# lizhiqi49/threestudio-3dgs

Measured on AMD Instinct MI355X. Metric: rendered views/sec fwd+bwd @1M Gaussians, 1024², SH=3; 1/2/4/8 GPU, higher is better.
Workload: dtype fp32

## Files before the change

threestudio-3dgs_amd/csrc/gsr_api.hip:

```cpp
#include <stdio.h>
#include <string.h>

#include <cmath>
#include <mutex>
#include <vector>

#include "../../include/gsr.h"
#include "gsr_kernels.h"

using namespace gsr;

static thread_local char g_err[512] = "";

static int fail(int code, const char* fmt, const char* what) {
  snprintf(g_err, sizeof(g_err), fmt, what);
  return code;
}

#define GSR_HIP_CHECK(expr)                                                        \
  do {                                                                             \
    hipError_t e_ = (expr);                                                        \
    if (e_ != hipSuccess) return fail(GSR_EHIP, "HIP error: %s", hipGetErrorString(e_)); \
  } while (0)

// ... 75 lines not shown
  int dm = (int)std::lround(std::sqrt((double)(M > 0 ? M : 1))) - 1;
  int d = degree < dm ? degree : dm;
  if (d < 0) d = 0;
  if (d > 3) d = 3;
  return d;
}

static int tile_sort_result(int W, int H) { return digit_plan(tile_key_bits(W, H)).passes & 1; }
static int depth_sort_result() { return digit_plan(32).passes & 1; }

static GaussBackwardArgs shared_args(const gsr_set_scene& sc, const gsr_set_grads& gr) {
  GaussBackwardArgs a;
  a.P = sc.P;
  a.g0 = 0;
  a.g1 = sc.P;
  a.M = sc.shs ? sc.M : 0;
  a.deg = effective_degree(sc.degree, a.M);
  a.means3D = sc.means3D;
  a.scales = sc.scales;
  a.rotations = sc.rotations;
  a.shs = sc.shs;
  a.cov3D_precomp = sc.cov3D_precomp;
  a.scale_modifier = sc.scale_modifier;
  a.dL_dcolors = gr.dL_dcolors;
  a.dL_dopacity = gr.dL_dopacity;
  a.dL_dmeans3D = gr.dL_dmeans3D;
  a.dL_dcov3D = gr.dL_dcov3D;
  a.dL_dsh = sc.shs ? gr.dL_dsh : nullptr;
  a.dL_dscales = sc.cov3D_precomp ? nullptr : gr.dL_dscales;
  a.dL_drotations = sc.cov3D_precomp ? nullptr : gr.dL_drotations;
  return a;
}

static int inst_segments(int V, const int* K, SegInfo& seg, long long* total) {
  seg.V = V;
  long long run = 0;
  for (int v = 0; v < V; ++v) {
    if (K[v] < 0) return fail(GSR_EINVAL, "%s", "negative instance count");
    seg.n[v] = (uint32_t)K[v];
    seg.start[v] = (uint32_t)run;
    run += K[v];
    if (run >= (1ll << 32)) return fail(GSR_EINVAL, "%s", "instances of a view set exceed 2^32: use smaller sets");
  }
  seg_fill_blocks(seg, GSR_SORT_TILE);
  if (total) *total = run;
  return GSR_OK;
}

static int set_cams(const gsr_set_scene& sc, SetCams& cams) {
  if (sc.viewmatrices == nullptr || sc.projmatrices == nullptr || sc.campos == nullptr || sc.tanfovx == nullptr ||
      sc.tanfovy == nullptr)
    return fail(GSR_EINVAL, "%s", "null camera array");
  for (int v = 0; v < sc.V; ++v) {
    if (sc.viewmatrices[v] == nullptr || sc.projmatrices[v] == nullptr || sc.campos[v] == nullptr)
      return fail(GSR_EINVAL, "%s", "null camera pointer");
    cams.c[v].view = sc.viewmatrices[v];
    cams.c[v].proj = sc.projmatrices[v];
    cams.c[v].campos = sc.campos[v];
    cams.c[v].tanx = sc.tanfovx[v];
    cams.c[v].tany = sc.tanfovy[v];
  }
  return GSR_OK;
}

static int check_set(int V, int P) {
  if (V < 1 || V > GSR_SET_MAX) return fail(GSR_EINVAL, "%s", "a view set holds 1..64 views");
  if (P < 0) return fail(GSR_EINVAL, "%s", "P must be >= 0");
  if ((long long)V * (long long)(P > 0 ? P : 1) >= (1ll << 32))
    return fail(GSR_EINVAL, "%s", "views x Gaussians of a set exceed 2^32: use smaller sets");
  return GSR_OK;
}

static void render_set_shared(RenderSet& rs, const GeomState& g, const ImageState& img, const BinningState& b,
                              const TilePack& tp, int tres, int V, int P, int width, int height) {
  rs.P = P;
  rs.W = width;
  rs.H = height;
  rs.gx = div_up(width, GSR_TILE_X);
  rs.gy = div_up(height, GSR_TILE_Y);
  rs.gmask = tp.gmask;
  rs.col2_rec = g.drange + 130;
  rs.order = img.order;
  rs.split_mode = img.split_mode;
  rs.split_items = img.split_items;
  rs.split_cap = img.split_cap;
  rs.split_extra = split_extra(V, (size_t)rs.gx * rs.gy);
  rs.qkeys = tp.qmask ? b.key[tres] : nullptr;
}

extern "C" {

#ifndef GSR_BUILD_ID
#define GSR_BUILD_ID "unknown"
#endif
const char* gsr_version(void) { return "gsr 0.4.0 gfx950 build " GSR_BUILD_ID; }
int gsr_abi_version(void) { return GSR_ABI_VERSION; }
const char* gsr_last_error(void) { return g_err; }


size_t gsr_set_geom_bytes(int V, int P) {
  size_t b = 0;
  GeomState::carve(nullptr, V, P, &b);
  return b;
}
static bool set_total(int V, const int* K, SegInfo& seg, long long* total) {
  return V >= 1 && V <= GSR_SET_MAX && K != nullptr && inst_segments(V, K, seg, total) == GSR_OK;
}
size_t gsr_set_binning_bytes(int V, int P, const int* K, int width, int height) {
  SegInfo seg;
  long long total = 0;
  if (!set_total(V, K, seg, &total)) return 0;
  size_t b = 0;
  BinningState::carve(nullptr, V, total, seg.blk[V], !set_tile_pack(P, width, height).packed, &b);
  return b;
}
size_t gsr_set_image_bytes(int V, int P, const int* K, int width, int height, int two_colors) {
  SegInfo seg;
  long long total = 0;
  if (K != nullptr && !set_total(V, K, seg, &total)) return 0;
  size_t b = 0;
  ImageState::carve(nullptr, V, width, height, &b,
                    K == nullptr || split_forward(V, P, width, height, total, two_colors != 0));
  return b;
}
static size_t carry_bytes(int P) { return align_up(sizeof(float) * 6 * (size_t)(P > 0 ? P : 1), 256); }

size_t gsr_set_backward_bytes(int V, int P, const int* K, int two_colors) {
  SegInfo seg;
  long long total = 0;
  if (!set_total(V, K, seg, &total)) return 0;
  return BackwardState::bytes_for(total, V, P, two_colors != 0) + carry_bytes(P);
}

static int check_timed(const gsr_set_scene& sc, const gsr_set_timed& tm) {
  if (sc.shs != nullptr) return fail(GSR_EINVAL, "%s", "timed view sets take precomputed colours: shs is not built");
  if (sc.cov3D_precomp != nullptr) return fail(GSR_EINVAL, "%s", "timed view sets: cov3D_precomp is not built");
  if (tm.means3D_v == nullptr && sc.P > 0) return fail(GSR_EINVAL, "%s", "timed view sets need means3D_v");
  return GSR_OK;
}
static gsr_set_scene timed_scene(const gsr_set_scene& sc, const gsr_set_timed& tm) {
  gsr_set_scene e = sc;
  e.means3D = tm.means3D_v;
  if (tm.scales_v != nullptr) e.scales = tm.scales_v;
  if (tm.rotations_v != nullptr) e.rotations = tm.rotations_v;
  return e;
}

static int set_preprocess(const gsr_set_scene* scene, const gsr_set_state* state, const float* colors2,
                          const gsr_set_timed* timed, void* stream) {
  const gsr_set_scene& sc = *scene;
  const int V = sc.V, P = sc.P;
  if (check_set(V, P) != GSR_OK) return GSR_EINVAL;
  if (sc.width <= 0 || sc.height <= 0) return fail(GSR_EINVAL, "%s", "image size must be positive");
  if ((sc.shs == nullptr) == (sc.colors_precomp == nullptr))
    return fail(GSR_EINVAL, "%s", "Please provide exactly one of either SHs or precomputed colors!");
  if (((sc.scales == nullptr || sc.rotations == nullptr) && sc.cov3D_precomp == nullptr) ||
      ((sc.scales != nullptr || sc.rotations != nullptr) && sc.cov3D_precomp != nullptr))
    return fail(GSR_EINVAL, "%s",
                "Please provide exactly one of either scale/rotation pair or precomputed 3D covariance!");
  if (state->geom == nullptr ||
      (P > 0 && (sc.means3D == nullptr || sc.opacities == nullptr || state->radii == nullptr)))
    return fail(GSR_EINVAL, "%s", "null pointer argument");
  if (sc.shs != nullptr && sc.M <= 0) return fail(GSR_EINVAL, "%s", "M must be >= 1 with SHs");
  SetCams cams;
  if (set_cams(sc, cams) != GSR_OK) return GSR_EINVAL;
  for (int v = 0; v < V; ++v) {
    cams.c[v].fx = (float)sc.width / (2.0f * cams.c[v].tanx);
    cams.c[v].fy = (float)sc.height / (2.0f * cams.c[v].tany);
  }
  hipStream_t s = (hipStream_t)stream;
  GeomState g = GeomState::carve(state->geom, V, P, nullptr);

  PreprocessArgs a;
  a.V = V;
  a.P = P;
  a.deg = effective_degree(sc.degree, sc.M);
  a.M = sc.M;
  a.means3D = sc.means3D;
  a.scales = sc.scales;
  a.rotations = sc.rotations;
  a.opacities = sc.opacities;
  a.shs = sc.shs;
  a.colors_precomp = sc.colors_precomp;
  a.cov3D_precomp = sc.cov3D_precomp;
  a.scale_modifier = sc.scale_modifier;
  a.W = sc.width;
  a.H = sc.height;
  a.radii = state->radii;
  a.col2 = colors2;
  {
    PhaseScope ps(GSR_PHASE_PREPROCESS, s);
    if (timed != nullptr) {
      const size_t n = (size_t)P;
      const PreprocessTimed pt = {3 * n, timed->scales_v ? 3 * n : 0, timed->rotations_v ? 4 * n : 0, 3 * n};
      launch_preprocess(a, cams, g, s, &pt);
    } else {
      launch_preprocess(a, cams, g, s);
    }
  }
  {
    PhaseScope ps(GSR_PHASE_DEPTH_SORT, s);
    SegInfo seg;
    seg.V = V;
    for (int v = 0; v < V; ++v) {
      seg.n[v] = (uint32_t)P;
      seg.start[v] = (uint32_t)((size_t)v * P);
    }
    seg.rebase = g.drange + 128;
    const int res = seg_sort(g.dkey, g.dval, false, seg, 0, 32, g.sort_counts, g.sort_totals, s);
    if (res != depth_sort_result()) return fail(GSR_EHIP, "%s", "internal: depth sort result buffer");
    launch_binning_counts(V, P, g, s);
  }
  return last_launch();
}

int gsr_set_preprocess(const gsr_set_scene* scene, const gsr_set_state* state, const float* colors2, void* stream) {
  if (scene == nullptr || state == nullptr) return fail(GSR_EINVAL, "%s", "null pointer argument");
  return set_preprocess(scene, state, colors2, nullptr, stream);
}

int gsr_set_timed_preprocess(const gsr_set_scene* scene, const gsr_set_state* state, const gsr_set_timed* timed,
                             void* stream) {
  if (scene == nullptr || state == nullptr || timed == nullptr) return fail(GSR_EINVAL, "%s", "null pointer argument");
  if (check_timed(*scene, *timed) != GSR_OK) return GSR_EINVAL;
  const gsr_set_scene e = timed_scene(*scene, *timed);
  return set_preprocess(&e, state, timed->colors2_v, timed, stream);
}

int gsr_composite_forward(int V, int height, int width, const float* color, const float* alpha, const float* bg,
                          int bg_layout, float* out, void* stream) {
  if (V < 0 || height < 0 || width < 0 || bg_layout < 0 || bg_layout > 2) return fail(GSR_EINVAL, "%s", "bad sizes");
  if (V == 0 || height == 0 || width == 0) return last_launch();
  if (color == nullptr || alpha == nullptr || bg == nullptr || out == nullptr)
    return fail(GSR_EINVAL, "%s", "null pointer argument");
  launch_composite_fwd(V, (size_t)height * width, color, alpha, bg, bg_layout, out, (hipStream_t)stream);
  return last_launch();
}

int gsr_composite_backward(int V, int height, int width, const float* dL_dout, const float* color,
                           const float* alpha, const float* bg, int bg_layout, float* dL_dcolor, float* dL_dalpha,
                           float* dL_dbg, void* stream) {
  if (V < 0 || height < 0 || width < 0 || bg_layout < 0 || bg_layout > 2) return fail(GSR_EINVAL, "%s", "bad sizes");
  if (V == 0 || height == 0 || width == 0) return last_launch();
  if (dL_dout == nullptr || color == nullptr || alpha == nullptr || bg == nullptr || dL_dcolor == nullptr ||
      dL_dalpha == nullptr)
    return fail(GSR_EINVAL, "%s", "null pointer argument");
  if (dL_dbg != nullptr && bg_layout == GSR_BG_CONSTANT)
    return fail(GSR_EINVAL, "%s", "dL_dbg is computed for image backgrounds only");
  launch_composite_bwd(V, (size_t)height * width, dL_dout, color, alpha, bg, bg_layout, dL_dcolor, dL_dalpha,
                       dL_dbg, (hipStream_t)stream);
  return last_launch();
}

int gsr_normal_map_forward(int V, int height, int width, const float* normal, const float* alpha, float* out,
                           void* stream) {
  if (V < 0 || height < 0 || width < 0) return fail(GSR_EINVAL, "%s", "bad sizes");
  if (V == 0 || height == 0 || width == 0) return last_launch();
  if (normal == nullptr || alpha == nullptr || out == nullptr) return fail(GSR_EINVAL, "%s", "null pointer argument");
  launch_normal_map_fwd(V, (size_t)height * width, normal, alpha, out, (hipStream_t)stream);
  return last_launch();
}

int gsr_normal_map_backward(int V, int height, int width, const float* dL_dout, const float* normal,
                            const float* alpha, float* dL_dnormal, float* dL_dalpha, void* stream) {
  if (V < 0 || height < 0 || width < 0) return fail(GSR_EINVAL, "%s", "bad sizes");
  if (V == 0 || height == 0 || width == 0) return last_launch();
  if (dL_dout == nullptr || normal == nullptr || alpha == nullptr || dL_dnormal == nullptr || dL_dalpha == nullptr)
    return fail(GSR_EINVAL, "%s", "null pointer argument");
  launch_normal_map_bwd(V, (size_t)height * width, dL_dout, normal, alpha, dL_dnormal, dL_dalpha, (hipStream_t)stream);
  return last_launch();
}

static int shade_args(int V, int H, int W, int flags, const int* modes, const float* color, const float* depth,
                      const float* alpha, const float* rays_o, const float* rays_d, const float* bg, int bg_layout,
                      const float* light, const float* pred_normal, const float* ambient, const float* diffuse,
                      ShadeArgs& A) {
  if (V < 0 || H < 0 || W < 0 || (flags & ~GSR_SHADE_MATERIAL) != 0)
    return fail(GSR_EINVAL, "%s", "bad sizes / flags");
  if (depth == nullptr || alpha == nullptr || rays_o == nullptr || rays_d == nullptr)
    return fail(GSR_EINVAL, "%s", "null pointer argument (depth / alpha / rays)");
  A = ShadeArgs{};
  A.V = V, A.H = H, A.W = W, A.flags = flags, A.bg_layout = bg_layout;
  A.color = color, A.depth = depth, A.alpha = alpha, A.rays_o = rays_o, A.rays_d = rays_d;
  A.bg = bg, A.light = light, A.pred_normal = pred_normal;
  if (flags & GSR_SHADE_MATERIAL) {
    if (color == nullptr || bg == nullptr || light == nullptr || ambient == nullptr || diffuse == nullptr ||
        modes == nullptr)
      return fail(GSR_EINVAL, "%s", "material: color, bg, light, ambient, diffuse and modes are required");
    if (bg_layout != GSR_BG_CONSTANT && bg_layout != GSR_BG_HWC)
      return fail(GSR_EINVAL, "%s", "material: bg_layout must be GSR_BG_CONSTANT or GSR_BG_HWC");
    for (int v = 0; v < V; ++v)
      if (modes[v] < GSR_SHADING_DIFFUSE || modes[v] > GSR_SHADING_TEXTURELESS)
        return fail(GSR_EINVAL, "%s", "bad shading mode");
  }
  return GSR_OK;
}

static void shade_launch(ShadeArgs A, const ShadeGrads* G, const int* modes, const float* ambient,
                         const float* diffuse, hipStream_t s) {
  const int V = A.V;
  for (int v0 = 0; v0 < V; v0 += GSR_SET_MAX) {
    const int n = V - v0 < GSR_SET_MAX ? V - v0 : GSR_SET_MAX;
    A.v0 = v0, A.V = n;
    for (int i = 0; i < n; ++i) {
      A.mode[i] = (A.flags & GSR_SHADE_MATERIAL) ? modes[v0 + i] : 0;
      for (int k = 0; k < 3; ++k) {
// ... 548 lines not shown
  if (((uintptr_t)c.pairs & 15u) != 0) return fail(GSR_EINVAL, "%s", "pairs must be 16-byte aligned");
  if (((uintptr_t)workspace & 7u) != 0) return fail(GSR_EINVAL, "%s", "workspace must be 8-byte aligned");
  if (workspace_bytes < meshreg_workspace_bytes(c.T, c.V, c.P, pass))
    return fail(GSR_EINVAL, "%s", "workspace too small");
  return GSR_OK;
}

size_t gsr_sugar_meshreg_workspace_bytes(int T, int V, int P, int pass) {
  if (pass < GSR_MESHREG_FORWARD || pass > GSR_MESHREG_LAP_BACKWARD) return 0;
  return meshreg_workspace_bytes(T < 0 ? 0 : T, V < 0 ? 0 : V, P < 0 ? 0 : P, pass);
}

int gsr_sugar_normal_consistency_forward(const gsr_sugar_meshreg* in, float* nc, void* workspace,
                                         size_t workspace_bytes, void* stream) {
  if (in == nullptr) return null_argument();
  if (meshreg_check(*in) != GSR_OK) return GSR_EINVAL;
  if (in->T == 0 || in->P == 0) return nothing_to_do();
  if (meshreg_args(*in, true, nc, "nc", workspace, workspace_bytes, false) != GSR_OK) return GSR_EINVAL;
  launch_normal_consistency_forward(*in, nc, workspace, (hipStream_t)stream);
  return last_launch();
}

int gsr_sugar_normal_consistency_backward(const gsr_sugar_meshreg* in, const float* dL_dnc, float* dL_dvert_xyz,
                                          void* workspace, size_t workspace_bytes, void* stream) {
  if (in == nullptr) return null_argument();
  if (meshreg_check(*in) != GSR_OK) return GSR_EINVAL;
  if (in->T == 0 || in->P == 0) return nothing_to_do();
  if (dL_dnc == nullptr) return null_named("dL_dnc");
  if (meshreg_args(*in, true, dL_dvert_xyz, "dL_dvert_xyz", workspace, workspace_bytes, true) != GSR_OK)
    return GSR_EINVAL;
  launch_normal_consistency_backward(*in, dL_dnc, dL_dvert_xyz, workspace, (hipStream_t)stream);
  return last_launch();
}

int gsr_sugar_laplacian_forward(const gsr_sugar_meshreg* in, float* lap, void* workspace, size_t workspace_bytes,
                                void* stream) {
  if (in == nullptr) return null_argument();
  if (meshreg_check(*in) != GSR_OK) return GSR_EINVAL;
  if (in->T == 0 || in->V == 0) return nothing_to_do();
  if (meshreg_args(*in, false, lap, "lap", workspace, workspace_bytes, false) != GSR_OK) return GSR_EINVAL;
  launch_laplacian_forward(*in, lap, workspace, (hipStream_t)stream);
  return last_launch();
}

int gsr_sugar_laplacian_backward(const gsr_sugar_meshreg* in, const float* dL_dlap, float* dL_dvert_xyz,
                                 void* workspace, size_t workspace_bytes, void* stream) {
  if (in == nullptr) return null_argument();
  if (meshreg_check(*in) != GSR_OK) return GSR_EINVAL;
  if (in->T == 0 || in->V == 0) return nothing_to_do();
  if (dL_dlap == nullptr) return null_named("dL_dlap");
  if (meshreg_args(*in, false, dL_dvert_xyz, "dL_dvert_xyz", workspace, workspace_bytes, true) != GSR_OK)
    return GSR_EINVAL;
  launch_laplacian_backward(*in, dL_dlap, dL_dvert_xyz, workspace, (hipStream_t)stream);
  return last_launch();
}

int gsr_densify_stats(const gsr_densify_batch* in, void* stream) {
  if (in == nullptr) return null_argument();
  if (in->V < 0 || in->V > GSR_SET_MAX) return fail(GSR_EINVAL, "%s", "a densification call takes 0..64 views");
  if (in->P < 0) return fail(GSR_EINVAL, "%s", "P must be >= 0");
  if (in->P == 0 || in->V == 0) return nothing_to_do();
  if (in->max_radii == nullptr) return null_named("max_radii");
  if (in->grad_norm_sum == nullptr) return null_named("grad_norm_sum");
  if (in->count == nullptr) return null_named("count");
  int with_rows = 0;
  for (int v = 0; v < in->V; ++v) {
    if (in->radii[v] == nullptr) return null_named("radii row");
    with_rows += in->visible[v] != nullptr;
  }
  if (with_rows != 0 && with_rows != in->V)
    return fail(GSR_EINVAL, "%s", "visibility rows must be given for every view or for none");
  launch_densify_stats(*in, (hipStream_t)stream);
  return last_launch();
}

struct SortWork {
  uint32_t *keys2, *vals2, *counts, *totals;
  static SortWork carve(void* base, int V, long long total, uint32_t blocks, size_t* bytes) {
    Carver c(base);
    SortWork w;
    w.keys2 = c.take<uint32_t>((size_t)(total > 0 ? total : 1));
    w.vals2 = c.take<uint32_t>((size_t)(total > 0 ? total : 1));
    w.counts = c.take<uint32_t>((size_t)GSR_RADIX * (blocks > 0 ? blocks : 1));
    w.totals = c.take<uint32_t>((size_t)GSR_RADIX * (size_t)V);
    if (bytes) *bytes = align_up(c.off, 256);
    return w;
  }
};

size_t gsr_sort_work_bytes(int V, const int* n) {
  SegInfo seg;
  long long total = 0;
  if (!set_total(V, n, seg, &total)) return 0;
  size_t b = 0;
  SortWork::carve(nullptr, V, total, seg.blk[V], &b);
  return b;
}

int gsr_sort_pairs(int V, const int* n, uint32_t* keys, uint32_t* vals, int key_bits, int max_bits, void* work,
                   size_t work_bytes, void* stream) {
  if (V < 1 || V > GSR_SET_MAX) return fail(GSR_EINVAL, "%s", "1..64 segments");
  if (n == nullptr || keys == nullptr || work == nullptr) return fail(GSR_EINVAL, "%s", "null pointer argument");
  if (key_bits < 1 || key_bits > 32 || max_bits < 1 || max_bits > GSR_RADIX_BITS)
    return fail(GSR_EINVAL, "%s", "key_bits must be 1..32 and max_bits 1..8");
  SegInfo seg;
  long long total = 0;
  if (inst_segments(V, n, seg, &total) != GSR_OK) return GSR_EINVAL;
  size_t need = 0;
  SortWork w = SortWork::carve(work, V, total, seg.blk[V], &need);
  if (work_bytes < need) return fail(GSR_EINVAL, "%s", "sort work buffer too small");
  if (total == 0) return last_launch();
  hipStream_t s = (hipStream_t)stream;
  uint32_t* kk[2] = {keys, w.keys2};
  uint32_t* vv[2] = {vals, vals != nullptr ? w.vals2 : nullptr};
  const int r = seg_sort(kk, vals != nullptr ? vv : nullptr, false, seg, 0, key_bits, w.counts, w.totals, s,
                         max_bits);
  if (r == 1) {
    GSR_HIP_CHECK(hipMemcpyAsync(keys, w.keys2, sizeof(uint32_t) * (size_t)total, hipMemcpyDeviceToDevice, s));
    if (vals != nullptr)
      GSR_HIP_CHECK(hipMemcpyAsync(vals, w.vals2, sizeof(uint32_t) * (size_t)total, hipMemcpyDeviceToDevice, s));
  }
  return last_launch();
}

int gsr_sort_rank_mode(void) { return sort_rank_mode(); }

int gsr_set_num_rendered(int V, const void* geom, int P, int* num_rendered, int* num_visible, int* num_listed,
                         void* stream) {
  if (check_set(V, P) != GSR_OK) return GSR_EINVAL;
  if (geom == nullptr || num_rendered == nullptr) return fail(GSR_EINVAL, "%s", "null pointer argument");
  GeomState g = GeomState::carve((void*)geom, V, P, nullptr);
  hipStream_t s = (hipStream_t)stream;
  static thread_local uint32_t* pinned = nullptr;
  if (pinned == nullptr) GSR_HIP_CHECK(hipHostMalloc((void**)&pinned, 3 * GSR_SET_MAX * sizeof(uint32_t), hipHostMallocDefault));
  GSR_HIP_CHECK(hipMemcpyAsync(pinned, g.counters, 3 * (size_t)V * sizeof(uint32_t), hipMemcpyDeviceToHost, s));
  GSR_HIP_CHECK(hipStreamSynchronize(s));
  for (int v = 0; v < V; ++v) {
    num_rendered[v] = (int)pinned[v];
    if (num_visible) num_visible[v] = (int)pinned[V + v];
    if (num_listed) num_listed[v] = (int)pinned[2 * V + v];
    if (pinned[v] > 0x7fffffffu) return fail(GSR_EINVAL, "%s", "instance count of a view exceeds 2^31");
  }
  g_err[0] = 0;
  return GSR_OK;
}

int gsr_set_gauss_state(int V, const void* geom, int P, void* out_rec, void* out_tiles, void* stream) {
  if (check_set(V, P) != GSR_OK) return GSR_EINVAL;
  if (geom == nullptr) return fail(GSR_EINVAL, "%s", "null pointer argument");
  if (P == 0) return GSR_OK;
  GeomState g = GeomState::carve((void*)geom, V, P, nullptr);
  hipStream_t s = (hipStream_t)stream;
  const size_t n = (size_t)V * (size_t)P;
  if (out_rec) GSR_HIP_CHECK(hipMemcpyAsync(out_rec, g.rec, n * sizeof(GaussRec), hipMemcpyDeviceToDevice, s));
  if (out_tiles) GSR_HIP_CHECK(hipMemcpyAsync(out_tiles, g.tiles, n * sizeof(uint2), hipMemcpyDeviceToDevice, s));
  return last_launch();
}

int gsr_set_render(const gsr_set_scene* scene, const gsr_set_state* state, const gsr_set_outputs* outputs,
                   void* stream) {
  if (scene == nullptr || state == nullptr || outputs == nullptr)
    return fail(GSR_EINVAL, "%s", "null pointer argument");
  const gsr_set_outputs& o = *outputs;
  const int V = scene->V, P = scene->P, width = scene->width, height = scene->height;
  const int* K = state->num_rendered;
  const float* const* bgs = scene->bgs;
  void *geom = state->geom, *binning = state->binning, *image = state->image;
  const float* colors2 = o.colors2;
  if (check_set(V, P) != GSR_OK) return GSR_EINVAL;
  if ((colors2 == nullptr) != (o.out_color2 == nullptr)) return fail(GSR_EINVAL, "%s", "null second colour argument");
  if (o.bg_images != nullptr && o.out_render == nullptr) return fail(GSR_EINVAL, "%s", "composite needs out_render");
  if (width <= 0 || height <= 0) return fail(GSR_EINVAL, "%s", "bad sizes");
  if (K == nullptr || bgs == nullptr || geom == nullptr || binning == nullptr || image == nullptr ||
      o.out_color == nullptr || o.out_depth == nullptr || o.out_alpha == nullptr)
    return fail(GSR_EINVAL, "%s", "null pointer argument");
  for (int v = 0; v < V; ++v)
    if (bgs[v] == nullptr) return fail(GSR_EINVAL, "%s", "null background");
  SegInfo inst;
  long long total = 0;
  if (inst_segments(V, K, inst, &total) != GSR_OK) return GSR_EINVAL;
  hipStream_t s = (hipStream_t)stream;
  GeomState g = GeomState::carve(geom, V, P, nullptr);
  const TilePack tp = set_tile_pack(P, width, height);
  BinningState b = BinningState::carve(binning, V, total, inst.blk[V], !tp.packed, nullptr);
  const bool split = split_forward(V, P, width, height, total, colors2 != nullptr);
  ImageState img = ImageState::carve(image, V, width, height, nullptr, split);
  const int gx = div_up(width, GSR_TILE_X), gy = div_up(height, GSR_TILE_Y);
  const int tres = tile_sort_result(width, height);
  inst.ndev = g.counters + 2 * V;
  GSR_HIP_CHECK(hipMemsetAsync(img.split_mode, split ? 1 : 0, sizeof(uint32_t), s));
  const bool tile_masks = fwd_tile_chosen(total, (long long)V * P, V);
  GSR_HIP_CHECK(hipMemsetAsync(img.split_mode + 1, total > 0 ? (tile_masks ? 1 : 2) : 0, sizeof(uint32_t), s));
  {
    PhaseScope ps(GSR_PHASE_BINNING, s);
    GSR_HIP_CHECK(hipMemsetAsync(img.ranges, 0, sizeof(uint2) * (size_t)V * gx * gy, s));
    if (total > 0) {
      launch_emit(V, P, width, g, inst, tp, b.key[0], b.val[0], s);
      const int res = seg_sort(b.key, b.val, false, inst, tp.gbits, tp.tile_bits, b.sort_counts, b.sort_totals, s);
      if (res != tres) return fail(GSR_EHIP, "%s", "internal: tile sort buffer");
      launch_tile_ranges(inst, gx * gy, tp, b.key[res], img.ranges, s);
    }
    launch_tile_order(V, gx, gy, img.ranges, img.order, s);
  }
  {
    PhaseScope ps(GSR_PHASE_RENDER_FWD, s);
    RenderSet rs;
    render_set_shared(rs, g, img, b, tp, tres, V, P, width, height);
    rs.cbg = o.bg_images;
    rs.comp = o.out_render;
    rs.ccolor = nullptr;
    rs.dcbg = nullptr;
    rs.col2 = colors2;
    rs.out_col2 = o.out_color2;
    rs.dpix2 = nullptr;
    rs.ochunk = order_chunk(V, gx, gy, true);
    rs.ckpt = split ? img.ckpt : nullptr;
    rs.qbytes = total > 0 ? reinterpret_cast<uint8_t*>(b.key[tres ^ 1]) : nullptr;
    rs.V = V;
    rs.v0 = 0;
    for (int v = 0; v < V; ++v) {
      rs.inst_start[v] = inst.start[v];
      rs.row_start[v] = 0;
      rs.bg[v] = bgs[v];
    }
    launch_render_forward(rs, g, tp.packed ? b.key[tres] : b.val[tres], img, o.out_color, o.out_depth, o.out_alpha,
                          total, s);
  }
  return last_launch();
}

static int grad_chunk_size(int P, int n) {
  const int q = (P + n - 1) / n;
  return (q + GSR_GRAD_CHUNK_ALIGN - 1) / GSR_GRAD_CHUNK_ALIGN * GSR_GRAD_CHUNK_ALIGN;
}

static int set_backward(const gsr_set_scene* scene, const gsr_set_state* state, const gsr_set_grads* grads,
                        const gsr_set_timed* timed, const gsr_set_timed_grads* tgrads, void* stream) {
  const gsr_set_scene& sc = *scene;
  const gsr_set_grads& gr = *grads;
  const int V = sc.V, P = sc.P, width = sc.width, height = sc.height;
  const int* K = state->num_rendered;
  const float* const* bgs = sc.bgs;
  const float *colors_override = gr.colors_override, *color = gr.color, *comp_bg = gr.bg_images;
  float *dL_dcov3D = gr.dL_dcov3D, *dL_dbg = gr.dL_dbg;
  const float *dL_dcolor = gr.dL_dcolor, *dL_ddepth = gr.dL_ddepth, *dL_dalpha = gr.dL_dalpha;
  if (check_set(V, P) != GSR_OK) return GSR_EINVAL;
  const bool two = gr.colors2 != nullptr || gr.dL_dcolor2 != nullptr || gr.dL_dcolors2 != nullptr;
  if (two && (gr.colors2 == nullptr || gr.dL_dcolor2 == nullptr || gr.dL_dcolors2 == nullptr ||
              colors_override != nullptr))
    return fail(GSR_EINVAL, "%s", "two-colour backward needs colors2, dL_dcolor2 and dL_dcolors2");
  if (colors_override != nullptr && (sc.shs != nullptr || gr.dL_dsh != nullptr || dL_ddepth != nullptr ||
                                     dL_dalpha != nullptr))
    return fail(GSR_EINVAL, "%s", "colors_override excludes SHs and the depth / alpha gradients");
  if (comp_bg != nullptr && color == nullptr) return fail(GSR_EINVAL, "%s", "composite needs the forward's color");
  if (comp_bg == nullptr && dL_dbg != nullptr) return fail(GSR_EINVAL, "%s", "dL_dbg needs bg_images");
  if (gr.n_chunks < 0 || gr.n_chunks > GSR_GRAD_CHUNKS_MAX || (gr.n_chunks > 0 && gr.chunk_events == nullptr))
    return fail(GSR_EINVAL, "%s", "bad gradient chunk request");
  if (width <= 0 || height <= 0) return fail(GSR_EINVAL, "%s", "bad sizes");
  if (P == 0) return last_launch();
  if (K == nullptr || bgs == nullptr || state->geom == nullptr || state->binning == nullptr ||
      state->image == nullptr || gr.work == nullptr || dL_dcolor == nullptr || gr.dL_dmeans2D == nullptr ||
      gr.dL_dcolors == nullptr || gr.dL_dopacity == nullptr || (timed == nullptr && gr.dL_dmeans3D == nullptr) ||
      state->radii == nullptr || sc.means3D == nullptr)
    return fail(GSR_EINVAL, "%s", "null pointer argument");
  for (int v = 0; v < V; ++v)
    if (bgs[v] == nullptr) return fail(GSR_EINVAL, "%s", "null background");
  if (sc.shs != nullptr && gr.dL_dsh == nullptr) return fail(GSR_EINVAL, "%s", "dL_dsh required with SHs");
  const bool need_dscales = timed == nullptr || timed->scales_v == nullptr;
  const bool need_drots = timed == nullptr || timed->rotations_v == nullptr;
  if (sc.cov3D_precomp == nullptr && (sc.scales == nullptr || sc.rotations == nullptr ||
                                      (need_dscales && gr.dL_dscales == nullptr) ||
                                      (need_drots && gr.dL_drotations == nullptr)))
    return fail(GSR_EINVAL, "%s", "scales/rotations and their gradients required");
  SetCams cams;
  if (set_cams(sc, cams) != GSR_OK) return GSR_EINVAL;
  SegInfo inst;
  long long total = 0;
  if (inst_segments(V, K, inst, &total) != GSR_OK) return GSR_EINVAL;
  hipStream_t s = (hipStream_t)stream;
  GeomState g = GeomState::carve(state->geom, V, P, nullptr);
  const TilePack tp = set_tile_pack(P, width, height);
  BinningState b = BinningState::carve(state->binning, V, total, inst.blk[V], !tp.packed, nullptr);
  ImageState img = ImageState::carve(state->image, V, width, height, nullptr, true);
  const int gx = div_up(width, GSR_TILE_X), gy = div_up(height, GSR_TILE_Y);
  const size_t HW = (size_t)width * height;
  const int tres = tile_sort_result(width, height);
  const uint32_t* sorted = tp.packed ? b.key[tres] : b.val[tres];
  GaussBackwardArgs a = shared_args(sc, gr);
  if (timed == nullptr && gr.accumulate != 0 && sc.cov3D_precomp == nullptr && dL_dcov3D == nullptr)
    return fail(GSR_EINVAL, "%s", "accumulate needs dL_dcov3D: it carries the running dL/dcov3D between calls");
  void* work = gr.work;
  if (gr.work_bytes < carry_bytes(P)) return fail(GSR_EINVAL, "%s", "backward work buffer too small");
  const size_t avail = (gr.work_bytes - carry_bytes(P)) & ~(size_t)255;
  float* carry = dL_dcov3D ? dL_dcov3D : (float*)((char*)work + avail);
  bool first = gr.accumulate == 0;
  for (int g0 = 0; g0 < V;) {
    int g1 = g0;
    long long rows = 0;
    while (g1 < V && (g1 == g0 || BackwardState::bytes_for(rows + K[g1], g1 + 1 - g0, P, two) <= avail))
      rows += K[g1++];
    if (BackwardState::bytes_for(rows, g1 - g0, P, two) > avail)
      return fail(GSR_EINVAL, "%s", "backward work buffer smaller than one view's gradient rows");
    BackwardState bw = BackwardState::carve(work, rows, P, two);
    RenderSet rs;
    render_set_shared(rs, g, img, b, tp, tres, V, P, width, height);
    rs.cbg = comp_bg ? comp_bg + (size_t)g0 * HW * 3 : nullptr;
    rs.comp = nullptr;
// ... 237 lines not shown
```

threestudio-3dgs_amd/csrc/gsr_backward.hip:

```cpp
#include <cstdlib>
#include <cstring>

#include "gsr_chain.h"
#include "gsr_kernels.h"
#include "gsr_math.h"
#include "gsr_wave.h"

namespace gsr {

__device__ __forceinline__ void sh_backward(int deg, int M, const float* sh, float (&dsh)[48], float3 dRGB,
                                            const float3 mean, const float* campos, float3& dmean) {
  const float3 dir_orig = make_float3(mean.x - campos[0], mean.y - campos[1], mean.z - campos[2]);
  const float len = sqrtf(dir_orig.x * dir_orig.x + dir_orig.y * dir_orig.y + dir_orig.z * dir_orig.z);
  const float x = dir_orig.x / len, y = dir_orig.y / len, z = dir_orig.z / len;
  float basis[16];
  float bdx[16], bdy[16], bdz[16];
#pragma unroll
  for (int k = 0; k < 16; ++k) basis[k] = bdx[k] = bdy[k] = bdz[k] = 0.f;
  basis[0] = SH_C0;
  if (deg > 0) {
    basis[1] = -SH_C1 * y; basis[2] = SH_C1 * z; basis[3] = -SH_C1 * x;
    bdy[1] = -SH_C1; bdz[2] = SH_C1; bdx[3] = -SH_C1;
    if (deg > 1) {
      const float xx = x * x, yy = y * y, zz = z * z, xy = x * y, yz = y * z, xz = x * z;
      basis[4] = SH_C2[0] * xy; basis[5] = SH_C2[1] * yz;
      basis[6] = SH_C2[2] * (2.f * zz - xx - yy); basis[7] = SH_C2[3] * xz;
      basis[8] = SH_C2[4] * (xx - yy);
      bdx[4] = SH_C2[0] * y; bdy[4] = SH_C2[0] * x;
      bdy[5] = SH_C2[1] * z; bdz[5] = SH_C2[1] * y;
      bdx[6] = SH_C2[2] * 2.f * -x; bdy[6] = SH_C2[2] * 2.f * -y; bdz[6] = SH_C2[2] * 2.f * 2.f * z;
      bdx[7] = SH_C2[3] * z; bdz[7] = SH_C2[3] * x;
      bdx[8] = SH_C2[4] * 2.f * x; bdy[8] = SH_C2[4] * 2.f * -y;
      if (deg > 2) {
        basis[9] = SH_C3[0] * y * (3.f * xx - yy);
        basis[10] = SH_C3[1] * xy * z;
        basis[11] = SH_C3[2] * y * (4.f * zz - xx - yy);
        basis[12] = SH_C3[3] * z * (2.f * zz - 3.f * xx - 3.f * yy);
        basis[13] = SH_C3[4] * x * (4.f * zz - xx - yy);
        basis[14] = SH_C3[5] * z * (xx - yy);
        basis[15] = SH_C3[6] * x * (xx - 3.f * yy);
        bdx[9] = SH_C3[0] * 3.f * 2.f * xy;          bdy[9] = SH_C3[0] * 3.f * (xx - yy);
        bdx[10] = SH_C3[1] * yz;                     bdy[10] = SH_C3[1] * xz;          bdz[10] = SH_C3[1] * xy;
        bdx[11] = SH_C3[2] * -2.f * xy;              bdy[11] = SH_C3[2] * (-3.f * yy + 4.f * zz - xx);
        bdz[11] = SH_C3[2] * 4.f * 2.f * yz;
        bdx[12] = SH_C3[3] * -3.f * 2.f * xz;        bdy[12] = SH_C3[3] * -3.f * 2.f * yz;
        bdz[12] = SH_C3[3] * 3.f * (2.f * zz - xx - yy);
        bdx[13] = SH_C3[4] * (-3.f * xx + 4.f * zz - yy); bdy[13] = SH_C3[4] * -2.f * xy;
        bdz[13] = SH_C3[4] * 4.f * 2.f * xz;
        bdx[14] = SH_C3[5] * 2.f * xz;               bdy[14] = SH_C3[5] * -2.f * yz;   bdz[14] = SH_C3[5] * (xx - yy);
        bdx[15] = SH_C3[6] * 3.f * (xx - yy);        bdy[15] = SH_C3[6] * -3.f * 2.f * xy;
      }
    }
  }
  const int ncoef = (deg + 1) * (deg + 1);
  float3 dRGBdx = make_float3(0.f, 0.f, 0.f), dRGBdy = dRGBdx, dRGBdz = dRGBdx;
#pragma unroll
  for (int k = 0; k < 16; ++k) {
    if (k < ncoef && k < M) {
      dsh[3 * k] += basis[k] * dRGB.x;
      dsh[3 * k + 1] += basis[k] * dRGB.y;
      dsh[3 * k + 2] += basis[k] * dRGB.z;
      if (k > 0) {
        const float3 s = make_float3(sh[3 * k], sh[3 * k + 1], sh[3 * k + 2]);
        dRGBdx.x += bdx[k] * s.x; dRGBdx.y += bdx[k] * s.y; dRGBdx.z += bdx[k] * s.z;
        dRGBdy.x += bdy[k] * s.x; dRGBdy.y += bdy[k] * s.y; dRGBdy.z += bdy[k] * s.z;
        dRGBdz.x += bdz[k] * s.x; dRGBdz.y += bdz[k] * s.y; dRGBdz.z += bdz[k] * s.z;
      }
    }
  }
  const float3 ddir = make_float3(dRGBdx.x * dRGB.x + dRGBdx.y * dRGB.y + dRGBdx.z * dRGB.z,
                                  dRGBdy.x * dRGB.x + dRGBdy.y * dRGB.y + dRGBdy.z * dRGB.z,
                                  dRGBdz.x * dRGB.x + dRGBdz.y * dRGB.y + dRGBdz.z * dRGB.z);
  const float3 v = dir_orig;
  const float sum2 = v.x * v.x + v.y * v.y + v.z * v.z;
  const float invsum32 = 1.0f / sqrtf(sum2 * sum2 * sum2);
  dmean.x += ((sum2 - v.x * v.x) * ddir.x - v.y * v.x * ddir.y - v.z * v.x * ddir.z) * invsum32;
  dmean.y += (-v.x * v.y * ddir.x + (sum2 - v.y * v.y) * ddir.y - v.z * v.y * ddir.z) * invsum32;
  dmean.z += (-v.x * v.z * ddir.x - v.y * v.z * ddir.y + (sum2 - v.z * v.z) * ddir.z) * invsum32;
}

static inline __host__ __device__ int sh_lds_stride(int M) { return ((3 * M + 3) & ~3) + 4; }

#ifndef GSR_VG_ITEMS
#define GSR_VG_ITEMS 16
#endif
template <bool TWO, bool CUT_LDS>
__attribute__((amdgpu_waves_per_eu(4, 8)))
__global__ __launch_bounds__(256) void k_view_grad(GaussBackwardArgs a, ViewGradArgs va) {
  extern __shared__ uint2 s_cut[];
  const int t = threadIdx.x;
  const int vl = blockIdx.x % va.V;
  const int vg = va.v0 + vl;
  const uint2* cut = CUT_LDS ? reinterpret_cast<const uint2*>(s_cut) : va.img.cut + (size_t)vg * va.tiles;
  if (CUT_LDS) {
    const uint4* src = reinterpret_cast<const uint4*>(va.img.cut + (size_t)vg * va.tiles);
    uint4* dst = reinterpret_cast<uint4*>(s_cut);
    for (int k = t; k < va.tiles / 2; k += 256) dst[k] = src[k];
    if ((va.tiles & 1) && t == 0) s_cut[va.tiles - 1] = va.img.cut[(size_t)vg * va.tiles + va.tiles - 1];
    __syncthreads();
  }
  const ViewCam& cam = va.cam[vl];
  typedef __attribute__((address_space(4))) const float* cfptr;
  float viewm[16], projm[16];
#pragma unroll
  for (int i = 0; i < 16; ++i) viewm[i] = ((cfptr)cam.view)[i], projm[i] = ((cfptr)cam.proj)[i];
  ViewGeom vgm;
  vgm.view = viewm;
  vgm.proj = projm;
  vgm.tanx = cam.tanx;
  vgm.tany = cam.tany;
  vgm.fy = va.H / (2.0f * cam.tany);
  vgm.fx = va.W / (2.0f * cam.tanx);
  const float4* grow = va.grow + (size_t)(TWO ? 4 : 3) * va.row_start[vl];
  constexpr int RS = TWO ? GSR_REC_STRIDE2 : GSR_REC_STRIDE;
  float4* recv = reinterpret_cast<float4*>(va.vrec + (size_t)vl * RS * a.P);
  const unsigned long long vbit = 1ull << vl;
  __shared__ uint16_t s_list[4][64 * GSR_VG_ITEMS];
  const int wave = t >> 6, lane = t & 63;
  uint16_t* list = s_list[wave];
  const int items = va.items;
  const int slice = a.g0 + (blockIdx.x / va.V) * (256 * items);
  int cnt = 0;
#pragma unroll
  for (int it = 0; it < GSR_VG_ITEMS; ++it) {
    const int local = it * 256 + t;
    const int idx = slice + local;
    const bool valid = it < items && idx < a.g1;
    const bool rch = valid && (va.reach[idx] & vbit) != 0ull;
    if (valid && !rch) {
      float* m2 = va.dmeans2D + 3 * ((size_t)vg * a.P + idx);
      m2[0] = 0.f;
      m2[1] = 0.f;
      m2[2] = 0.f;
    }
    const unsigned long long bal = __ballot(rch);
    if (rch) list[cnt + mask_rank(bal)] = (uint16_t)local;
    cnt += __popcll(bal);
  }
  asm volatile("s_waitcnt lgkmcnt(0)" ::: "memory");
  GaussRec nrec;
  uint32_t ngo = 0u;
  int nidx = 0;
  if (lane < cnt) {
    nidx = slice + list[lane];
    const size_t o0 = (size_t)vg * a.P + nidx;
    nrec = va.g.rec[o0], ngo = va.g.goff[o0];
  }
#pragma unroll 1
  for (int i = lane; i - lane < cnt; i += 64) {
    if (i >= cnt) break;
    const int idx = nidx;
    const size_t o = (size_t)vg * a.P + idx;
    const GaussRec gr = nrec;
    const uint32_t go = ngo;
    if (i + 64 < cnt) {
      nidx = slice + list[i + 64];
      const size_t on = (size_t)vg * a.P + nidx;
      nrec = va.g.rec[on], ngo = va.g.goff[on];
    }
    float* m2 = va.dmeans2D + 3 * o;
    float4* rec = recv + (size_t)idx * (RS / 4);
    const uint32_t clamp_bits = gr.d.w;
    const RowSums r = gather_rows<TWO>((uint32_t)idx, gr, go, va.gx, cut, grow);
    bool reached = (r.dmx != 0.f) | (r.dmy != 0.f) | (r.dca != 0.f) | (r.dcb != 0.f) | (r.dcc != 0.f) |
                   (r.dop != 0.f) | (r.dcr != 0.f) | (r.dcg != 0.f) | (r.dcbl != 0.f) | (r.ddep != 0.f);
    if (TWO) reached = reached | (r.dr2 != 0.f) | (r.dg2 != 0.f) | (r.db2 != 0.f);
    if (!reached) {
      m2[0] = 0.f;
      m2[1] = 0.f;
      m2[2] = 0.f;
#pragma unroll
      for (int q = 0; q < RS / 4; ++q)
        rec[q] = q == 3 ? make_float4(0.f, __uint_as_float(clamp_bits), 0.f, 0.f) : make_float4(0.f, 0.f, 0.f, 0.f);
      continue;
    }
    m2[0] = TWO ? r.dmx1 : r.dmx;
    m2[1] = TWO ? r.dmy1 : r.dmy;
    m2[2] = 0.f;
    const float3 mean = make_float3(a.means3D[3 * idx], a.means3D[3 * idx + 1], a.means3D[3 * idx + 2]);
    float cov3D[6];
    if (a.cov3D_precomp) {
#pragma unroll
      for (int k = 0; k < 6; ++k) cov3D[k] = a.cov3D_precomp[6 * idx + k];
    } else {
      const float3 scale = make_float3(a.scales[3 * idx], a.scales[3 * idx + 1], a.scales[3 * idx + 2]);
      const float4 rot = make_float4(a.rotations[4 * idx], a.rotations[4 * idx + 1], a.rotations[4 * idx + 2],
                                     a.rotations[4 * idx + 3]);
      cov3d_from_scale_rot(scale, a.scale_modifier, rot, cov3D);
    }
    float dcv[6];
    float3 dm;
    cov2d_backward(mean, cov3D, vgm, r.dca, r.dcb, r.dcc, dcv, dm);
    proj_backward(mean, projm, r.dmx, r.dmy, dm);
    dm.x += viewm[2] * r.ddep;
    dm.y += viewm[6] * r.ddep;
    dm.z += viewm[10] * r.ddep;
    const float f[GSR_REC_STRIDE2] = {dm.x,   dm.y,  dm.z,  dcv[0], dcv[1], dcv[2], dcv[3],
                                      dcv[4], dcv[5], r.dcr, r.dcg,  r.dcbl, r.dop,  __uint_as_float(clamp_bits),
                                      r.dr2,  r.dg2, r.db2, 0.f,   0.f,    0.f};
#pragma unroll
    for (int q = 0; q < RS / 4; ++q) rec[q] = make_float4(f[4 * q], f[4 * q + 1], f[4 * q + 2], f[4 * q + 3]);
  }
}

__attribute__((amdgpu_waves_per_eu(3, 8)))
__global__ __launch_bounds__(256) void k_gauss_accum(GaussBackwardArgs a, AccumArgs b) {
  extern __shared__ __attribute__((aligned(16))) float s_sh[];
  const int t = threadIdx.x;
  const int block0 = a.g0 + blockIdx.x * 256;
  const int idx = block0 + t;
  const int nblk = min(256, a.g1 - block0);
  const int F = 3 * a.M;
  const int S = sh_lds_stride(a.M);
  const bool has_sh = a.shs != nullptr && F > 0;
  const bool acc = b.accumulate != 0;
  const float invF = has_sh ? 1.0f / (float)F : 0.0f;
  __shared__ uint8_t s_rl[256];
  __shared__ int s_wcnt[4];
  const unsigned long long reach_word = idx < a.g1 ? b.reach[idx] : 0ull;
  const bool reached = reach_word != 0ull;
  int nr = 0;
  if (has_sh) {
    const unsigned long long bal = __ballot(reached);
    const int w = t >> 6;
    if ((t & 63) == 0) s_wcnt[w] = (int)__popcll(bal);
    __syncthreads();
    int base = 0;
    for (int k = 0; k < 4; ++k) {
      base += k < w ? s_wcnt[k] : 0;
      nr += s_wcnt[k];
    }
    if (reached) s_rl[base + mask_rank(bal)] = (uint8_t)t;
    __syncthreads();
    const int cnt = nr * F;
    for (int e = t; e < cnt; e += 256) {
      const int r = (int)(((float)e + 0.5f) * invF);
      const int tl = s_rl[r];
      const int k = e - r * F;
      s_sh[tl * S + k] = a.shs[(size_t)(block0 + tl) * F + k];
    }
    __syncthreads();
  }
  if (idx < a.g1 && !reached) {
    if (!acc) {
      for (int k = 0; k < 3; ++k) a.dL_dmeans3D[3 * idx + k] = 0.f;
      a.dL_dopacity[idx] = 0.f;
      if (a.dL_dcolors)
        for (int k = 0; k < 3; ++k) a.dL_dcolors[3 * idx + k] = 0.f;
      if (b.dcolors2)
        for (int k = 0; k < 3; ++k) b.dcolors2[3 * idx + k] = 0.f;
      if (b.dcov_carry)
        for (int k = 0; k < 6; ++k) b.dcov_carry[6 * idx + k] = 0.f;
      if (a.dL_dcov3D && a.dL_dcov3D != b.dcov_carry)
        for (int k = 0; k < 6; ++k) a.dL_dcov3D[6 * idx + k] = 0.f;
      if (!a.cov3D_precomp && a.dL_dscales) {
        for (int k = 0; k < 3; ++k) a.dL_dscales[3 * idx + k] = 0.f;
        for (int k = 0; k < 4; ++k) a.dL_drotations[4 * idx + k] = 0.f;
      }
      if (has_sh) {
        float* row = s_sh + t * S;
        for (int k = 0; k < F; ++k) row[k] = 0.f;
      }
    }
  } else if (idx < a.g1) {
    const float3 mean = make_float3(a.means3D[3 * idx], a.means3D[3 * idx + 1], a.means3D[3 * idx + 2]);
    float3 dmean = make_float3(0.f, 0.f, 0.f);
    float dcov[6] = {0.f, 0.f, 0.f, 0.f, 0.f, 0.f};
    float dop = 0.f, dcr = 0.f, dcg = 0.f, dcb = 0.f;
    float dsh[48];
#pragma unroll
    for (int k = 0; k < 48; ++k) dsh[k] = 0.f;
    if (acc) {
      dmean = make_float3(a.dL_dmeans3D[3 * idx], a.dL_dmeans3D[3 * idx + 1], a.dL_dmeans3D[3 * idx + 2]);
      dop = a.dL_dopacity[idx];
      if (a.dL_dcolors) dcr = a.dL_dcolors[3 * idx], dcg = a.dL_dcolors[3 * idx + 1], dcb = a.dL_dcolors[3 * idx + 2];
      if (b.dcov_carry)
#pragma unroll
        for (int k = 0; k < 6; ++k) dcov[k] = b.dcov_carry[6 * idx + k];
      if (has_sh) {
        const float* prev = a.dL_dsh + (size_t)idx * F;
#pragma unroll
        for (int k = 0; k < 48; ++k)
          if (k < F) dsh[k] = prev[k];
      }
    }
    const float* sh_row = has_sh ? s_sh + t * S : nullptr;
    const int RS = b.dcolors2 ? GSR_REC_STRIDE2 : GSR_REC_STRIDE;
    float d2[3] = {0.f, 0.f, 0.f};
    if (b.dcolors2 && acc)
      for (int k = 0; k < 3; ++k) d2[k] = b.dcolors2[3 * idx + k];
    unsigned long long pending = reach_word;
    auto next_view = [&]() -> int {
      if (pending == 0ull) return -1;
      const int v = __builtin_ctzll(pending);
      pending &= pending - 1ull;
      return v;
    };
    auto load = [&](float4 (&f)[4], int vl) {
      const float4* src = reinterpret_cast<const float4*>(b.vrec + ((size_t)vl * a.P + idx) * RS);
#pragma unroll
      for (int q = 0; q < 4; ++q) f[q] = src[q];
    };
    auto process = [&](const float4 (&f4)[4], int vl) {
      const float f[16] = {f4[0].x, f4[0].y, f4[0].z, f4[0].w, f4[1].x, f4[1].y, f4[1].z, f4[1].w,
                           f4[2].x, f4[2].y, f4[2].z, f4[2].w, f4[3].x, f4[3].y, f4[3].z, f4[3].w};
      dmean.x += f[0];
      dmean.y += f[1];
      dmean.z += f[2];
#pragma unroll
      for (int k = 0; k < 6; ++k) dcov[k] += f[3 + k];
      dcr += f[9];
      dcg += f[10];
      dcb += f[11];
      dop += f[12];
      if (b.dcolors2) {
        d2[0] += f[14];
        d2[1] += f[15];
        d2[2] += b.vrec[((size_t)vl * a.P + idx) * RS + 16];
      }
      if (has_sh && ((f[9] != 0.f) | (f[10] != 0.f) | (f[11] != 0.f))) {
        const uint32_t cl = __float_as_uint(f[13]);
        const float3 dRGB = make_float3((cl & 1u) ? 0.f : f[9], (cl & 2u) ? 0.f : f[10], (cl & 4u) ? 0.f : f[11]);
        const float* shv = sh_row;
        typedef __attribute__((address_space(4))) const float* cfptr;
        const float cpos[3] = {((cfptr)b.campos[vl])[0], ((cfptr)b.campos[vl])[1], ((cfptr)b.campos[vl])[2]};
        sh_backward(a.deg, a.M, shv, dsh, dRGB, mean, cpos, dmean);
      }
    };
    float4 fa[4], fb[4];
    int va_ = next_view(), vb_ = next_view();
    if (va_ >= 0) load(fa, va_);
    if (vb_ >= 0) load(fb, vb_);
    for (;;) {
      if (va_ < 0) break;
      process(fa, va_);
      va_ = next_view();
      if (va_ >= 0) load(fa, va_);
      if (vb_ < 0) break;
      process(fb, vb_);
      vb_ = next_view();
      if (vb_ >= 0) load(fb, vb_);
    }
    a.dL_dmeans3D[3 * idx] = dmean.x;
    a.dL_dmeans3D[3 * idx + 1] = dmean.y;
    a.dL_dmeans3D[3 * idx + 2] = dmean.z;
    a.dL_dopacity[idx] = dop;
    if (a.dL_dcolors) {
      a.dL_dcolors[3 * idx] = dcr;
      a.dL_dcolors[3 * idx + 1] = dcg;
      a.dL_dcolors[3 * idx + 2] = dcb;
    }
    if (b.dcolors2)
      for (int k = 0; k < 3; ++k) b.dcolors2[3 * idx + k] = d2[k];
    if (b.dcov_carry)
      for (int k = 0; k < 6; ++k) b.dcov_carry[6 * idx + k] = dcov[k];
    if (a.dL_dcov3D && a.dL_dcov3D != b.dcov_carry)
      for (int k = 0; k < 6; ++k) a.dL_dcov3D[6 * idx + k] = dcov[k];
    if (!a.cov3D_precomp && a.dL_dscales) {
      const float3 scale = make_float3(a.scales[3 * idx], a.scales[3 * idx + 1], a.scales[3 * idx + 2]);
      const float4 rot = make_float4(a.rotations[4 * idx], a.rotations[4 * idx + 1], a.rotations[4 * idx + 2],
                                     a.rotations[4 * idx + 3]);
      float ds[3], dq[4];
      scale_rot_backward(scale, rot, a.scale_modifier, dcov, ds, dq);
      for (int k = 0; k < 3; ++k) a.dL_dscales[3 * idx + k] = ds[k];
      for (int k = 0; k < 4; ++k) a.dL_drotations[4 * idx + k] = dq[k];
    }
    if (has_sh) {
      float* row = s_sh + t * S;
      float4* row4w = reinterpret_cast<float4*>(row);
#pragma unroll
      for (int c = 0; c < 12; ++c)
        if (4 * c < F) row4w[c] = make_float4(dsh[4 * c], dsh[4 * c + 1], dsh[4 * c + 2], dsh[4 * c + 3]);
      for (int k = 48; k < F; ++k) row[k] = 0.f;
    }
  }
  if (has_sh) {
    __syncthreads();
    if (!acc) {
      float* dst = a.dL_dsh + (size_t)block0 * F;
      const int cnt = nblk * F;
      for (int e = t; e < cnt; e += 256) {
        const int te = (int)(((float)e + 0.5f) * invF);
        dst[e] = s_sh[te * S + (e - te * F)];
      }
    } else {
      const int cnt = nr * F;
      for (int e = t; e < cnt; e += 256) {
        const int r = (int)(((float)e + 0.5f) * invF);
        const int tl = s_rl[r];
        const int k = e - r * F;
        a.dL_dsh[(size_t)(block0 + tl) * F + k] = s_sh[tl * S + k];
      }
    }
  }
}

template <bool TWO>
__global__ __launch_bounds__(256) void k_gauss_fused(GaussBackwardArgs a, ViewGradArgs va, AccumArgs b) {
  const int idx = a.g0 + blockIdx.x * 256 + threadIdx.x;
  const bool valid = idx < a.g1;
  const int ix = valid ? idx : a.g0;
  const bool acc = b.accumulate != 0;
  const unsigned long long reach_word = valid ? va.reach[ix] : 0ull;
  float3 dmean = make_float3(0.f, 0.f, 0.f);
  float dcov[6] = {0.f, 0.f, 0.f, 0.f, 0.f, 0.f};
  float dop = 0.f, dcr = 0.f, dcg = 0.f, dcb = 0.f;
  float d2[3] = {0.f, 0.f, 0.f};
  if (valid && acc) {
    dmean = make_float3(a.dL_dmeans3D[3 * idx], a.dL_dmeans3D[3 * idx + 1], a.dL_dmeans3D[3 * idx + 2]);
    dop = a.dL_dopacity[idx];
    if (a.dL_dcolors) dcr = a.dL_dcolors[3 * idx], dcg = a.dL_dcolors[3 * idx + 1], dcb = a.dL_dcolors[3 * idx + 2];
    if (b.dcov_carry)
#pragma unroll
      for (int k = 0; k < 6; ++k) dcov[k] = b.dcov_carry[6 * idx + k];
    if (TWO)
      for (int k = 0; k < 3; ++k) d2[k] = b.dcolors2[3 * idx + k];
  }
  const float3 mean = make_float3(a.means3D[3 * ix], a.means3D[3 * ix + 1], a.means3D[3 * ix + 2]);
  float cov3D[6];
  if (reach_word != 0ull) {
    if (a.cov3D_precomp) {
#pragma unroll
      for (int k = 0; k < 6; ++k) cov3D[k] = a.cov3D_precomp[6 * ix + k];
    } else {
      const float3 scale = make_float3(a.scales[3 * ix], a.scales[3 * ix + 1], a.scales[3 * ix + 2]);
      const float4 rot = make_float4(a.rotations[4 * ix], a.rotations[4 * ix + 1], a.rotations[4 * ix + 2],
                                     a.rotations[4 * ix + 3]);
      cov3d_from_scale_rot(scale, a.scale_modifier, rot, cov3D);
    }
  }
  GaussRec nrec;
  uint32_t ngo = 0u;
  auto fetch = [&](int vl) {
    const size_t o = (size_t)(va.v0 + vl) * a.P + ix;
    nrec = va.g.rec[o];
    ngo = va.g.goff[o];
  };
  const int vfirst = reach_word != 0ull ? (int)__builtin_ctzll(reach_word) : va.V;
  if (vfirst < va.V) fetch(vfirst);
#pragma unroll 1
  for (int vl = 0; vl < va.V; ++vl) {
    const int vg = va.v0 + vl;
    float* m2 = va.dmeans2D + 3 * ((size_t)vg * a.P + ix);
    if (!((reach_word >> vl) & 1ull)) {
      if (valid) m2[0] = 0.f, m2[1] = 0.f, m2[2] = 0.f;
      continue;
    }
    const GaussRec gr = nrec;
    const uint32_t go = ngo;
    const unsigned long long later = reach_word & ~((2ull << vl) - 1ull);
    if (later != 0ull) fetch((int)__builtin_ctzll(later));
    const ViewCam& cam = va.cam[vl];
    typedef __attribute__((address_space(4))) const float* cfptr;
    float viewm[16], projm[16];
#pragma unroll
    for (int i = 0; i < 16; ++i) viewm[i] = ((cfptr)cam.view)[i], projm[i] = ((cfptr)cam.proj)[i];
    ViewGeom vgm;
    vgm.view = viewm;
    vgm.proj = projm;
    vgm.tanx = cam.tanx;
    vgm.tany = cam.tany;
    vgm.fy = va.H / (2.0f * cam.tany);
    vgm.fx = va.W / (2.0f * cam.tanx);
    const float4* grow = va.grow + (size_t)(TWO ? 4 : 3) * va.row_start[vl];
    const uint2* cut = va.img.cut + (size_t)vg * va.tiles;
    const RowSums r = gather_rows<TWO>((uint32_t)ix, gr, go, va.gx, cut, grow);
    bool reached = (r.dmx != 0.f) | (r.dmy != 0.f) | (r.dca != 0.f) | (r.dcb != 0.f) | (r.dcc != 0.f) |
                   (r.dop != 0.f) | (r.dcr != 0.f) | (r.dcg != 0.f) | (r.dcbl != 0.f) | (r.ddep != 0.f);
    if (TWO) reached = reached | (r.dr2 != 0.f) | (r.dg2 != 0.f) | (r.db2 != 0.f);
    if (!reached) {
      if (valid) m2[0] = 0.f, m2[1] = 0.f, m2[2] = 0.f;
      continue;
    }
    if (valid) {
      m2[0] = TWO ? r.dmx1 : r.dmx;
      m2[1] = TWO ? r.dmy1 : r.dmy;
      m2[2] = 0.f;
    }
    float dcv[6];
    float3 dm;
    cov2d_backward(mean, cov3D, vgm, r.dca, r.dcb, r.dcc, dcv, dm);
    proj_backward(mean, projm, r.dmx, r.dmy, dm);
    dm.x += viewm[2] * r.ddep;
    dm.y += viewm[6] * r.ddep;
    dm.z += viewm[10] * r.ddep;
    dmean.x += dm.x;
    dmean.y += dm.y;
    dmean.z += dm.z;
#pragma unroll
    for (int k = 0; k < 6; ++k) dcov[k] += dcv[k];
    dcr += r.dcr;
    dcg += r.dcg;
    dcb += r.dcbl;
    dop += r.dop;
    if (TWO) {
      d2[0] += r.dr2;
      d2[1] += r.dg2;
      d2[2] += r.db2;
    }
  }
  if (!valid) return;
  a.dL_dmeans3D[3 * idx] = dmean.x;
  a.dL_dmeans3D[3 * idx + 1] = dmean.y;
  a.dL_dmeans3D[3 * idx + 2] = dmean.z;
  a.dL_dopacity[idx] = dop;
  if (a.dL_dcolors) {
    a.dL_dcolors[3 * idx] = dcr;
    a.dL_dcolors[3 * idx + 1] = dcg;
    a.dL_dcolors[3 * idx + 2] = dcb;
  }
  if (TWO)
    for (int k = 0; k < 3; ++k) b.dcolors2[3 * idx + k] = d2[k];
  if (b.dcov_carry)
    for (int k = 0; k < 6; ++k) b.dcov_carry[6 * idx + k] = dcov[k];
  if (a.dL_dcov3D && a.dL_dcov3D != b.dcov_carry)
    for (int k = 0; k < 6; ++k) a.dL_dcov3D[6 * idx + k] = dcov[k];
  if (!a.cov3D_precomp && a.dL_dscales) {
    const float3 scale = make_float3(a.scales[3 * idx], a.scales[3 * idx + 1], a.scales[3 * idx + 2]);
    const float4 rot = make_float4(a.rotations[4 * idx], a.rotations[4 * idx + 1], a.rotations[4 * idx + 2],
                                   a.rotations[4 * idx + 3]);
    float ds[3], dq[4];
    scale_rot_backward(scale, rot, a.scale_modifier, dcov, ds, dq);
    for (int k = 0; k < 3; ++k) a.dL_dscales[3 * idx + k] = ds[k];
    for (int k = 0; k < 4; ++k) a.dL_drotations[4 * idx + k] = dq[k];
  }
}

static bool gauss_fused_on(const GaussBackwardArgs& a) {
  if (a.shs != nullptr && a.M > 0) return false;
  const char* e = getenv("GSR_GAUSS_FUSED");
  return !(e != nullptr && strcmp(e, "0") == 0);
}

#define GSR_CUT_LDS_MAX (48 * 1024)

void launch_gauss_backward(const GaussBackwardArgs& a, ViewGradArgs va, const AccumArgs& b, hipStream_t stream) {
  const int n = a.g1 - a.g0;
  if (n <= 0 || va.V <= 0) return;
  if (gauss_fused_on(a)) {
    auto kern = b.dcolors2 ? k_gauss_fused<true> : k_gauss_fused<false>;
    hipLaunchKernelGGL(kern, dim3(div_up(n, 256)), dim3(256), 0, stream, a, va, b);
    return;
  }
  const size_t cut_bytes = sizeof(uint2) * (size_t)va.tiles;
  va.cut_in_lds = cut_bytes <= GSR_CUT_LDS_MAX ? 1 : 0;
  va.items = GSR_VG_ITEMS;
  while (va.items > 2 && (long long)va.V * div_up(n, 256 * va.items) < 1024) va.items >>= 1;
  const dim3 vg_grid(va.V * div_up(n, 256 * va.items));
  auto vg_kern = b.dcolors2 ? (va.cut_in_lds ? k_view_grad<true, true> : k_view_grad<true, false>)
                            : (va.cut_in_lds ? k_view_grad<false, true> : k_view_grad<false, false>);
  hipLaunchKernelGGL(vg_kern, vg_grid, dim3(256), va.cut_in_lds ? cut_bytes : 0, stream, a, va);
  const size_t lds = (a.shs && a.M > 0) ? (size_t)256 * sh_lds_stride(a.M) * sizeof(float) : 0;
  hipLaunchKernelGGL(k_gauss_accum, dim3(div_up(n, 256)), dim3(256), lds, stream, a, b);
}

}
```

threestudio-3dgs_amd/csrc/gsr_binning.hip:

```cpp
#include "gsr_kernels.h"
#include "gsr_wave.h"

namespace gsr {

#ifndef GSR_INST_GROUPS
#define GSR_INST_GROUPS 8
#endif
__global__ __launch_bounds__(256) void k_inst_count(int P, int nbe, GeomState g) {
  const uint32_t* __restrict__ order = g.sorted_dval();
  constexpr int GPB = 4 * GSR_INST_GROUPS;
  const int nbb = (nbe + GPB - 1) / GPB;
  const int v = blockIdx.x / nbb;
  const int lb0 = (blockIdx.x - v * nbb) * GPB + (threadIdx.x >> 6) * GSR_INST_GROUPS;
  const int lane = threadIdx.x & 63;
  const size_t vo = (size_t)v * P;
  const uint32_t ks = g.vsent();
  uint32_t val[GSR_INST_GROUPS];
#pragma unroll
  for (int k = 0; k < GSR_INST_GROUPS; ++k) {
    const int r = (lb0 + k) * GSR_DUP_TILE + lane;
    val[k] = lb0 + k < nbe && r < P ? order[vo + r] : 0u;
  }
  uint32_t mine = 0u;
#pragma unroll
  for (int k = 0; k < GSR_INST_GROUPS; ++k) {
    uint32_t kept = 0u;
    if (lb0 + k < nbe && (lb0 + k) * GSR_DUP_TILE + lane < P) {
      kept = g.vbits <= 26 ? val[k] >> g.vbits : ks;
      if (kept == ks) kept = g.tiles[vo + (val[k] & g.vmask())].y;
    }
    const uint32_t ktot = __builtin_amdgcn_readlane((int)wave_incl_sum_dpp(kept), 63);
    if (lane == k) mine = ktot;
  }
  if (lane < GSR_INST_GROUPS && lb0 + lane < nbe) g.kept_counts[(size_t)v * nbe + lb0 + lane] = mine;
}

#define GSR_ISCAN_PER 8
__global__ __launch_bounds__(1024) void k_inst_scan(int nbe, GeomState g) {
  constexpr int CH = 1024 * GSR_ISCAN_PER;
  __shared__ uint32_t s_x[CH + CH / 8];
  __shared__ uint32_t s_w[16];
  const int v = blockIdx.x, t = threadIdx.x, w = t >> 6, lane = t & 63;
  uint32_t* kept = g.kept_counts + (size_t)v * nbe;
  auto pad = [](int i) { return i + (i >> 3); };
  uint32_t carry = 0u;
  for (int c0 = 0; c0 < nbe; c0 += CH) {
#pragma unroll
    for (int k = 0; k < GSR_ISCAN_PER; ++k) {
      const int i = k * 1024 + t;
      s_x[pad(i)] = c0 + i < nbe ? kept[c0 + i] : 0u;
    }
    __syncthreads();
    uint32_t x[GSR_ISCAN_PER], run = 0u;
#pragma unroll
    for (int k = 0; k < GSR_ISCAN_PER; ++k) {
      x[k] = run;
      run += s_x[pad(t * GSR_ISCAN_PER + k)];
    }
    uint32_t inc = run;
#pragma unroll
    for (int o = 1; o < 64; o <<= 1) {
      const uint32_t y = (uint32_t)__shfl_up((int)inc, o, 64);
      if (lane >= o) inc += y;
    }
    if (lane == 63) s_w[w] = inc;
    __syncthreads();
    uint32_t before = 0u, tot = 0u;
#pragma unroll
    for (int i = 0; i < 16; ++i) {
      const uint32_t sw = s_w[i];
      before += i < w ? sw : 0u;
      tot += sw;
    }
    const uint32_t off = carry + before + (inc - run);
#pragma unroll
    for (int k = 0; k < GSR_ISCAN_PER; ++k) s_x[pad(t * GSR_ISCAN_PER + k)] = off + x[k];
    __syncthreads();
#pragma unroll
    for (int k = 0; k < GSR_ISCAN_PER; ++k) {
      const int i = k * 1024 + t;
      if (c0 + i < nbe) kept[c0 + i] = s_x[pad(i)];
    }
    carry += tot;
    __syncthreads();
  }
  if (t == 0) g.counters[2 * gridDim.x + v] = carry;
}

__global__ __launch_bounds__(256) void k_goff_count(int P, int nbg, GeomState g) {
  __shared__ uint32_t s_wave[8];
  const int v = blockIdx.x / nbg, b = blockIdx.x - v * nbg, t = threadIdx.x;
  const uint2* tl = g.tiles + (size_t)v * P;
  uint32_t sum = 0u, vis = 0u;
#pragma unroll
  for (int k = 0; k < GSR_GOFF_TILE / 256; ++k) {
    const int i = b * GSR_GOFF_TILE + k * 256 + t;
    const uint32_t x = i < P ? tl[i].x : 0u;
    sum += x;
    vis += x > 0u ? 1u : 0u;
  }
  sum = block_sum_u32<256>(sum, s_wave);
  vis = block_sum_u32<256>(vis, s_wave);
  if (t == 0) g.goff_part[(size_t)v * nbg + b] = sum, g.vis_part[(size_t)v * nbg + b] = vis;
}

__global__ __launch_bounds__(1024) void k_goff_scan(int nbg, GeomState g) {
  __shared__ uint32_t s_w[16];
  const int v = blockIdx.x, t = threadIdx.x, w = t >> 6, lane = t & 63;
  uint32_t* row = g.goff_part + (size_t)v * nbg;
  uint32_t carry = 0u, vis = 0u;
  for (int i = t; i < nbg; i += 1024) vis += g.vis_part[(size_t)v * nbg + i];
  for (int c0 = 0; c0 < nbg; c0 += 1024 * 4) {
    const int i0 = c0 + 4 * t;
    uint32_t x[4], run = 0u;
#pragma unroll
    for (int k = 0; k < 4; ++k) {
      x[k] = run;
      run += i0 + k < nbg ? row[i0 + k] : 0u;
    }
    uint32_t inc = run;
#pragma unroll
    for (int o = 1; o < 64; o <<= 1) {
      const uint32_t y = (uint32_t)__shfl_up((int)inc, o, 64);
      if (lane >= o) inc += y;
    }
    if (lane == 63) s_w[w] = inc;
    __syncthreads();
    uint32_t before = 0u, tot = 0u;
#pragma unroll
    for (int i = 0; i < 16; ++i) {
      const uint32_t sw = s_w[i];
      before += i < w ? sw : 0u;
      tot += sw;
    }
    __syncthreads();
    const uint32_t off = carry + before + (inc - run);
#pragma unroll
    for (int k = 0; k < 4; ++k)
      if (i0 + k < nbg) row[i0 + k] = off + x[k];
    carry += tot;
  }
  __syncthreads();
#pragma unroll
  for (int o = 32; o > 0; o >>= 1) vis += (uint32_t)__shfl_xor((int)vis, o, 64);
  if (lane == 0) s_w[w] = vis;
  __syncthreads();
  if (t == 0) {
    uint32_t vt = 0u;
    for (int i = 0; i < 16; ++i) vt += s_w[i];
    g.counters[v] = carry;
    g.counters[gridDim.x + v] = vt;
  }
}

__global__ __launch_bounds__(256) void k_goff_write(int P, int nbg, GeomState g) {
  __shared__ uint32_t s_x[GSR_GOFF_TILE + GSR_GOFF_TILE / 16];
  __shared__ uint32_t s_wave[8];
  const int v = blockIdx.x / nbg, b = blockIdx.x - v * nbg, t = threadIdx.x;
  const uint2* tl = g.tiles + (size_t)v * P + (size_t)b * GSR_GOFF_TILE;
  uint32_t* go = g.goff + (size_t)v * P + (size_t)b * GSR_GOFF_TILE;
  const int n = min(GSR_GOFF_TILE, P - b * GSR_GOFF_TILE);
  constexpr int PER = GSR_GOFF_TILE / 256;
  auto pad = [](int i) { return i + (i >> 4); };
#pragma unroll
  for (int k = 0; k < PER; ++k) {
    const int i = k * 256 + t;
    s_x[pad(i)] = i < n ? tl[i].x : 0u;
  }
  __syncthreads();
  uint32_t x[PER], run = 0u;
#pragma unroll
  for (int k = 0; k < PER; ++k) {
    const uint32_t c = s_x[pad(t * PER + k)];
    x[k] = run;
    run += c;
  }
  uint32_t tot;
  const uint32_t off = g.goff_part[(size_t)v * nbg + b] + block_exclusive_scan<256>(run, &tot, s_wave);
#pragma unroll
  for (int k = 0; k < PER; ++k) s_x[pad(t * PER + k)] = off + x[k];
  __syncthreads();
#pragma unroll
  for (int k = 0; k < PER; ++k) {
    const int i = k * 256 + t;
    if (i < n) go[i] = s_x[pad(i)];
  }
}

template <bool QM>
struct EmitLDS {
  uint32_t gi[GSR_DUP_TILE];
  uint32_t roff[GSR_DUP_TILE];
  uint2 rect[GSR_DUP_TILE];
  SpanPrep sp[GSR_DUP_TILE];
  uint32_t own[64];
  uint32_t rk[64];
  uint32_t rtile[64];
  uint32_t rgi[64];
  uint32_t rx0[QM ? 64 : 1];
  uint2 rq[QM ? 64 : 1];
  uint32_t kown[64];
};

#ifndef GSR_EMIT_GROUPS
#define GSR_EMIT_GROUPS 2
#endif

template <bool QM>
__global__ __launch_bounds__(64) void k_emit(int P, int nbe, int grid_x, GeomState g, SegInfo inst, int gbits,
                                             uint32_t* __restrict__ keys, uint32_t* __restrict__ vals) {
  const uint32_t* __restrict__ order = g.sorted_dval();
  const uint32_t* __restrict__ dkeys = g.sorted_dkey();
  __shared__ EmitLDS<QM> s;
  const int nw = div_up(nbe, GSR_EMIT_GROUPS);
  const int v = blockIdx.x / nw;
  const int lb0 = (blockIdx.x % nw) * GSR_EMIT_GROUPS, lb1 = min(nbe, lb0 + GSR_EMIT_GROUPS);
  const int lane = threadIdx.x;
  const size_t vo = (size_t)v * P;
  uint32_t* kout = keys + inst.start[v];
  uint32_t* vout = vals ? vals + inst.start[v] : nullptr;
  uint32_t n_gi = 0u, n_koff = 0u;
  bool n_vis = false;
  float4 n_ra = make_float4(0.f, 0.f, 0.f, 0.f), n_rb = n_ra;
  uint2 n_d = make_uint2(0u, 0u);
  auto fetch = [&](int lb) {
    const int r = lb * GSR_DUP_TILE + lane;
    n_gi = r < P ? (order[vo + r] & g.vmask()) : 0u;
    n_vis = r < P && dkeys[vo + r] != 0xFFFFFFFFu;
    n_koff = g.kept_counts[(size_t)v * nbe + lb];
    if (n_vis) {
      const GaussRec& rc = g.rec[vo + n_gi];
      const uint4 d = rc.d;
      n_d = make_uint2(d.x, d.y);
      n_ra = rc.a;
      n_rb = rc.b;
    }
  };
  if (lb0 < lb1) fetch(lb0);
  for (int lb = lb0; lb < lb1; ++lb) {
    const uint32_t gi = n_gi;
    const bool vis = n_vis;
    const float4 ra = n_ra, rb = n_rb;
    const uint2 d = n_d;
    uint32_t kbase = n_koff;
    if (lb + 1 < lb1) fetch(lb + 1);
    uint32_t cnt = 0u, h = 0u;
    if (vis) {
      const uint32_t wd = (d.y & 0xffffu) - (d.x & 0xffffu);
      h = (d.y >> 16) - (d.x >> 16);
      cnt = wd * h;
      if (cnt == 0u) h = 0u;
    }
    const uint32_t rincl = wave_incl_sum_dpp(h);
    const uint32_t roff = rincl - h;
    const uint32_t R = (uint32_t)__builtin_amdgcn_readlane((int)rincl, 63);
    s.gi[lane] = gi;
    s.roff[lane] = roff;
    s.rect[lane] = d;
    if (h) s.sp[lane] = span_prep(ra.x, ra.y, ra.z, ra.w, rb.x, rb.y);
    uint32_t carry = 0u;
    for (uint32_t r0 = 0; r0 < R; r0 += 64) {
      s.own[lane] = 0u;
      asm volatile("s_waitcnt lgkmcnt(0)" ::: "memory");
      if (h && roff >= r0 && roff < r0 + 64) s.own[roff - r0] = (uint32_t)lane + 1u;
      asm volatile("s_waitcnt lgkmcnt(0)" ::: "memory");
      const uint32_t ow1 = max(carry, wave_incl_max_dpp(s.own[lane]));
      carry = (uint32_t)__builtin_amdgcn_readlane((int)ow1, 63);
      const uint32_t r = r0 + (uint32_t)lane;
      uint32_t kc = 0u, tile0 = 0u, rg = 0u;
      if (r < R) {
        const uint32_t ow = ow1 - 1u;
        const uint2 rc = s.rect[ow];
        const int xmin = (int)(rc.x & 0xffffu), xmax = (int)(rc.y & 0xffffu);
        const int row = (int)(rc.x >> 16) + (int)(r - s.roff[ow]);
        int t0, t1;
        span_row(s.sp[ow], row, xmin, xmax, t0, t1);
        kc = (uint32_t)(t1 - t0);
        tile0 = (uint32_t)row * (uint32_t)grid_x + (uint32_t)t0;
        rg = s.gi[ow];
        if (QM) {
          const float v1 = s.sp[ow].py - (float)(row * GSR_TILE_Y);
          s.rx0[lane] = (uint32_t)t0;
          s.rq[lane] = make_uint2(span_quads(s.sp[ow], v1), span_quads(s.sp[ow], v1 - 8.0f));
        }
      }
      const uint32_t kincl = wave_incl_sum_dpp(kc);
      const uint32_t kstart = kincl - kc;
      const uint32_t KC = (uint32_t)__builtin_amdgcn_readlane((int)kincl, 63);
      s.rk[lane] = kstart;
      s.rtile[lane] = tile0;
      s.rgi[lane] = rg;
      uint32_t kcarry = 0u;
      for (uint32_t k0 = 0; k0 < KC; k0 += 64) {
        s.kown[lane] = 0u;
        asm volatile("s_waitcnt lgkmcnt(0)" ::: "memory");
        if (kc && kstart >= k0 && kstart < k0 + 64) s.kown[kstart - k0] = (uint32_t)lane + 1u;
        asm volatile("s_waitcnt lgkmcnt(0)" ::: "memory");
        const uint32_t kw1 = max(kcarry, wave_incl_max_dpp(s.kown[lane]));
        kcarry = (uint32_t)__builtin_amdgcn_readlane((int)kw1, 63);
        const uint32_t j = k0 + (uint32_t)lane;
        if (j < KC) {
          const uint32_t rr = kw1 - 1u;
          const uint32_t tile = s.rtile[rr] + (j - s.rk[rr]);
          const uint32_t gv = s.rgi[rr];
          uint32_t qm = 0u;
          if (QM) {
            const uint2 rq = s.rq[rr];
            qm = quads_of_tile(rq.x, rq.y, (int)(s.rx0[rr] + (j - s.rk[rr])));
          }
          kout[kbase + j] = vout ? (QM ? tile | qm << GSR_QMASK_SHIFT : tile) : ((tile << gbits) | gv);
          if (vout) vout[kbase + j] = gv;
        }
        asm volatile("s_waitcnt lgkmcnt(0)" ::: "memory");
      }
      kbase += KC;
      asm volatile("s_waitcnt lgkmcnt(0)" ::: "memory");
    }
  }
}

__global__ __launch_bounds__(256) void k_tile_bounds(SegInfo inst, int n_tiles, int gbits, uint32_t tmask,
                                                     const uint32_t* __restrict__ keys, uint2* __restrict__ ranges) {
  const int v = blockIdx.y;
  const int t = blockIdx.x * 256 + threadIdx.x;
  if (t > n_tiles) return;
  const uint32_t K = seg_live(inst, v);
  const uint32_t* kv = keys + inst.start[v];
  uint32_t lo = 0u;
  uint32_t step = K == 0u ? 0u : 1u << (31 - __builtin_clz(K));
  for (; step > 0u; step >>= 1) {
    const uint32_t m = lo + step;
    if (m <= K && ((kv[m - 1] >> gbits) & tmask) < (uint32_t)t) lo = m;
  }
  uint2* rv = ranges + (size_t)v * n_tiles;
  if (t < n_tiles) rv[t].x = lo;
  if (t > 0) rv[t - 1].y = lo;
}

void launch_binning_counts(int V, int P, const GeomState& g, hipStream_t stream) {
  if (V <= 0) return;
  const int nbe = GeomState::dup_blocks(P);
  const int nbg = GeomState::goff_blocks(P);
  if (P > 0) hipLaunchKernelGGL(k_goff_count, dim3(V * nbg), dim3(256), 0, stream, P, nbg, g);
  hipLaunchKernelGGL(k_goff_scan, dim3(V), dim3(1024), 0, stream, P > 0 ? nbg : 0, g);
  if (P > 0) hipLaunchKernelGGL(k_goff_write, dim3(V * nbg), dim3(256), 0, stream, P, nbg, g);
  if (P > 0)
    hipLaunchKernelGGL(k_inst_count, dim3(V * ((nbe + 4 * GSR_INST_GROUPS - 1) / (4 * GSR_INST_GROUPS))), dim3(256),
                       0, stream, P, nbe, g);
  hipLaunchKernelGGL(k_inst_scan, dim3(V), dim3(1024), 0, stream, P > 0 ? nbe : 0, g);
}

void launch_emit(int V, int P, int W, const GeomState& g, const SegInfo& inst, const TilePack& tp, uint32_t* keys,
                 uint32_t* vals, hipStream_t stream) {
  if (V <= 0 || P <= 0) return;
  const int nbe = GeomState::dup_blocks(P);
  const dim3 grid(V * div_up(nbe, GSR_EMIT_GROUPS));
  if (tp.qmask)
    hipLaunchKernelGGL(k_emit<true>, grid, dim3(64), 0, stream, P, nbe, div_up(W, GSR_TILE_X), g, inst, tp.gbits,
                       keys, vals);
  else
    hipLaunchKernelGGL(k_emit<false>, grid, dim3(64), 0, stream, P, nbe, div_up(W, GSR_TILE_X), g, inst, tp.gbits,
                       keys, vals);
}

void launch_tile_ranges(SegInfo inst, int n_tiles, const TilePack& tp, const uint32_t* keys, uint2* ranges,
                        hipStream_t stream) {
  if (inst.V <= 0 || n_tiles <= 0) return;
  hipLaunchKernelGGL(k_tile_bounds, dim3(div_up(n_tiles + 1, 256), inst.V), dim3(256), 0, stream, inst, n_tiles,
                     tp.gbits, tp.tmask, keys, ranges);
}

__global__ __launch_bounds__(256) void k_mark_visible(int P, const float* __restrict__ means3D,
                                                      const float* __restrict__ view,
                                                      const float* __restrict__ proj,
                                                      uint8_t* __restrict__ present) {
  const int i = blockIdx.x * blockDim.x + threadIdx.x;
  if (i >= P) return;
  const float3 p = make_float3(means3D[3 * i], means3D[3 * i + 1], means3D[3 * i + 2]);
  const float z = view[2] * p.x + view[6] * p.y + view[10] * p.z + view[14];
  present[i] = z > GSR_NEAR_CULL ? 1 : 0;
  (void)proj;
}

void launch_mark_visible(int P, const float* means3D, const float* view, const float* proj,
                         uint8_t* present, hipStream_t stream) {
  if (P <= 0) return;
  hipLaunchKernelGGL(k_mark_visible, dim3((P + 255) / 256), dim3(256), 0, stream, P, means3D, view,
                     proj, present);
}

}
```

threestudio-3dgs_amd/csrc/gsr_common.h:

```cpp
#pragma once

#include <hip/hip_runtime.h>

#if !defined(GSR_DIAG_BUILD) &&                                                                          \
    (defined(GSR_EXP_COALROWS) || defined(GSR_EXP_FWD_NOC) || defined(GSR_EXP_LDSPAD) ||                  \
     defined(GSR_EXP_NOCULL) || defined(GSR_EXP_NOFLUSH) || defined(GSR_EXP_NOGROUP) ||                   \
     defined(GSR_EXP_NOMFMA) || defined(GSR_EXP_NOREACH) || defined(GSR_EXP_NOREPLAY) ||                \
     defined(GSR_EXP_NOCOL2) || defined(GSR_EXP_HOTREC) || defined(GSR_EXP_NOEMBED))
#error "GSR_EXP_* experiment switches build only through `make exp` (a diagnostic library, not libgsr_hip.so)"
#endif
#include <stddef.h>
#include <stdlib.h>
#include <string.h>
#include <stdint.h>

#define GSR_TILE_X 16
#define GSR_TILE_Y 16
#define GSR_TILE_PIX (GSR_TILE_X * GSR_TILE_Y)

#define GSR_SET_MAX 64
#define GSR_SORT_THREADS 256
#ifndef GSR_SORT_ITEMS
#define GSR_SORT_ITEMS 16
#endif
#define GSR_SORT_TILE (GSR_SORT_THREADS * GSR_SORT_ITEMS)
#define GSR_RADIX_BITS 8
#define GSR_RADIX (1 << GSR_RADIX_BITS)
#define GSR_GOFF_TILE 4096
#define GSR_DUP_TILE 64

#define GSR_NEAR_CULL 0.2f
#define GSR_ALPHA_MAX 0.99f
#define GSR_ALPHA_MIN (1.0f / 255.0f)
#define GSR_T_EPS 0.0001f

namespace gsr {


static inline size_t align_up(size_t x, size_t a) { return (x + a - 1) / a * a; }

struct Carver {
  char* base;
  size_t off;
  __host__ __device__ Carver(void* b) : base((char*)b), off(0) {}
  template <typename T>
  T* take(size_t count) {
    off = align_up(off, 256);
    T* p = (T*)(base ? base + off : nullptr);
    off += count * sizeof(T);
    return p;
  }
};

__host__ __device__ static inline int div_up(long long a, long long b) { return (int)((a + b - 1) / b); }

static inline int tile_key_bits(int W, int H) {
  const int tiles = div_up(W, GSR_TILE_X) * div_up(H, GSR_TILE_Y);
  int bits = 0;
  while ((1 << bits) < tiles) ++bits;
  return bits < 1 ? 1 : bits;
}

#define GSR_QMASK_SHIFT 28
struct TilePack {
  bool packed;
  bool qmask;
  int gbits, tile_bits;
  uint32_t gmask;
  uint32_t tmask;
};
static inline TilePack tile_pack(int P, int W, int H, int force_mode) {
  const bool force = force_mode != 0;
  TilePack t;
  t.tile_bits = tile_key_bits(W, H);
  int gb = 1;
  while (gb < 32 && (1ll << gb) < (long long)P) ++gb;
  t.packed = gb + t.tile_bits <= 32 && !force;
  t.gbits = t.packed ? gb : 0;
  t.gmask = t.packed ? (uint32_t)((1ull << gb) - 1ull) : 0xFFFFFFFFu;
  t.qmask = !t.packed && t.tile_bits <= GSR_QMASK_SHIFT && force_mode != 2;
  t.tmask = t.tile_bits >= 32 ? 0xFFFFFFFFu : (uint32_t)((1ull << t.tile_bits) - 1ull);
  return t;
}

struct DigitPlan {
  int passes, bits;
  __host__ __device__ int width(int p, int key_bits) const {
    const int lo = p * bits;
    return key_bits - lo < bits ? key_bits - lo : bits;
  }
};
static inline DigitPlan digit_plan(int key_bits, int max_bits = GSR_RADIX_BITS) {
  if (key_bits < 1) key_bits = 1;
  if (max_bits < 1 || max_bits > GSR_RADIX_BITS) max_bits = GSR_RADIX_BITS;
  DigitPlan d;
  d.passes = (key_bits + max_bits - 1) / max_bits;
  d.bits = (key_bits + d.passes - 1) / d.passes;
  return d;
}
struct SegInfo {
  int V, tile;
  uint32_t n[GSR_SET_MAX];
  uint32_t start[GSR_SET_MAX];
  uint32_t blk[GSR_SET_MAX + 1];
  const uint32_t* ndev = nullptr;
  const uint32_t* rebase = nullptr;
};
__device__ __forceinline__ uint32_t seg_live(const SegInfo& s, int v) {
  return s.ndev ? min(s.ndev[v], s.n[v]) : s.n[v];
}
__device__ __forceinline__ uint32_t seg_key_base(const SegInfo& s) { return s.rebase ? s.rebase[0] : 0u; }
__device__ __forceinline__ uint32_t seg_key(uint32_t kb, uint32_t key) {
  return key == 0xFFFFFFFFu ? key : key - kb;
}
__device__ __forceinline__ bool seg_skip_last(const SegInfo& s, int last) {
  return last && s.rebase != nullptr && s.rebase[1] != 0u;
}
static inline void seg_fill_blocks(SegInfo& s, int tile) {
  s.tile = tile;
  s.blk[0] = 0;
  for (int v = 0; v < s.V; ++v) s.blk[v + 1] = s.blk[v] + (uint32_t)div_up((long long)s.n[v], tile);
}
__device__ __forceinline__ uint32_t xcd_block(uint32_t b, uint32_t n) {
  const uint32_t x = b & 7u, q = n >> 3, r = n & 7u;
  return x * q + (x < r ? x : r) + (b >> 3);
}
__device__ __forceinline__ int seg_of_block(const SegInfo& s, uint32_t b, uint32_t& lb) {
  int lo = 0, hi = s.V;
  while (hi - lo > 1) {
    const int mid = (lo + hi) >> 1;
    if (s.blk[mid] <= b) lo = mid;
    else hi = mid;
  }
  lb = b - s.blk[lo];
  return lo;
}

struct ViewCam {
  const float *view, *proj, *campos;
  float tanx, tany;
  float fx, fy;
};
struct SetCams {
  ViewCam c[GSR_SET_MAX];
};

struct __attribute__((aligned(64))) GaussRec {
  float4 a, b, c;
  uint4 d;
};

struct GeomState {
  GaussRec* rec;
  uint2* tiles;
  uint32_t* dkey[2];
  uint32_t* dval[2];
  uint32_t* sort_counts;
  uint32_t* sort_totals;
  uint32_t* kept_counts;
  uint32_t* goff;
  uint32_t* goff_part;
  uint32_t* vis_part;
  int vbits;
  __host__ __device__ uint32_t vmask() const { return vbits >= 32 ? 0xFFFFFFFFu : (1u << vbits) - 1u; }
  __host__ __device__ uint32_t vsent() const { return vbits > 26 ? 0u : (1u << (32 - vbits)) - 1u; }
  uint32_t* drange;
  __device__ const uint32_t* sorted_dval() const { return drange[129] ? dval[1] : dval[0]; }
  __device__ const uint32_t* sorted_dkey() const { return drange[129] ? dkey[1] : dkey[0]; }
  uint32_t* counters;
  static int sort_blocks(int P) { return div_up(P > 0 ? P : 1, GSR_SORT_TILE); }
  static int dup_blocks(int P) { return div_up(P > 0 ? P : 1, GSR_DUP_TILE); }
  static int goff_blocks(int P) { return div_up(P > 0 ? P : 1, GSR_GOFF_TILE); }
  static GeomState carve(void* base, int V, int P, size_t* bytes) {
    Carver c(base);
    GeomState g;
    const size_t n = (size_t)(V > 0 ? V : 1) * (size_t)(P > 0 ? P : 1);
    const size_t nv = (size_t)(V > 0 ? V : 1);
    g.rec = c.take<GaussRec>(n);
    g.tiles = c.take<uint2>(n);
    g.dkey[0] = c.take<uint32_t>(n);
    g.dkey[1] = c.take<uint32_t>(n);
    g.dval[0] = c.take<uint32_t>(n);
    g.dval[1] = c.take<uint32_t>(n);
    g.sort_counts = c.take<uint32_t>(nv * GSR_RADIX * sort_blocks(P));
    g.sort_totals = c.take<uint32_t>(nv * GSR_RADIX);
    g.kept_counts = c.take<uint32_t>(nv * dup_blocks(P));
    g.counters = c.take<uint32_t>(3 * nv + 64);
    g.goff = c.take<uint32_t>(n);
    g.goff_part = c.take<uint32_t>(nv * goff_blocks(P));
    g.vis_part = c.take<uint32_t>(nv * goff_blocks(P));
    g.vbits = 1;
    while (g.vbits < 32 && (1ull << g.vbits) < (unsigned long long)(P > 1 ? P : 2)) ++g.vbits;
    g.drange = c.take<uint32_t>(132);
    if (bytes) *bytes = align_up(c.off, 256);
    return g;
  }
};

struct BinningState {
  uint32_t* key[2];
  uint32_t* val[2];
  uint32_t* sort_counts;
  uint32_t* sort_totals;
  static BinningState carve(void* base, int V, long long Ktot, long long sort_blocks, bool with_vals, size_t* bytes) {
    Carver c(base);
    BinningState b;
    const size_t n = (size_t)(Ktot > 0 ? Ktot : 1);
    b.key[0] = c.take<uint32_t>(n);
    b.key[1] = c.take<uint32_t>(n);
    b.val[0] = with_vals ? c.take<uint32_t>(n) : nullptr;
    b.val[1] = with_vals ? c.take<uint32_t>(n) : nullptr;
    b.sort_counts = c.take<uint32_t>((size_t)GSR_RADIX * (size_t)(sort_blocks > 0 ? sort_blocks : 1));
    b.sort_totals = c.take<uint32_t>((size_t)GSR_RADIX * (size_t)(V > 0 ? V : 1));
    if (bytes) *bytes = align_up(c.off, 256);
    return b;
  }
};

#define GSR_SPLIT_MAX_TILES 4096
#define GSR_SPLIT_CH 256
#define GSR_SPLIT_NCK 15
__host__ __device__ inline bool split_fits(int V, size_t tiles) {
  return V >= 1 && tiles > 0 && (size_t)V * tiles <= GSR_SPLIT_MAX_TILES;
}
__host__ __device__ inline int split_extra(int V, size_t tiles) {
  const size_t e = (size_t)V * tiles / 4;
  return e < 1024 ? 1024 : e > 4096 ? 4096 : (int)e;
}
#define GSR_CKPT_FIELDS 5
__host__ __device__ inline size_t ckpt_offset(size_t vg, size_t tiles, size_t tile, int k) {
  return ((vg * tiles + tile) * (GSR_SPLIT_NCK + 1) + (size_t)k) * GSR_CKPT_FIELDS * 256;
}

struct ImageState {
  uint2* ranges;
  uint32_t* quad_maxc;
  uint4* tile_info;
  uint2* cut;
  float* final_T;
  uint32_t* n_contrib;
  uint32_t* order;
  uint32_t* split_mode;
  uint32_t* split_items;
  uint32_t* split_cap;
  float* ckpt;
  static ImageState carve(void* base, int V, int W, int H, size_t* bytes, bool with_ckpt = true) {
    Carver c(base);
    ImageState s;
    const size_t nv = (size_t)(V > 0 ? V : 1);
    const size_t tiles = (size_t)div_up(W, GSR_TILE_X) * div_up(H, GSR_TILE_Y);
    const size_t pix = (size_t)W * H;
    s.split_mode = c.take<uint32_t>(2);
    s.ranges = c.take<uint2>(nv * (tiles > 0 ? tiles : 1));
    s.quad_maxc = c.take<uint32_t>(nv * 4 * (tiles > 0 ? tiles : 1));
    s.tile_info = c.take<uint4>(nv * (tiles > 0 ? tiles : 1));
    s.cut = c.take<uint2>(nv * (tiles > 0 ? tiles : 1));
    s.final_T = c.take<float>(nv * (pix > 0 ? pix : 1));
    s.n_contrib = c.take<uint32_t>(nv * (pix > 0 ? pix : 1));
    const size_t st = (size_t)((div_up(W, GSR_TILE_X) + 1) >> 1) * ((div_up(H, GSR_TILE_Y) + 1) >> 1);
    s.order = c.take<uint32_t>(nv * (st > 0 ? st : 1));
    const bool split = split_fits(V, tiles);
    s.split_items = c.take<uint32_t>(split ? 1 + (size_t)split_extra(V, tiles) : 1);
    s.split_cap = c.take<uint32_t>(split ? nv * tiles : 1);
    s.ckpt = c.take<float>(split && with_ckpt ? ckpt_offset(nv, tiles, 0, 0) : 1);
    if (bytes) *bytes = align_up(c.off, 256);
    return s;
  }
};

#define GSR_GRAD_FIELDS 14
#define GSR_GRAD_FIELDS2 17
#define GSR_REC_STRIDE 16
#define GSR_REC_STRIDE2 20
struct BackwardState {
  unsigned long long* reach;
  float4* grow;
  float* vrec;
  static size_t reach_bytes(int P) { return align_up(sizeof(unsigned long long) * (size_t)(P > 0 ? P : 1), 256); }
  static size_t rows_bytes(long long K, bool two = false) {
    return align_up(sizeof(float4) * (two ? 4 : 3) * (size_t)(K > 0 ? K : 1), 256);
  }
  static size_t bytes_for(long long K, int views, int P, bool two = false) {
    return reach_bytes(P) + rows_bytes(K, two) +
           align_up(sizeof(float) * (two ? GSR_REC_STRIDE2 : GSR_REC_STRIDE) * (size_t)views * (size_t)(P > 0 ? P : 1),
                    256);
  }
  static BackwardState carve(void* base, long long K, int P, bool two = false) {
    BackwardState s;
    s.reach = (unsigned long long*)base;
    s.grow = (float4*)((char*)base + reach_bytes(P));
    s.vrec = (float*)((char*)s.grow + rows_bytes(K, two));
    return s;
  }
};


__device__ __forceinline__ float xform_row(float m0, float m1, float m2, float m3, const float3 p) {
  return fmaf(m2, p.z, fmaf(m1, p.y, m0 * p.x)) + m3;
}
__device__ __forceinline__ float3 xform_point4x3(const float3 p, const float* m) {
  return make_float3(xform_row(m[0], m[4], m[8], m[12], p), xform_row(m[1], m[5], m[9], m[13], p),
                     xform_row(m[2], m[6], m[10], m[14], p));
}
__device__ __forceinline__ float4 xform_point4x4(const float3 p, const float* m) {
  return make_float4(xform_row(m[0], m[4], m[8], m[12], p), xform_row(m[1], m[5], m[9], m[13], p),
                     xform_row(m[2], m[6], m[10], m[14], p), xform_row(m[3], m[7], m[11], m[15], p));
}
__device__ __forceinline__ float3 xform_vec4x3_T(const float3 p, const float* m) {
  return make_float3(m[0] * p.x + m[1] * p.y + m[2] * p.z,
                     m[4] * p.x + m[5] * p.y + m[6] * p.z,
                     m[8] * p.x + m[9] * p.y + m[10] * p.z);
}
__device__ __forceinline__ float ndc2pix(float v, int S) {
  return (float)((((double)v + 1.0) * (double)S - 1.0) * 0.5);
}

__device__ __forceinline__ float fast_rcp(float x) { return __builtin_amdgcn_rcpf(x); }

__device__ __forceinline__ float gauss_power(float a, float b, float c, float dx, float dy) {
  float q = fmaf(c * dy, dy, (a * dx) * dx);
  return fmaf(-0.5f, q, -((b * dx) * dy));
}

#define GSR_CONIC_K_AC (-0.72134752044448170f)
#define GSR_CONIC_K_B (-1.4426950408889634f)
__device__ __forceinline__ float gauss_power2(float A, float B, float C, float dx, float dy) {
  return fmaf(dx, fmaf(A, dx, B * dy), (C * dy) * dy);
}

struct SpanPrep {
  float px, py, b, D, ia, thra, ue, ve;
  int mode;
};
__device__ __forceinline__ SpanPrep span_prep(float px, float py, float a, float b, float c, float o) {
#pragma clang fp contract(off)
  SpanPrep p;
  p.px = px;
  p.py = py;
  p.b = b;
  p.D = a * c - b * b;
  p.mode = !(o >= GSR_ALPHA_MIN * 0.9999f) ? 0 : !(a > 0.0f && c > 0.0f && p.D > 0.0f) ? 1 : 2;
  const float tau = fmaxf(0.0f, __logf(255.0f * o));
  const float thr = 2.0f * (tau * 1.002f + 2e-3f);
// ... 65 lines not shown
```

threestudio-3dgs_amd/csrc/gsr_kernels.h:

```cpp
#pragma once

#include "../../include/gsr.h"
#include "gsr_common.h"

namespace gsr {

int seg_sort(uint32_t* keys[2], uint32_t* vals[2], bool vals_identity, SegInfo seg, int bit_lo, int key_bits,
             uint32_t* counts, uint32_t* totals, hipStream_t stream, int max_bits = GSR_RADIX_BITS);
struct RunWork {
  uint32_t* keys[2];
  uint32_t* vals[2];
  uint32_t *counts, *totals;
  uint32_t* bounds;
  void carve(Carver& c, size_t items, size_t n, float** coef = nullptr) {
    for (int i = 0; i < 2; ++i) keys[i] = c.take<uint32_t>(items);
    for (int i = 0; i < 2; ++i) vals[i] = c.take<uint32_t>(items);
    if (coef) *coef = c.take<float>(items);
    counts = c.take<uint32_t>((size_t)GSR_RADIX * (size_t)div_up((long long)items, GSR_SORT_TILE));
    totals = c.take<uint32_t>((size_t)GSR_RADIX);
    bounds = c.take<uint32_t>(2 * n);
  }
};
int sort_runs(RunWork w, uint32_t n, int N, int* half, hipStream_t stream);
int sort_rank_mode();

struct PreprocessArgs {
  int V, P, deg, M;
  const float *means3D, *scales, *rotations, *opacities, *shs, *colors_precomp, *cov3D_precomp;
  float scale_modifier;
  int W, H;
  int* radii;
  const float* col2;
};
struct PreprocessTimed {
  size_t means, scales, rotations, col2;
};
void launch_preprocess(const PreprocessArgs& a, const SetCams& cams, const GeomState& g, hipStream_t stream,
                       const PreprocessTimed* timed = nullptr);

void launch_binning_counts(int V, int P, const GeomState& g, hipStream_t stream);
void launch_emit(int V, int P, int W, const GeomState& g, const SegInfo& inst, const TilePack& tp, uint32_t* keys,
                 uint32_t* vals, hipStream_t stream);
void launch_tile_ranges(SegInfo inst, int n_tiles, const TilePack& tp, const uint32_t* keys, uint2* ranges,
                        hipStream_t stream);
void launch_mark_visible(int P, const float* means3D, const float* view, const float* proj,
                         uint8_t* present, hipStream_t stream);

__device__ __forceinline__ float quad_form(float a, float b, float c, float u, float v) {
  return fmaf(a * u, u, fmaf(2.0f * b * u, v, c * v * v));
}
__device__ __forceinline__ bool quadrant_hit(const float4 r0, const float4 r1, float qx, float qy) {
  const float o = r1.y;
  if (!(o >= GSR_ALPHA_MIN * 0.9999f)) return false;
  const float a = r0.z, b = r0.w, c = r1.x;
  if (!(a > 0.0f && c > 0.0f && a * c - b * b > 0.0f)) return true;
  const float tau = fmaxf(0.0f, __logf(255.0f * o));
  const float thr = 2.0f * (tau * 1.002f + 2e-3f);
  const float u1 = r0.x - qx, u0 = u1 - 7.0f;
  const float v1 = r0.y - qy, v0 = v1 - 7.0f;
  if (u0 <= 0.0f && u1 >= 0.0f && v0 <= 0.0f && v1 >= 0.0f) return true;
  const float ia = 1.0f / a, ic = 1.0f / c;
  const float q0 = quad_form(a, b, c, u0, fminf(fmaxf(-b * u0 * ic, v0), v1));
  const float q1 = quad_form(a, b, c, u1, fminf(fmaxf(-b * u1 * ic, v0), v1));
  const float q2 = quad_form(a, b, c, fminf(fmaxf(-b * v0 * ia, u0), u1), v0);
  const float q3 = quad_form(a, b, c, fminf(fmaxf(-b * v1 * ia, u0), u1), v1);
  const float qmin = fminf(fminf(q0, q1), fminf(q2, q3));
  return qmin * 0.998f <= thr;
}

struct RenderSet {
  int V, v0, P, W, H, gx, gy;
  uint32_t gmask;
  uint32_t inst_start[GSR_SET_MAX];
  uint32_t row_start[GSR_SET_MAX];
  const float* bg[GSR_SET_MAX];
  const float* cbg;
  float* comp;
  const float* ccolor;
  float* dcbg;
  const float* col2;
  float* out_col2;
  const float* dpix2;
  const uint32_t* order;
  int ochunk;
  float* ckpt;
  const uint32_t* split_mode;
  const uint32_t* col2_rec;
  uint32_t* split_items;
  uint32_t* split_cap;
  int split_extra;
  const uint32_t* qkeys;
  uint8_t* qbytes;
};
bool split_on(int V, int P, int width, int height, long long instances);
bool fwd_tile_chosen(long long instances, long long gaussians, int views);
int order_chunk(int V, int gx, int gy, bool forward);
const char* blend_kernel_name(int which);
inline bool split_forward(int V, int P, int width, int height, long long instances, bool two_colors) {
  return !two_colors && split_on(V, P, width, height, instances);
}
void launch_tile_order(int V, int gx, int gy, const uint2* ranges, uint32_t* order, hipStream_t stream);
void launch_render_forward(const RenderSet& rs, const GeomState& g, const uint32_t* sorted_gauss,
                           const ImageState& img, float* out_color, float* out_depth, float* out_alpha,
                           long long instances, hipStream_t stream);
void launch_render_backward(const RenderSet& rs, const GeomState& g, const uint32_t* sorted_gauss,
                            const ImageState& img, const float* dL_dcolor, const float* dL_ddepth,
                            const float* dL_dalpha, const BackwardState& bw, hipStream_t stream);

struct GaussBackwardArgs {
  int P, deg, M;
  int g0, g1;
  const float *means3D, *scales, *rotations, *shs, *cov3D_precomp;
  float scale_modifier;
  float *dL_dcolors, *dL_dopacity, *dL_dmeans3D, *dL_dcov3D, *dL_dsh, *dL_dscales, *dL_drotations;
};
struct ViewGradArgs {
  int V, v0, W, H, gx, tiles, cut_in_lds, items;
  GeomState g;
  ImageState img;
  const unsigned long long* reach;
  const float4* grow;
  float* dmeans2D;
  float* vrec;
  uint32_t row_start[GSR_SET_MAX];
  ViewCam cam[GSR_SET_MAX];
};
struct AccumArgs {
  int V, v0, accumulate, pad_;
  const unsigned long long* reach;
  const float* vrec;
  float* dcov_carry;
  float* dcolors2;
  const float* campos[GSR_SET_MAX];
};
void launch_composite_fwd(int V, size_t HW, const float* color, const float* alpha, const float* bg, int layout,
                          float* out, hipStream_t stream);
void launch_composite_bwd(int V, size_t HW, const float* dout, const float* color, const float* alpha,
                          const float* bg, int layout, float* dcolor, float* dalpha, float* dbg,
                          hipStream_t stream);
void launch_normal_map_fwd(int V, size_t HW, const float* normal, const float* alpha, float* out, hipStream_t stream);
void launch_normal_map_bwd(int V, size_t HW, const float* dout, const float* normal, const float* alpha,
                           float* dnormal, float* dalpha, hipStream_t stream);
struct ShadeArgs {
  int V, v0, H, W, flags, bg_layout;
  const float* color;
  const float* depth;
  const float* alpha;
  const float* rays_o;
  const float* rays_d;
  const float* bg;
  const float* light;
  const float* pred_normal;
  float ka[GSR_SET_MAX][3], kd[GSR_SET_MAX][3];
  int mode[GSR_SET_MAX];
  float* render;
  float* nmap;
  float* unit;
  float* depth_out;
};
struct ShadeGrads {
  const float* d_render;
  const float* d_nmap;
  const float* d_unit;
  const float* d_depth_out;
  float* d_color;
  float* d_depth;
  float* d_alpha;
  float* d_bg;
};
void launch_shade_fwd(const ShadeArgs& A, hipStream_t stream);
void launch_shade_bwd(const ShadeArgs& A, const ShadeGrads& G, hipStream_t stream);
size_t knn_workspace_bytes(int P);
int launch_knn_mean_dist(int P, const float* points, float* out, void* workspace, hipStream_t stream);
int launch_knn_points(int P, int K, const float* points, float* dists, long long* idx, void* workspace,
                      hipStream_t stream);
using FieldCall = gsr_sugar_field;
size_t field_workspace_bytes(long long M, int K, int N);
int field_gauss_lanes(long long M, int K, int N);
void launch_field_forward(const FieldCall& c, float* density, float* beta_avg, float* op, void* workspace,
                          hipStream_t stream);
int launch_field_backward(const FieldCall& c, const float* g_density, const float* g_beta, const float* g_op, float* dx,
                          float* dcenters, float* dinv_sr, float* dstrengths, float* dmin_scale, void* workspace,
                          hipStream_t stream);
using NormalCall = gsr_sugar_normal;
size_t normal_workspace_bytes(long long M, int K, int N);
int normal_gauss_lanes(long long M, int K, int N);
void launch_normal_forward(const NormalCall& c, float* loss, float* rec, void* workspace, hipStream_t stream);
int launch_normal_backward(const NormalCall& c, const float* rec, const float* g_loss, float* dnormals,
                           void* workspace, hipStream_t stream);
using MeshCall = gsr_sugar_mesh;
size_t mesh_workspace_bytes(int F, int V);
// ... 60 lines not shown
```

threestudio-3dgs_amd/csrc/gsr_preprocess.hip:

```cpp
#include "gsr_kernels.h"
#include "gsr_math.h"

namespace gsr {

void launch_preprocess_kernel(const PreprocessArgs& a, const SetCams& cams, const GeomState& g, hipStream_t stream,
                              const PreprocessTimed* timed);

#ifndef GSR_PRE_VIEWS
#define GSR_PRE_VIEWS 64
#endif
#define GSR_PRE_GAUSS 128
#define GSR_PRE_LDS_FLOATS (8 * 1024)

template <bool SH_LDS, bool TIMED>
__device__ __forceinline__ void preprocess_body(const PreprocessArgs& a, const SetCams& cams, const GeomState& g,
                                                const PreprocessTimed& tv, float* s_sh) {
  const int nvc = (a.V + GSR_PRE_VIEWS - 1) / GSR_PRE_VIEWS;
  const int vc = blockIdx.x % nvc;
  const int idx0 = (blockIdx.x / nvc) * GSR_PRE_GAUSS;
  const int t = threadIdx.x;
  const int gl = t % GSR_PRE_GAUSS;
  const int half = __builtin_amdgcn_readfirstlane(t / GSR_PRE_GAUSS);
  const int idx = idx0 + gl;
  const int vb = vc * GSR_PRE_VIEWS, ve = min(a.V, vb + GSR_PRE_VIEWS);
  const int vh = (ve - vb + 1) / 2;
  const int v0 = vb + half * vh, v1 = half == 0 ? min(ve, vb + vh) : ve;
  const int nsh = a.colors_precomp == nullptr ? 3 * a.M : 0;
  const int sstride = nsh + 1;
  const bool staged = SH_LDS;
  if (staged) {
    const int n = min(GSR_PRE_GAUSS, a.P - idx0) * nsh;
    const float4* src = reinterpret_cast<const float4*>(a.shs + (size_t)idx0 * nsh);
    const float inv_nsh = 1.0f / (float)nsh;
    for (int e4 = t; e4 * 4 < n; e4 += 256) {
      const float4 q = src[e4];
      const float qv[4] = {q.x, q.y, q.z, q.w};
#pragma unroll
      for (int k = 0; k < 4; ++k) {
        const int e = 4 * e4 + k;
        const int r = (int)(((float)e + 0.5f) * inv_nsh);
        if (e < n) s_sh[r * sstride + (e - r * nsh)] = qv[k];
      }
    }
    __syncthreads();
  }
  const bool valid = idx < a.P;
  const int ix = valid ? idx : idx0;
  uint32_t kmn = 0xFFFFFFFFu, kmx = 0u;

  float3 p_orig = make_float3(0.f, 0.f, 0.f);
  if (!TIMED) p_orig = make_float3(a.means3D[3 * ix], a.means3D[3 * ix + 1], a.means3D[3 * ix + 2]);
  float cov3D[6];
  if (TIMED) {
#pragma unroll
    for (int i = 0; i < 6; ++i) cov3D[i] = 0.f;
  } else if (a.cov3D_precomp != nullptr) {
#pragma unroll
    for (int i = 0; i < 6; ++i) cov3D[i] = a.cov3D_precomp[6 * ix + i];
  } else {
    const float3 s = make_float3(a.scales[3 * ix], a.scales[3 * ix + 1], a.scales[3 * ix + 2]);
    const float4 q = make_float4(a.rotations[4 * ix], a.rotations[4 * ix + 1],
                                 a.rotations[4 * ix + 2], a.rotations[4 * ix + 3]);
    cov3d_from_scale_rot(s, a.scale_modifier, q, cov3D);
  }
  const float opacity = a.opacities[ix];
  float3 rgb_pre = make_float3(0.f, 0.f, 0.f);
  if (a.colors_precomp != nullptr)
    rgb_pre = make_float3(a.colors_precomp[3 * ix], a.colors_precomp[3 * ix + 1], a.colors_precomp[3 * ix + 2]);
  const float* my_sh = staged ? s_sh + gl * sstride : a.shs + (size_t)ix * nsh;
  float3 c2 = make_float3(0.f, 0.f, 0.f);
  if (!TIMED && a.col2 != nullptr) c2 = make_float3(a.col2[3 * ix], a.col2[3 * ix + 1], a.col2[3 * ix + 2]);
  const int gx = (a.W + GSR_TILE_X - 1) / GSR_TILE_X;
  const int gy = (a.H + GSR_TILE_Y - 1) / GSR_TILE_Y;

#pragma unroll 1
  for (int v = v0; v < v1; ++v) {
    const ViewCam cam = cams.c[v];
    const size_t vi = (size_t)v * a.P + idx;
    typedef __attribute__((address_space(4))) const float* cfptr;
    float viewmatrix[16], projmatrix[16], cpos[3];
#pragma unroll
    for (int i = 0; i < 16; ++i) viewmatrix[i] = ((cfptr)cam.view)[i], projmatrix[i] = ((cfptr)cam.proj)[i];
#pragma unroll
    for (int i = 0; i < 3; ++i) cpos[i] = ((cfptr)cam.campos)[i];
    const float tanfovx = cam.tanx, tanfovy = cam.tany;
    const float focal_x = cam.fx, focal_y = cam.fy;
    if (TIMED) {
      const float* m = a.means3D + (size_t)v * tv.means + 3 * (size_t)ix;
      const float* sv = a.scales + (size_t)v * tv.scales + 3 * (size_t)ix;
      const float* qv = a.rotations + (size_t)v * tv.rotations + 4 * (size_t)ix;
      p_orig = make_float3(m[0], m[1], m[2]);
      cov3d_from_scale_rot(make_float3(sv[0], sv[1], sv[2]), a.scale_modifier, make_float4(qv[0], qv[1], qv[2], qv[3]),
                           cov3D);
      if (a.col2 != nullptr) {
        const float* cv = a.col2 + (size_t)v * tv.col2 + 3 * (size_t)ix;
        c2 = make_float3(cv[0], cv[1], cv[2]);
      }
    }
    int radius = 0;
    uint2 tiles = make_uint2(0u, 0u);
    uint32_t dkey = 0xFFFFFFFFu;
    const float3 p_view = xform_point4x3(p_orig, viewmatrix);
    if (p_view.z > GSR_NEAR_CULL) {
      const float4 p_hom = xform_point4x4(p_orig, projmatrix);
      const float p_w = 1.0f / (p_hom.w + 0.0000001f);
      const float3 p_proj = make_float3(p_hom.x * p_w, p_hom.y * p_w, p_hom.z * p_w);
      Cov2DState st;
      const float3 cov = cov2d_ewa(p_orig, focal_x, focal_y, tanfovx, tanfovy, cov3D, viewmatrix, st);
      const float det = cov.x * cov.z - cov.y * cov.y;
      if (det != 0.0f) {
        const float det_inv = 1.f / det;
        const float3 conic = make_float3(cov.z * det_inv, -cov.y * det_inv, cov.x * det_inv);
        const float mid = 0.5f * (cov.x + cov.z);
        const float lambda1 = mid + sqrtf(fmaxf(0.1f, mid * mid - det));
        const float lambda2 = mid - sqrtf(fmaxf(0.1f, mid * mid - det));
        const float my_radius = ceilf(3.f * sqrtf(fmaxf(lambda1, lambda2)));
        const float2 pimg = make_float2(ndc2pix(p_proj.x, a.W), ndc2pix(p_proj.y, a.H));
        const int r = (int)my_radius;
        const int xmin = min(gx, max(0, (int)((pimg.x - r) / GSR_TILE_X)));
        const int ymin = min(gy, max(0, (int)((pimg.y - r) / GSR_TILE_Y)));
        const int xmax = min(gx, max(0, (int)((pimg.x + r + GSR_TILE_X - 1) / GSR_TILE_X)));
        const int ymax = min(gy, max(0, (int)((pimg.y + r + GSR_TILE_Y - 1) / GSR_TILE_Y)));
        const int area = (xmax - xmin) * (ymax - ymin);
        if (area != 0) {
          float3 rgb = rgb_pre;
          uint32_t clamp_bits = 0;
          if (a.colors_precomp == nullptr)
            rgb = sh_to_rgb(a.deg, my_sh, p_orig, make_float3(cpos[0], cpos[1], cpos[2]),
                            &clamp_bits);
          GaussRec rec;
          rec.a = make_float4(pimg.x, pimg.y, conic.x, conic.y);
          rec.b = make_float4(conic.z, opacity, p_view.z, c2.x);
          rec.c = make_float4(rgb.x, rgb.y, rgb.z, c2.y);
          rec.d = make_uint4((uint32_t)xmin | ((uint32_t)ymin << 16), (uint32_t)xmax | ((uint32_t)ymax << 16),
                             __float_as_uint(c2.z), clamp_bits);
          if (valid) g.rec[vi] = rec;
          radius = r;
          uint32_t kept = 0;
          const SpanPrep sp = span_prep(rec.a.x, rec.a.y, rec.a.z, rec.a.w, rec.b.x, rec.b.y);
          for (int ty = ymin; ty < ymax; ++ty) {
            int t0, t1;
            span_row(sp, ty, xmin, xmax, t0, t1);
            kept += (uint32_t)(t1 - t0);
          }
          tiles = make_uint2((uint32_t)area, kept);
          dkey = __float_as_uint(p_view.z);
        }
      }
    }
    if (valid) {
      a.radii[vi] = radius;
      g.tiles[vi] = tiles;
      g.dkey[0][vi] = dkey;
      const uint32_t ks = g.vsent();
      g.dval[0][vi] = (uint32_t)idx | (g.vbits <= 26 ? min(tiles.y, ks) << g.vbits : 0u);
      if (dkey != 0xFFFFFFFFu) kmn = min(kmn, dkey), kmx = max(kmx, dkey);
    }
  }
  __shared__ uint32_t s_rng[2][4];
#pragma unroll
  for (int o = 32; o > 0; o >>= 1) {
    kmn = min(kmn, (uint32_t)__shfl_xor((int)kmn, o, 64));
    kmx = max(kmx, (uint32_t)__shfl_xor((int)kmx, o, 64));
  }
  if ((t & 63) == 0) s_rng[0][t >> 6] = kmn, s_rng[1][t >> 6] = kmx;
  __syncthreads();
  if (t == 0) {
    kmn = min(min(s_rng[0][0], s_rng[0][1]), min(s_rng[0][2], s_rng[0][3]));
    kmx = max(max(s_rng[1][0], s_rng[1][1]), max(s_rng[1][2], s_rng[1][3]));
    if (kmn != 0xFFFFFFFFu) {
      atomicMin(&g.drange[blockIdx.x & 63], kmn);
      atomicMax(&g.drange[64 + (blockIdx.x & 63)], kmx);
    }
  }
}

template <bool SH_LDS>
__attribute__((amdgpu_waves_per_eu(6, 8)))
__global__ __launch_bounds__(256) void k_preprocess(PreprocessArgs a, SetCams cams, GeomState g) {
  extern __shared__ float s_sh[];
  preprocess_body<SH_LDS, false>(a, cams, g, PreprocessTimed{0, 0, 0, 0}, s_sh);
}

__attribute__((amdgpu_waves_per_eu(6, 8)))
__global__ __launch_bounds__(256) void k_preprocess_timed(PreprocessArgs a, SetCams cams, GeomState g,
                                                          PreprocessTimed tv) {
  preprocess_body<false, true>(a, cams, g, tv, nullptr);
}

__global__ void k_depth_range_init(uint32_t* drange, unsigned long long col2) {
  drange[threadIdx.x] = 0xFFFFFFFFu;
  drange[64 + threadIdx.x] = 0u;
  if (threadIdx.x < 2) drange[130 + threadIdx.x] = (uint32_t)(col2 >> (32 * threadIdx.x));
}

__global__ void k_depth_range(uint32_t* drange) {
  const int t = threadIdx.x;
  uint32_t mn = drange[t], mx = drange[64 + t];
#pragma unroll
  for (int o = 32; o > 0; o >>= 1) {
    mn = min(mn, (uint32_t)__shfl_xor((int)mn, o, 64));
    mx = max(mx, (uint32_t)__shfl_xor((int)mx, o, 64));
  }
  if (t == 0) {
    const bool any = mn != 0xFFFFFFFFu;
    drange[128] = any ? mn : 0u;
    drange[129] = (!any || mx - mn < 0x00FFFFFFu) ? 1u : 0u;
  }
}

void launch_preprocess(const PreprocessArgs& a, const SetCams& cams, const GeomState& g, hipStream_t stream,
                       const PreprocessTimed* timed) {
  hipLaunchKernelGGL(k_depth_range_init, dim3(1), dim3(64), 0, stream, g.drange,
                     (unsigned long long)(uintptr_t)(a.P > 0 ? a.col2 : nullptr));
  if (a.P > 0 && a.V > 0) launch_preprocess_kernel(a, cams, g, stream, timed);
  hipLaunchKernelGGL(k_depth_range, dim3(1), dim3(64), 0, stream, g.drange);
}

void launch_preprocess_kernel(const PreprocessArgs& a, const SetCams& cams, const GeomState& g, hipStream_t stream,
                              const PreprocessTimed* timed) {
  const int nvc = (a.V + GSR_PRE_VIEWS - 1) / GSR_PRE_VIEWS;
  if (timed != nullptr) {
    hipLaunchKernelGGL(k_preprocess_timed, dim3(nvc * ((a.P + GSR_PRE_GAUSS - 1) / GSR_PRE_GAUSS)), dim3(256), 0,
                       stream, a, cams, g, *timed);
    return;
  }
  const size_t want = a.colors_precomp == nullptr ? (size_t)GSR_PRE_GAUSS * (3 * a.M + 1) : 0;
  const bool sh_lds = a.colors_precomp == nullptr && a.M > 0 && want <= GSR_PRE_LDS_FLOATS;
  const size_t lds = sh_lds ? sizeof(float) * want : 0;
  hipLaunchKernelGGL(sh_lds ? k_preprocess<true> : k_preprocess<false>,
                     dim3(nvc * ((a.P + GSR_PRE_GAUSS - 1) / GSR_PRE_GAUSS)), dim3(256), lds, stream, a, cams, g);
}

}
```

threestudio-3dgs_amd/csrc/gsr_render.hip:

```cpp
#include <cstdlib>
#include <cstring>

#include "gsr_kernels.h"
#include "gsr_wave.h"

#ifndef GSR_FWD_PREFETCH
#define GSR_FWD_PREFETCH 1
#endif
#ifndef GSR_FWD_WPE
#define GSR_FWD_WPE 1
#endif
#ifndef GSR_BWD_OVERLAP
#define GSR_BWD_OVERLAP 1
#endif

namespace gsr {

#ifdef GSR_TIMELINE
#define GSR_TL_MAX 65536
__device__ uint4 g_timeline[2][GSR_TL_MAX];
__device__ unsigned long long g_pairs[8];
#define GSR_TL_BEGIN const uint32_t tl_t0 = (uint32_t)__builtin_amdgcn_s_memrealtime();
#define GSR_TL_END(which, work)                                                                  \
  if (threadIdx.x == 0 && blockIdx.x < GSR_TL_MAX)                                                \
// ... 587 lines not shown
        float p0 = CrCg[q].x + Tq * bg[0], p1 = CrCg[q].y + Tq * bg[1], p2 = CbD[q].x + Tq * bg[2];
        if (rs.cbg != nullptr) {
          const float am = 1.0f - (1.0f - Tq);
          const float* bgi = rs.cbg + ((size_t)v * HWs + pid) * 3;
          p0 = p0 + am * bgi[0];
          p1 = p1 + am * bgi[1];
          p2 = p2 + am * bgi[2];
        }
        float* cp = rs.comp + (size_t)v * 3 * HWs + pid;
        cp[0] = fminf(fmaxf(p0, 0.0f), 1.0f);
        cp[HWs] = fminf(fmaxf(p1, 0.0f), 1.0f);
        cp[2 * HWs] = fminf(fmaxf(p2, 0.0f), 1.0f);
      }
    }
    uint32_t mc = last[q];
#pragma unroll
    for (int o = 32; o > 0; o >>= 1) mc = max(mc, (uint32_t)__shfl_xor((int)mc, o, 64));
    if (lane == 0) quad_maxc[4 * tile + q] = mc;
  }
#ifdef GSR_TIMELINE
  atomicAdd(&g_pairs[0], pc_eval);
  atomicAdd(&g_pairs[1], pc_slot);
#endif
}

__global__ __launch_bounds__(256) void k_tile_order(int gx, int gy, const uint2* __restrict__ ranges,
                                                    uint32_t* __restrict__ order) {
  __shared__ uint32_t cnt[33], cur[33];
  const int t = threadIdx.x, v = blockIdx.x;
  const int sgx = (gx + 1) >> 1, sgy = (gy + 1) >> 1, S = sgx * sgy;
  ranges += (size_t)v * gx * gy;
  order += (size_t)v * S;
  if (t < 33) cnt[t] = 0u;
  __syncthreads();
  auto bucket = [&](int s) -> int {
    const int x0 = (s % sgx) * 2, y0 = (s / sgx) * 2;
    uint32_t w = 0u;
#pragma unroll
    for (int k = 0; k < 4; ++k) {
      const int x = x0 + (k & 1), y = y0 + (k >> 1);
      if (x < gx && y < gy) {
        const uint2 r = ranges[y * gx + x];
        w += r.y - r.x;
      }
    }
    return 32 - (w ? 32 - __clz((int)w) : 0);
  };
  for (int s = t; s < S; s += 256) atomicAdd(&cnt[bucket(s)], 1u);
  __syncthreads();
  if (t == 0) {
    uint32_t run = 0u;
    for (int b = 0; b < 33; ++b) {
      cur[b] = run;
      run += cnt[b];
    }
  }
  __syncthreads();
  for (int s = t; s < S; s += 256) order[atomicAdd(&cur[bucket(s)], 1u)] = (uint32_t)s;
}

void launch_tile_order(int V, int gx, int gy, const uint2* ranges, uint32_t* order, hipStream_t stream) {
  if (V > 0 && gx > 0 && gy > 0) hipLaunchKernelGGL(k_tile_order, dim3(V), dim3(256), 0, stream, gx, gy, ranges, order);
}


__global__ __launch_bounds__(256) void k_ckpt_suffix(RenderSet rs, const uint32_t* __restrict__ quad_maxc) {
  const int tiles = rs.gx * rs.gy;
  const int v = blockIdx.x / tiles, tile = blockIdx.x % tiles;
  const int t = threadIdx.x, q = t >> 6;
  const size_t vg = (size_t)(rs.v0 + v);
  const int qmaxc = (int)quad_maxc[(vg * tiles + tile) * 4 + q];
  const int cl = qmaxc > 0 ? min(GSR_SPLIT_NCK, (qmaxc - 1) / GSR_SPLIT_CH) : 0;
  if (t == 0) {
    const uint4 qm = reinterpret_cast<const uint4*>(quad_maxc)[vg * tiles + tile];
    const int maxc = (int)max(max(qm.x, qm.y), max(qm.z, qm.w));
    const int nc = maxc > 0 ? min(GSR_SPLIT_NCK, (maxc - 1) / GSR_SPLIT_CH) : 0;
    uint32_t cap = 0xffffffffu;
    if (nc > 0) {
      const uint32_t at = atomicAdd(rs.split_items, (uint32_t)nc);
      const uint32_t E = (uint32_t)rs.split_extra;
      const int m = (int)min((uint32_t)nc, at < E ? E - at : 0u);
      for (int j = 0; j < m; ++j)
        rs.split_items[1 + at + j] = ((uint32_t)vg << 26) | ((uint32_t)(nc - j) << 22) | (uint32_t)tile;
      if (m > 0) cap = (uint32_t)(nc - m + 1) * GSR_SPLIT_CH;
    }
    rs.split_cap[vg * tiles + tile] = cap;
  }
  if (cl < 2) return;
  float4* const part = reinterpret_cast<float4*>(rs.ckpt + ckpt_offset(vg, (size_t)tiles, tile, 0) + 256) + t;
  constexpr size_t SL = GSR_CKPT_FIELDS * 256 / 4;
  float4 p[GSR_SPLIT_NCK + 1];
#pragma unroll
  for (int j = 1; j <= GSR_SPLIT_NCK; ++j) p[j] = part[(size_t)min(j, cl) * SL];
  float4 acc = p[GSR_SPLIT_NCK];
#pragma unroll
  for (int j = GSR_SPLIT_NCK - 1; j >= 1; --j) {
    if (j < cl) {
      acc = make_float4(p[j].x + acc.x, p[j].y + acc.y, p[j].z + acc.z, p[j].w + acc.w);
      part[(size_t)j * SL] = acc;
    } else if (j == cl) {
      acc = p[j];
    }
  }
}

static bool fwd_tile_kernel(long long instances, long long gaussians, int views) {
  const char* e = getenv("GSR_FWD_KERNEL");
  if (e != nullptr && strcmp(e, "quadrant") == 0) return false;
  if (e != nullptr && strcmp(e, "tile") == 0) return true;
  return views >= 16 && gaussians > 0 && instances >= 3 * gaussians;
}
bool fwd_tile_chosen(long long instances, long long gaussians, int views) {
  return fwd_tile_kernel(instances, gaussians, views);
}

static const char* g_blend_kernel[2] = {"", ""};
const char* blend_kernel_name(int which) { return which >= 0 && which < 2 ? g_blend_kernel[which] : ""; }

void launch_render_forward(const RenderSet& rs, const GeomState& g, const uint32_t* sorted_gauss,
                           const ImageState& img, float* out_color, float* out_depth, float* out_alpha,
                           long long instances, hipStream_t stream) {
  const int nt = rs.gx * rs.gy;
  if (nt <= 0 || rs.V <= 0) return;
  if (fwd_tile_kernel(instances, (long long)rs.V * rs.P, rs.V)) {
    const dim3 grid(block_grid(rs, 4));
    g_blend_kernel[0] = rs.col2 != nullptr ? "k_render_fwd_tile<true>" : "k_render_fwd_tile<false>";
    if (rs.col2 != nullptr)
      hipLaunchKernelGGL(k_render_fwd_tile<true>, grid, dim3(64), 0, stream, rs, (const uint2*)img.ranges,
                         sorted_gauss, (const GaussRec*)g.rec, out_color, out_depth, out_alpha, img.final_T,
                         img.n_contrib, img.quad_maxc);
    else
      hipLaunchKernelGGL(k_render_fwd_tile<false>, grid, dim3(64), 0, stream, rs, (const uint2*)img.ranges,
                         sorted_gauss, (const GaussRec*)g.rec, out_color, out_depth, out_alpha, img.final_T,
                         img.n_contrib, img.quad_maxc);
  } else {
    auto kern = rs.col2 != nullptr ? (rs.ckpt != nullptr ? k_render_fwd<true, true> : k_render_fwd<true, false>)
                                   : (rs.ckpt != nullptr ? k_render_fwd<false, true> : k_render_fwd<false, false>);
    g_blend_kernel[0] = rs.col2 != nullptr ? (rs.ckpt != nullptr ? "k_render_fwd<true, true>" : "k_render_fwd<true, false>")
                                           : (rs.ckpt != nullptr ? "k_render_fwd<false, true>" : "k_render_fwd<false, false>");
    hipLaunchKernelGGL(kern, dim3(block_grid(rs, 16)), dim3(64), 0, stream, rs, (const uint2*)img.ranges,
                       sorted_gauss, (const GaussRec*)g.rec, out_color, out_depth, out_alpha, img.final_T,
                       img.n_contrib, img.quad_maxc);
    if (rs.ckpt != nullptr)
      hipLaunchKernelGGL(k_ckpt_suffix, dim3(rs.V * nt), dim3(256), 0, stream, rs, (const uint32_t*)img.quad_maxc);
  }
  hipLaunchKernelGGL(k_tile_info, dim3(rs.V * div_up(nt, 256)), dim3(256), 0, stream, rs,
                     (const uint2*)img.ranges, (const uint32_t*)img.quad_maxc, sorted_gauss,
                     (const GaussRec*)g.rec, img.tile_info, img.cut);
}

__device__ __forceinline__ void bwd_tile(BwdLDS& s, const RenderSet& rs, int v, int tile, int chunk, bool split,
                                         const uint2* __restrict__ ranges, const uint32_t* __restrict__ quad_maxc,
                                         const uint32_t* __restrict__ sorted_gauss, const GaussRec* __restrict__ rec,
                                         const uint32_t* __restrict__ goff, const float* __restrict__ final_Ts,
                                         const uint32_t* __restrict__ n_contrib, const float* __restrict__ dL_dcolor,
                                         const float* __restrict__ dL_ddepth, const float* __restrict__ dL_dalpha,
                                         float4* __restrict__ grow, unsigned long long* __restrict__ reach) {
  constexpr int NG = NGV;
  constexpr int QS = GSR_QSUM_STRIDE;
  constexpr int GS = 8;
  constexpr int NPL = 4;
  constexpr int RW = 3;
  GSR_TL_BEGIN
  const int W = rs.W, H = rs.H, grid_x = rs.gx;
  const size_t vgs = (size_t)(rs.v0 + v);
  {
    const size_t vg = vgs, tiles = (size_t)rs.gx * rs.gy, HWs = (size_t)W * H;
    ranges += vg * tiles;
    quad_maxc += vg * 4 * tiles;
    sorted_gauss += rs.inst_start[v];
    rec += vg * rs.P;
    goff += vg * rs.P;
    final_Ts += vg * HWs;
    n_contrib += vg * HWs;
    dL_dcolor += (size_t)v * 3 * HWs;
    if (dL_ddepth) dL_ddepth += (size_t)v * HWs;
    if (dL_dalpha) dL_dalpha += (size_t)v * HWs;
    grow += (size_t)RW * rs.row_start[v];
  }
  const float* bg = rs.bg[v];
  int tl_work = 0, tl_max = 0;
  int tl_q[4] = {0, 0, 0, 0};
  int tl_staged = 0, tl_any = 0;
  const int t = threadIdx.x, q = __builtin_amdgcn_readfirstlane(t >> 6), lane = t & 63;
  const int txi = tile % grid_x, tyi = tile / grid_x;
  const int qx0 = txi * GSR_TILE_X + (q & 1) * 8;
  const int qy0 = tyi * GSR_TILE_Y + (q >> 1) * 8;
  const int px = qx0 + (lane & 7), py = qy0 + (lane >> 3);
  const bool inside = px < W && py < H;
  const float pxf = (float)px, pyf = (float)py;
  const uint2 range = ranges[tile];
  const uint4 qm = reinterpret_cast<const uint4*>(quad_maxc)[tile];
  const int qmaxc = (int)(q == 0 ? qm.x : q == 1 ? qm.y : q == 2 ? qm.z : qm.w);
  const int maxc = (int)max(max(qm.x, qm.y), max(qm.z, qm.w));
  int lo = 0, hi = maxc;
  if (split) {
    lo = chunk * GSR_SPLIT_CH;
    if (chunk == 0)
      hi = (int)min((uint32_t)maxc, rs.split_cap[vgs * rs.gx * rs.gy + tile]);
    else
      hi = chunk == GSR_SPLIT_NCK ? maxc : min(maxc, lo + GSR_SPLIT_CH);
  }
  lo = __builtin_amdgcn_readfirstlane(lo);
  hi = __builtin_amdgcn_readfirstlane(hi);
  const size_t pid = (size_t)py * W + px;
  const size_t HW = (size_t)H * W;

  const float T_final = inside ? final_Ts[pid] : 0.0f;
  float T = T_final;
  const uint32_t last_contributor = inside ? n_contrib[pid] : 0u;
  float dpix[3] = {0.f, 0.f, 0.f};
  float dpix_d = 0.f, dpix_a = 0.f;
  if (inside) {
    dpix[0] = dL_dcolor[pid];
    dpix[1] = dL_dcolor[HW + pid];
    dpix[2] = dL_dcolor[2 * HW + pid];
    if (dL_ddepth) dpix_d = dL_ddepth[pid];
    if (dL_dalpha) dpix_a = dL_dalpha[pid];
    if (rs.cbg != nullptr) {
#pragma clang fp contract(off)
      const float am = 1.0f - (1.0f - T_final);
      const float* bgi = rs.cbg + ((size_t)v * HW + pid) * 3;
      const float* col = rs.ccolor + (size_t)v * 3 * HW + pid;
      float da = 0.0f;
#pragma unroll
      for (int ch = 0; ch < 3; ++ch) {
        const float b = bgi[ch];
        const float pre = col[(size_t)ch * HW] + am * b;
        const float gch = (pre >= 0.0f && pre <= 1.0f) ? dpix[ch] : 0.0f;
        dpix[ch] = gch;
        da -= gch * b;
        if (rs.dcbg != nullptr && chunk == 0) rs.dcbg[((size_t)v * HW + pid) * 3 + ch] = gch * am;
      }
      dpix_a = da + dpix_a;
    } else if (rs.ccolor != nullptr) {
      const float* col = rs.ccolor + (size_t)v * 3 * HW + pid;
#pragma unroll
      for (int ch = 0; ch < 3; ++ch) {
        const float pre = col[(size_t)ch * HW];
        dpix[ch] = (pre >= 0.0f && pre <= 1.0f) ? dpix[ch] : 0.0f;
      }
    }
  }
  const float bg_dot = bg_dot3(bg, dpix[0], dpix[1], dpix[2]);

  float S = 0.f, Sd = 0.f;
  const float nbg = -T_final * bg_dot;
  const f2 pxy = {pxf, pyf};
  if (split && hi < maxc && qmaxc > hi) {
    const size_t tiles = (size_t)rs.gx * rs.gy;
    const float* ck = rs.ckpt + ckpt_offset(vgs, tiles, tile, hi / GSR_SPLIT_CH);
    const float Th = ck[t];
    const float4 b4 = reinterpret_cast<const float4*>(ck + 256)[t];
    const float br = b4.x, bgc = b4.y, bb = b4.z, bd = b4.w;
    const float inv = 1.0f / Th;
    T = Th;
    S = (br * dpix[0] + bgc * dpix[1] + bb * dpix[2]) * inv + (1.0f - T_final * inv) * dpix_a;
    Sd = bd * inv;
  }
  const float ddelx_dx = sgpr_f(0.5f * W), ddely_dy = sgpr_f(0.5f * H);
  const float4 zero4 = make_float4(0.f, 0.f, 0.f, 0.f);

  const uint32_t gmask = rs.gmask;
  const int cs = t >> 2, piece = t & 3;
  auto fetch_raw = [&](int h) -> uint32_t {
    const int r = h - 1 - cs;
    return r >= 0 ? sorted_gauss[range.x + r] : 0u;
  };
  auto fetch_index = [&](int h) -> uint32_t { return fetch_raw(h) & gmask; };
  float4 npc = zero4;
  uint32_t ngo = 0u;
  uint32_t gi_next = 0u;
  unsigned int* const reach32 = reinterpret_cast<unsigned int*>(reach) + (v >> 5);
  const unsigned int vbit = 1u << (v & 31);
  const uint32_t qlayout = rs.qbytes != nullptr && rs.split_mode != nullptr ? (rs.split_mode[1] & 0xffu) : 0u;
  const size_t qpos0 = (size_t)rs.inst_start[v] + range.x;
  const uint8_t* const qbm = qlayout == 0u ? nullptr : qlayout == 1u ? rs.qbytes + qpos0 : rs.qbytes + 4 * qpos0 + q;
  const uint32_t qstride = qlayout == 2u ? 4u : 1u, qsh = qlayout == 2u ? 0u : (uint32_t)q;
  uint32_t nqb = 0u;
  if (qbm != nullptr && hi - 1 - lane >= lo) nqb = qbm[qstride * (uint32_t)(hi - 1 - lane)];
  if (hi > lo) {
    const uint32_t g0 = fetch_index(hi);
    if (hi - 1 - cs >= lo) {
#ifdef GSR_EXP_HOTREC
      npc = reinterpret_cast<const float4*>(rec + (g0 & 4095u))[piece];
#else
      npc = reinterpret_cast<const float4*>(rec + g0)[piece];
#endif
      if (piece == 2 && rs.col2 != nullptr)
        npc = make_float4(rs.col2[3 * g0], rs.col2[3 * g0 + 1], rs.col2[3 * g0 + 2], 0.f);
      if (piece == 2) ngo = g0;
      if (piece == 3) ngo = goff[g0];
    }
    if (hi - 64 > lo) gi_next = fetch_raw(hi - 64);
  }

  f2 SS = {S, Sd};
  f2 TT = {0.f, T};
  auto replay = [&](const float4& ga, const float4& gb, const float4& gc, float& u, float& w) {
    const uint32_t rel = __float_as_uint(gb.w);
    const f2 dd = f2{ga.x, ga.y} - pxy;
    const f2 bcp = f2{ga.z, ga.w} * f2{dd.y, dd.y};
    const float power2 = fmaf(dd.x, fmaf(gb.x, dd.x, bcp.x), bcp.y * dd.y);
    const float G = __builtin_amdgcn_exp2f(power2);
    const float alpha = fminf(GSR_ALPHA_MAX, gb.y * G);
    const bool hit = rel < last_contributor && power2 <= 0.0f && alpha >= GSR_ALPHA_MIN;
    const f2 ga2 = {hit ? G : 0.0f, hit ? alpha : 0.0f};
    const float a_eff = ga2.y;
    const float oma = 1.f - a_eff;
    const float inv_1ma = fast_rcp(oma);
    TT.y = TT.y * inv_1ma;
    const float cd = fmaf(gc.x, dpix[0], fmaf(gc.y, dpix[1], fmaf(gc.z, dpix[2], dpix_a)));
    TT.x = fmaf(TT.y, fmaf(gb.z - SS.y, dpix_d, cd - SS.x), inv_1ma * nbg);
    const f2 uw2 = ga2 * TT;
    u = uw2.x;
    w = uw2.y;
    const f2 om = f2{oma, oma} * SS;
    SS.x = fmaf(a_eff, cd, om.x);
    SS.y = fmaf(a_eff, gb.z, om.y);
  };


  const int ncol = lane & 15;
  const bool dcol = ncol >= 6 && ncol < 6 + NPL;
  float fa[2], fbb[2], fc;
#pragma unroll
  for (int h = 0; h < 2; ++h) {
    const float y = (float)(2 * (lane >> 4) + h) - 3.5f;
    fa[h] = ncol == 0 ? 1.f : ncol == 2 ? y : ncol == 5 ? y * y : 0.f;
    fbb[h] = ncol == 1 ? 1.f : ncol == 4 ? y : 0.f;
  }
  fc = ncol == 3 ? 1.f : 0.f;
  float bv[16];
  {
    float* sdp = s.qsum + q * (NPL * 68 + 16);
    sdp[0 * 68 + lane] = dpix[0];
    sdp[1 * 68 + lane] = dpix[1];
    sdp[2 * 68 + lane] = dpix[2];
    sdp[3 * 68 + lane] = dpix_d;
    if (lane < 16) sdp[NPL * 68 + lane] = 0.f;
    asm volatile("s_waitcnt lgkmcnt(0)" ::: "memory");
    const float4* dsrc =
        reinterpret_cast<const float4*>(sdp + (dcol ? (ncol - 6) * 68 + 16 * (lane >> 4) : NPL * 68));
#pragma unroll
    for (int k = 0; k < 4; ++k) {
      const float4 d4 = dsrc[k];
      const float dk[4] = {d4.x, d4.y, d4.z, d4.w};
#pragma unroll
      for (int e = 0; e < 4; ++e) {
        const int i = 4 * k + e;
        const float x = (float)(i & 7) - 3.5f;
        bv[i] = dk[e] + (fa[i >> 3] + x * (fbb[i >> 3] + x * fc));
      }
    }
  }
  float* uw = s.uw[q];
  int wa[4];
#pragma unroll
  for (int sgrp = 0; sgrp < 4; ++sgrp)
    wa[sgrp] = gsr_uw_pg(lane >> 4) + 4 * (((lane >> 2) & 3) ^ sgrp) + (lane & 3);
  const float4* asrc = reinterpret_cast<const float4*>(uw + 16 * (lane & 15) + gsr_uw_pg(lane >> 4));
  const int aswz = (lane >> 2) & 3;
  const int mb = 4 * ((lane >> 4) & 1);
  const bool useful = (lane < 32) ? (ncol < 6) : dcol;
  const int field = ncol;

  uint32_t* mylist = s.list[q];
  float* myq = s.qsum + q * NG;

  float4 rowv = zero4;
  float4* rowp = nullptr;
  auto flush = [&](int hb) {
    rowp = nullptr;
#ifdef GSR_EXP_NOFLUSH
    if (hi < 0)
#else
    if (hb - 1 - cs >= lo)
#endif
    {
      int qq = piece;
      asm volatile("" : "+v"(qq));
      const float4 ga = s.s0[cs];
      const float4 gb = s.s1[cs];
      constexpr int NM = NGV;
      float m[NM];
#pragma unroll
      for (int i = 0; i < NM; ++i) m[i] = 0.f;
      if ((s.kmask[qq] >> cs) & 1ull) {
        const float* C = s.qsum + cs * QS + NG * qq;
        const float mx = ga.x - ((float)(txi * GSR_TILE_X + (qq & 1) * 8) + 3.5f);
        const float my = ga.y - ((float)(tyi * GSR_TILE_Y + (qq >> 1) * 8) + 3.5f);
        m[0] = C[0];
        m[1] = mx * C[0] - C[1];
        m[2] = my * C[0] - C[2];
        m[3] = mx * (mx * C[0] - 2.f * C[1]) + C[3];
        m[4] = mx * (my * C[0] - C[2]) - my * C[1] + C[4];
        m[5] = my * (my * C[0] - 2.f * C[2]) + C[5];
        m[6] = C[6];
        m[7] = C[7];
        m[8] = C[8];
        m[9] = C[9];
      }
#pragma unroll
      for (int i = 0; i < NM; ++i) {
        m[i] += dpp_f32<0xB1>(m[i]);
        m[i] += dpp_f32<0x4E>(m[i]);
      }
      const float o = gb.y;
#ifdef GSR_EXP_COALROWS
      float4* row = grow + RW * ((size_t)blockIdx.x * 64 + cs);
#else
      float4* row = grow + RW * (size_t)s.slot[cs];
#endif
      const float k = o * (1.0f / 1.4426950408889634f);
      if (qq == 0) {
        const float dmx = mean_grad(k, ddelx_dx, gb.x, ga.z, m[1], m[2]);
        const float dmy = mean_grad(k, ddely_dy, ga.w, ga.z, m[2], m[1]);
        rowv = make_float4(dmx, dmy, -0.5f * o * m[3], -0.5f * o * m[4]);
        rowp = row;
      } else if (qq == 1) {
        rowv = make_float4(-0.5f * o * m[5], m[0], m[6], m[7]);
        rowp = row + 1;
      } else if (qq == 2) {
        rowv = make_float4(m[8], m[9], 0.f, 0.f);
        rowp = row + 2;
      }
    }
  };

  for (int h = hi; h > lo; h -= 64) {
    asm volatile("s_waitcnt vmcnt(0)" ::: "memory");
    if (h != hi) flush(h + 64);
    uint32_t qcur;
    asm volatile("v_mov_b32 %0, %1" : "=v"(qcur) : "v"(nqb));
    const uint32_t gnx = gi_next & gmask;
    const float conic_a = __builtin_bit_cast(float, __builtin_amdgcn_mov_dpp(__builtin_bit_cast(int, npc.z), 0x00, 0xf, 0xf, false));
    const float conic_c = __builtin_bit_cast(float, __builtin_amdgcn_mov_dpp(__builtin_bit_cast(int, npc.x), 0x55, 0xf, 0xf, false));
    {
      const int rel_c = h - 1 - cs;
      int cst = cs;
      asm volatile("" : "+v"(cst));
      if (rel_c >= lo) {
        if (piece == 0) {
          s.s0[cst] = make_float4(npc.x, npc.y, GSR_CONIC_K_B * npc.w, GSR_CONIC_K_AC * conic_c);
        } else if (piece == 1) {
          s.s1[cst] = make_float4(GSR_CONIC_K_AC * conic_a, npc.y, npc.z, __uint_as_float((uint32_t)rel_c));
        } else if (piece == 2) {
          s.s2[cst] = npc;
          s.gidx[cst] = ngo;
        } else {
          const uint32_t dx_ = __float_as_uint(npc.x), dy_ = __float_as_uint(npc.y);
          const int xmin = dx_ & 0xffff, ymin = dx_ >> 16, xmax = dy_ & 0xffff;
          s.slot[cst] = ngo + (uint32_t)((tyi - ymin) * (xmax - xmin) + (txi - xmin));
        }
      }
      if (rowp != nullptr) *rowp = rowv;
      if (h - 64 > lo) {
        if (h - 65 - cs >= lo) {
#ifdef GSR_EXP_HOTREC
          npc = *reinterpret_cast<const float4*>(reinterpret_cast<const char*>(rec) + (((gnx & 4095u) * 4u + piece) << 4));
#else
          npc = *reinterpret_cast<const float4*>(reinterpret_cast<const char*>(rec) + ((gnx * 4u + (uint32_t)piece) << 4));
#endif
          if (piece == 2 && rs.col2 != nullptr)
            npc = make_float4(rs.col2[3 * gnx], rs.col2[3 * gnx + 1], rs.col2[3 * gnx + 2], 0.f);
          if (piece == 2) ngo = gnx;
          if (piece == 3) ngo = goff[gnx];
        }
        if (h - 128 > lo) gi_next = fetch_raw(h - 128);
      }
    }
    __syncthreads();
    const int rel_l = h - 1 - lane;
    bool keep = false;
#ifdef GSR_EXP_NOCULL
    if (rel_l >= lo && rel_l < qmaxc) keep = s.s0[lane].x > -1e30f;
#else
    keep = rel_l >= lo && rel_l < qmaxc && (qbm == nullptr || ((qcur >> qsh) & 1u));
#endif
    if (qbm != nullptr && h - 65 - lane >= lo) nqb = qbm[qstride * (uint32_t)(h - 65 - lane)];
    const unsigned long long bal = __ballot(keep);
    const int cnt = __popcll(bal);
    if (lane == 0) s.kmask[q] = bal;
#ifndef GSR_EXP_NOREACH
    if (qlayout == 1u ? (q == 0 && rel_l >= lo && (qcur & 0xfu) != 0u) : keep) {
      uint32_t vb;
      asm volatile("v_mov_b32 %0, %1" : "=v"(vb) : "s"(vbit));
      atomicOr(reach32 + 2 * s.gidx[lane], vb);
    }
#endif
#ifdef GSR_TIMELINE
    if (lane == 0) s.tl_cnt[q] = cnt;
#endif
    if (keep) mylist[mask_rank(bal)] = (uint32_t)lane * (uint32_t)QS;
    GSR_WAVE_LDS_ORDER();
    unsigned long long rest = bal;
#ifdef GSR_EXP_NOGROUP
    if (cnt < 0)
#endif
    for (int g0 = 0; g0 < cnt; g0 += GS) {
      const int gn = min(GS, cnt - g0);
      if (gn == GS) {
        int jj[GS];
#pragma unroll
        for (int c = 0; c < GS; ++c) {
          jj[c] = (int)__builtin_ctzll(rest);
          rest &= rest - 1ull;
        }
        float4 ca = s.s0[jj[0]], cb = s.s1[jj[0]], cc = s.s2[jj[0]];
#pragma unroll
        for (int c = 0; c < GS; ++c) {
          float4 na, nb, nc;
          if (c + 1 < GS) {
            na = s.s0[jj[c + 1]], nb = s.s1[jj[c + 1]], nc = s.s2[jj[c + 1]];
            asm volatile("" ::: "memory");
          }
          float u, w;
          replay(ca, cb, cc, u, w);
          uw[16 * c + wa[c >> 2]] = u;
          uw[16 * (c + 8) + wa[2 + (c >> 2)]] = w;
          if ((c & (GSR_BWD_OVERLAP - 1)) == GSR_BWD_OVERLAP - 1) __builtin_amdgcn_sched_barrier(0);
          if (c + 1 < GS) {
            ca = na;
            cb = nb;
            cc = nc;
          }
        }
      } else {
      int jj[GS];
#pragma unroll
      for (int c = 0; c < GS; ++c) {
        jj[c] = (int)__builtin_ctzll(rest | (1ull << 63));
        rest &= rest - 1ull;
      }
      float4 ca = s.s0[jj[0]], cb = s.s1[jj[0]], cc = s.s2[jj[0]];
#pragma unroll
      for (int c = 0; c < GS; ++c) {
        if (c < gn) {
          const bool more = c + 1 < gn;
          float4 na, nb, nc;
          if (more) {
            na = s.s0[jj[c + 1]], nb = s.s1[jj[c + 1]], nc = s.s2[jj[c + 1]];
            asm volatile("" ::: "memory");
          }
          float u, w;
#ifdef GSR_EXP_NOREPLAY
          u = ca.x * pxf;
          w = cb.x * pyf;
#else
          replay(ca, cb, cc, u, w);
#endif
          uw[16 * c + wa[c >> 2]] = u;
          uw[16 * (c + 8) + wa[2 + (c >> 2)]] = w;
          if (more) {
            ca = na;
            cb = nb;
            cc = nc;
          }
        }
      }
      }
      GSR_WAVE_LDS_ORDER();
#ifdef GSR_EXP_NOMFMA
      continue;
#endif
      float av[16];
#pragma unroll
      for (int k = 0; k < 4; ++k) {
        const float4 a4 = asrc[k ^ aswz];
        av[4 * k] = a4.x, av[4 * k + 1] = a4.y, av[4 * k + 2] = a4.z, av[4 * k + 3] = a4.w;
      }
      const uint4 jl = *reinterpret_cast<const uint4*>(mylist + g0 + mb);
      typedef float f4 __attribute__((ext_vector_type(4)));
      f4 acc0 = {0.f, 0.f, 0.f, 0.f}, acc1 = {0.f, 0.f, 0.f, 0.f};
#pragma unroll
      for (int i = 0; i < 16; ++i) {
        if (i & 1)
          acc1 = __builtin_amdgcn_mfma_f32_16x16x4f32(av[i], bv[i], acc1, 0, 0, 0);
        else
          acc0 = __builtin_amdgcn_mfma_f32_16x16x4f32(av[i], bv[i], acc0, 0, 0, 0);
      }
      if (useful) {
        const uint32_t jr[4] = {jl.x, jl.y, jl.z, jl.w};
        if (gn == GS) {
#pragma unroll
          for (int r = 0; r < 4; ++r) myq[jr[r] + (uint32_t)field] = acc0[r] + acc1[r];
        } else {
#pragma unroll
          for (int r = 0; r < 4; ++r)
            myq[mb + r < gn ? jr[r] + (uint32_t)field : (uint32_t)(QS - 1 - NG * q)] = acc0[r] + acc1[r];
        }
      }
      GSR_WAVE_LDS_ORDER();
    }
    __syncthreads();
#ifdef GSR_TIMELINE
    if (t == 0) {
      const int c0 = s.tl_cnt[0], c1 = s.tl_cnt[1], c2 = s.tl_cnt[2], c3 = s.tl_cnt[3];
      tl_work += c0 + c1 + c2 + c3;
      tl_max += 4 * max(max(c0, c1), max(c2, c3));
      tl_q[0] += c0, tl_q[1] += c1, tl_q[2] += c2, tl_q[3] += c3;
      tl_staged += min(h - lo, 64);
      tl_any += __popcll(s.kmask[0] | s.kmask[1] | s.kmask[2] | s.kmask[3]);
    }
#endif
  }
  if (hi > lo) {
    flush(lo + ((hi - lo - 1) & 63) + 1);
    if (rowp != nullptr) *rowp = rowv;
  }
#ifdef GSR_TIMELINE
  if (threadIdx.x == 0) {
    atomicAdd(&g_pairs[2], 64ull * (unsigned long long)tl_work);
    atomicAdd(&g_pairs[3], 64ull * (unsigned long long)tl_max);
    atomicAdd(&g_pairs[4], 256ull * (unsigned long long)max(max(tl_q[0], tl_q[1]), max(tl_q[2], tl_q[3])));
    atomicAdd(&g_pairs[5], (unsigned long long)tl_staged);
    atomicAdd(&g_pairs[6], (unsigned long long)tl_any);
  }
  if (threadIdx.x == 0 && blockIdx.x < GSR_TL_MAX)
    g_timeline[1][blockIdx.x] = make_uint4(tl_t0, (uint32_t)__builtin_amdgcn_s_memrealtime(), (uint32_t)tl_max,
                                           ((uint32_t)__builtin_amdgcn_s_getreg((15 << 11) | 20) << 24) |
                                               ((uint32_t)tl_work & 0xffffffu));
#endif
  (void)tl_work;
  (void)tl_max;
  (void)tl_q;
  (void)tl_staged;
  (void)tl_any;
}

__global__ __launch_bounds__(256) __attribute__((amdgpu_waves_per_eu(5, 8))) void k_render_bwd(
    RenderSet rs, const uint2* __restrict__ ranges, const uint32_t* __restrict__ quad_maxc,
    const uint32_t* __restrict__ sorted_gauss, const GaussRec* __restrict__ rec, const uint32_t* __restrict__ goff,
    const float* __restrict__ final_Ts, const uint32_t* __restrict__ n_contrib, const float* __restrict__ dL_dcolor,
    const float* __restrict__ dL_ddepth, const float* __restrict__ dL_dalpha, float4* __restrict__ grow,
    unsigned long long* __restrict__ reach, int extra, const uint32_t* __restrict__ items) {
  __shared__ BwdLDS s;
  static_assert(sizeof(BwdLDS) <= GSR_BWD_LDS_5WG, "backward blend: 5 workgroups per CU");
  int v, tile, chunk = 0;
  const bool split = rs.ckpt != nullptr && *rs.split_mode != 0u;
  if ((int)blockIdx.x < extra) {
    if (!split || blockIdx.x >= items[0]) return;
    const uint32_t it = items[1 + blockIdx.x];
    v = (int)(it >> 26) - rs.v0;
    if (v < 0 || v >= rs.V) return;
    tile = (int)(it & 0x3fffffu);
    chunk = (int)((it >> 22) & 15u);
  } else {
    int q_unused;
    if (!block_map<4>((int)blockIdx.x - extra, rs, v, tile, q_unused)) return;
  }
  v = __builtin_amdgcn_readfirstlane(v);
  tile = __builtin_amdgcn_readfirstlane(tile);
  chunk = __builtin_amdgcn_readfirstlane(chunk);
  bwd_tile(s, rs, v, tile, chunk, split, ranges, quad_maxc, sorted_gauss, rec, goff, final_Ts,
                n_contrib, dL_dcolor, dL_ddepth, dL_dalpha, grow, reach);
}

#define GSR_HCAP_TW 256
template <bool TWO>
__global__ __launch_bounds__(64) void k_render_bwd_tw(
    RenderSet rs, const uint2* __restrict__ ranges, const uint32_t* __restrict__ quad_maxc,
    const uint32_t* __restrict__ sorted_gauss, const GaussRec* __restrict__ rec, const uint32_t* __restrict__ goff,
    const float* __restrict__ final_Ts, const uint32_t* __restrict__ n_contrib, const float* __restrict__ dL_dcolor,
    const float* __restrict__ dL_ddepth, const float* __restrict__ dL_dalpha, float4* __restrict__ grow,
    unsigned long long* __restrict__ reach) {
  constexpr int NG = TWO ? NGV2 : NGV;
  constexpr int NM = TWO ? 15 : NGV;
  constexpr int RW = TWO ? 4 : 3;
  constexpr int NQ = 4;
  __shared__ float4 s0[65], s1[65], s2[65];
  __shared__ float4 s3[65];
  __shared__ uint32_t slot[64];
  __shared__ uint32_t list[64];
  __shared__ float4 hits[GSR_HCAP_TW];
  __shared__ float4 planes[TWO ? 128 : 64];
  int v, tile, q_unused;
  if (!block_map<4>(blockIdx.x, rs, v, tile, q_unused)) return;
  GSR_TL_BEGIN
  const int W = rs.W, H = rs.H, grid_x = rs.gx;
  const size_t vgs = (size_t)(rs.v0 + v);
  const size_t HW = (size_t)H * W;
  {
    const size_t tiles = (size_t)rs.gx * rs.gy;
    ranges += vgs * tiles;
    quad_maxc += vgs * 4 * tiles;
    sorted_gauss += rs.inst_start[v];
    rec += vgs * rs.P;
    goff += vgs * rs.P;
    final_Ts += vgs * HW;
    n_contrib += vgs * HW;
    dL_dcolor += (size_t)v * 3 * HW;
    if (dL_ddepth) dL_ddepth += (size_t)v * HW;
    if (dL_dalpha) dL_dalpha += (size_t)v * HW;
    grow += (size_t)RW * rs.row_start[v];
  }
  const float* bg = rs.bg[v];
  const int lane = threadIdx.x & 63;
  constexpr int qb = 0;
  const int txi = tile % grid_x, tyi = tile / grid_x;
  const uint2 range = ranges[tile];
  const uint4 qm = reinterpret_cast<const uint4*>(quad_maxc)[tile];
  const int qmaxc[4] = {(int)qm.x, (int)qm.y, (int)qm.z, (int)qm.w};
  const int hi = __builtin_amdgcn_readfirstlane((int)max(max(qm.x, qm.y), max(qm.z, qm.w)));
  const int lo = 0;

  float T[NQ], Sd[NQ], dpd[NQ];
  f2 de0[NQ], de1[NQ], de2[NQ], dpa0[NQ], nbgs[NQ], SS2[NQ];
  uint32_t last[NQ];
  const float lxf = (float)(txi * GSR_TILE_X + (lane & 7)), lyf = (float)(tyi * GSR_TILE_Y + (lane >> 3));
#pragma unroll
  for (int j = 0; j < NQ; ++j) {
    const int q = qb + j;
    const int px = txi * GSR_TILE_X + (q & 1) * 8 + (lane & 7), py = tyi * GSR_TILE_Y + (q >> 1) * 8 + (lane >> 3);
    const bool inside = px < W && py < H;
    const size_t pid = (size_t)py * W + px;
    const float T_final = inside ? final_Ts[pid] : 0.0f;
    T[j] = T_final;
    last[j] = inside ? n_contrib[pid] : 0u;
    float d[3] = {0.f, 0.f, 0.f};
    float dd = 0.f, da = 0.f;
    if (inside) {
      d[0] = dL_dcolor[pid];
      d[1] = dL_dcolor[HW + pid];
      d[2] = dL_dcolor[2 * HW + pid];
      if (dL_ddepth) dd = dL_ddepth[pid];
      if (dL_dalpha) da = dL_dalpha[pid];
      if (rs.cbg != nullptr) {
#pragma clang fp contract(off)
        const float am = 1.0f - (1.0f - T_final);
        const float* bgi = rs.cbg + ((size_t)v * HW + pid) * 3;
        const float* col = rs.ccolor + (size_t)v * 3 * HW + pid;
        float dsum = 0.0f;
#pragma unroll
        for (int ch = 0; ch < 3; ++ch) {
          const float b = bgi[ch];
          const float pre = col[(size_t)ch * HW] + am * b;
          const float gch = (pre >= 0.0f && pre <= 1.0f) ? d[ch] : 0.0f;
          d[ch] = gch;
          dsum -= gch * b;
          if (rs.dcbg != nullptr) rs.dcbg[((size_t)v * HW + pid) * 3 + ch] = gch * am;
        }
        da = dsum + da;
      } else if (rs.ccolor != nullptr) {
        const float* col = rs.ccolor + (size_t)v * 3 * HW + pid;
#pragma unroll
        for (int ch = 0; ch < 3; ++ch) {
          const float pre = col[(size_t)ch * HW];
          d[ch] = (pre >= 0.0f && pre <= 1.0f) ? d[ch] : 0.0f;
        }
      }
    }
    float e[3] = {0.f, 0.f, 0.f};
    if (TWO && inside) {
      const float* d2 = rs.dpix2 + (size_t)v * 3 * HW;
      e[0] = d2[pid];
      e[1] = d2[HW + pid];
      e[2] = d2[2 * HW + pid];
    }
    de0[j] = f2{d[0], e[0]};
    de1[j] = f2{d[1], e[1]};
    de2[j] = f2{d[2], e[2]};
    dpd[j] = dd;
    dpa0[j] = f2{da, -0.0f};
    nbgs[j] = f2{-T_final * bg_dot3(bg, d[0], d[1], d[2]), TWO ? -T_final * bg_dot3(bg, e[0], e[1], e[2]) : 0.f};
    SS2[j] = f2{0.f, 0.f};
    Sd[j] = 0.f;
  }
  const float ddelx_dx = 0.5f * W, ddely_dy = 0.5f * H;
  const float4 zero4 = make_float4(0.f, 0.f, 0.f, 0.f);

  const uint32_t gmask = rs.gmask;
  unsigned int* const reach32 = reinterpret_cast<unsigned int*>(reach) + (v >> 5);
  const unsigned int vbit = 1u << (v & 31);
  float4 na = zero4, nb = zero4, nc = zero4, nd = zero4, n2 = zero4;
  uint32_t ngo = 0u, gi_next = 0u, ng = 0u;
  const bool emb = col2_embedded(rs);
  auto load = [&](uint32_t g) {
    const float4* r = reinterpret_cast<const float4*>(rec + g);
    {
      na = r[0];
      nb = r[1];
      nd = r[3];
      ngo = goff[g];
      ng = g;
    }
    {
      nc = r[2];
      if (rs.col2 != nullptr && !(TWO && emb)) {
        const float4 c2 = make_float4(rs.col2[3 * g], rs.col2[3 * g + 1], rs.col2[3 * g + 2], 0.f);
        if (TWO)
          n2 = c2;
        else
          nc = c2;
      }
    }
  };
  const uint32_t qlayout = rs.qbytes != nullptr && rs.split_mode != nullptr ? (rs.split_mode[1] & 0xffu) : 0u;
  const uint8_t* const qbm = qlayout != 0u ? rs.qbytes + (qlayout == 2u ? 4 : 1) * ((size_t)rs.inst_start[v] + range.x)
                                           : nullptr;
  const uint32_t* qkeys = qbm == nullptr && rs.qkeys ? rs.qkeys + rs.inst_start[v] + range.x : nullptr;
  auto cull_raw = [&](int pos) -> uint32_t {
    if (qlayout == 2u) return reinterpret_cast<const uint32_t*>(qbm)[pos];
    if (qlayout == 1u) return qbm[pos];
    return qkeys[pos];
  };
  auto cull_decode = [&](uint32_t b) -> uint32_t {
    if (qlayout == 2u) return (b & 1u) | ((b >> 7) & 2u) | ((b >> 14) & 4u) | ((b >> 21) & 8u);
    if (qlayout == 1u) return b;
    return b >> GSR_QMASK_SHIFT;
  };
  const bool masks = qbm != nullptr || qkeys != nullptr;
  uint32_t nqm = 0u, qm_next = 0u;
  if (hi > lo) {
    if (hi - 1 - lane >= lo) {
      load(sorted_gauss[range.x + hi - 1 - lane] & gmask);
      if (masks) nqm = cull_decode(cull_raw(hi - 1 - lane));
    }
    if (hi - 64 > lo) {
      gi_next = sorted_gauss[range.x + max(hi - 65 - lane, lo)];
      if (masks) qm_next = cull_raw(max(hi - 65 - lane, lo));
    }
  }

  float acc[NM], accb[NM];
  auto pair_moments = [&](const int qq, const uint32_t e, float (&m)[NM]) {
    const int st = (int)(e & 0xffffu), n = (int)(e >> 16);
    const float4 ga = s0[lane];
    const float qx0 = (float)(txi * GSR_TILE_X + (qq & 1) * 8), qy0 = (float)(tyi * GSR_TILE_Y + (qq >> 1) * 8);
    float C[NG];
#pragma unroll
    for (int f = 0; f < NG; ++f) C[f] = 0.f;
    for (int k = st; k < st + n; ++k) {
      const float4 hv = hits[k];
      const uint32_t p = __float_as_uint(hv.w);
      const float dx = ga.x - (qx0 + (float)(p & 7u)), dy = ga.y - (qy0 + (float)(p >> 3));
      const float u = hv.x, w = hv.z;
      C[0] += u;
      C[1] = fmaf(u, dx, C[1]);
      C[2] = fmaf(u, dy, C[2]);
      C[3] = fmaf(u, dx * dx, C[3]);
      C[4] = fmaf(u, dx * dy, C[4]);
      C[5] = fmaf(u, dy * dy, C[5]);
      const float4 d = planes[TWO ? 2 * p : p];
      C[6] = fmaf(w, d.x, C[6]);
      C[7] = fmaf(w, d.y, C[7]);
      C[8] = fmaf(w, d.z, C[8]);
      C[9] = fmaf(w, d.w, C[9]);
      if constexpr (TWO) {
        const float u1 = hv.y;
        const float4 d2 = planes[2 * p + 1];
        C[10 % NG] += u1;
        C[11 % NG] = fmaf(u1, dx, C[11 % NG]);
        C[12 % NG] = fmaf(u1, dy, C[12 % NG]);
        C[13 % NG] = fmaf(w, d2.x, C[13 % NG]);
        C[14 % NG] = fmaf(w, d2.y, C[14 % NG]);
        C[15 % NG] = fmaf(w, d2.z, C[15 % NG]);
      }
    }
#pragma unroll
    for (int f = 0; f < 10; ++f) m[f] = C[f];
    if (TWO) {
      m[10 % NM] = C[11 % NG];
      m[11 % NM] = C[12 % NG];
      m[12 % NM] = C[13 % NG];
      m[13 % NM] = C[14 % NG];
      m[14 % NM] = C[15 % NG];
    }
  };
  auto flush = [&](const int j, const unsigned long long pend) {
    if (!((pend >> lane) & 1ull)) return;
    float m[NM];
    pair_moments(qb + j, list[lane], m);
#pragma unroll
    for (int i = 0; i < NM; ++i) {
      if (j == 0) acc[i] = m[i];
      else if (j == 1) acc[i] = acc[i] + m[i];
      else if (j == 2) accb[i] = m[i];
      else accb[i] = accb[i] + m[i];
    }
  };

  float4 rv[RW];
  uint32_t rslot = 0u;
  auto make_row = [&]() {
    float m[NM];
#pragma unroll
    for (int i = 0; i < NM; ++i) m[i] = acc[i] + accb[i];
    const float4 ga = s0[lane];
    const float4 gb = s1[lane];
    const float o = gb.y;
    rslot = slot[lane];
    const float k = o * (1.0f / 1.4426950408889634f);
    {
      const float dmx = mean_grad(k, ddelx_dx, gb.x, ga.z, m[1], m[2]);
      const float dmy = mean_grad(k, ddely_dy, ga.w, ga.z, m[2], m[1]);
      rv[0] = make_float4(dmx, dmy, -0.5f * o * m[3], -0.5f * o * m[4]);
    }
    rv[1] = make_float4(-0.5f * o * m[5], m[0], m[6], m[7]);
    rv[2] = TWO ? make_float4(m[8], m[9], m[12 % NM], m[13 % NM]) : make_float4(m[8], m[9], 0.f, 0.f);
    if (TWO) {
      const float dmx1 = mean_grad(k, ddelx_dx, gb.x, ga.z, m[10 % NM], m[11 % NM]);
      const float dmy1 = mean_grad(k, ddely_dy, ga.w, ga.z, m[11 % NM], m[10 % NM]);
      rv[RW - 1] = make_float4(m[14 % NM], dmx1, dmy1, 0.f);
    }
  };
  auto store_row = [&]() {
    float4* row = grow + RW * (size_t)rslot;
#pragma unroll
    for (int i = 0; i < RW; ++i) row[i] = rv[i];
  };
  for (int h = hi; h > lo; h -= 64) {
    asm volatile("s_waitcnt vmcnt(0)" ::: "memory");
    const bool row_pending = h != hi && h + 63 - lane >= lo;
    if (row_pending) make_row();
    const float4 ca = make_float4(vcopy(na.x), vcopy(na.y), vcopy(na.z), vcopy(na.w));
    const float4 cb = make_float4(vcopy(nb.x), vcopy(nb.y), vcopy(nb.z), 0.f);
    const float4 cc = make_float4(vcopy(nc.x), vcopy(nc.y), vcopy(nc.z), 0.f);
    const float4 c2 = !TWO ? zero4
                      : emb ? make_float4(vcopy(nb.w), vcopy(nc.w), vcopy(nd.z), 0.f)
                            : make_float4(vcopy(n2.x), vcopy(n2.y), vcopy(n2.z), 0.f);
    const uint32_t cdx = __float_as_uint(vcopy(nd.x)), cdy = __float_as_uint(vcopy(nd.y));
    const uint32_t cgo = __float_as_uint(vcopy(__uint_as_float(ngo)));
    const int rel_c = h - 1 - lane;
    const bool staged = rel_c >= lo;
    uint32_t keep4 = 0u;
    if (staged) {
      s0[lane] = make_float4(ca.x, ca.y, GSR_CONIC_K_B * ca.w, GSR_CONIC_K_AC * cb.x);
      s1[lane] = make_float4(GSR_CONIC_K_AC * ca.z, cb.y, cb.z, __uint_as_float((uint32_t)rel_c));
      const int xmin = cdx & 0xffff, ymin = cdx >> 16, xmax = cdy & 0xffff;
      slot[lane] = cgo + (uint32_t)((tyi - ymin) * (xmax - xmin) + (txi - xmin));
      if (masks) {
#pragma unroll
        for (int q = 0; q < 4; ++q) keep4 |= rel_c < qmaxc[q] ? nqm & (1u << q) : 0u;
      } else {
#pragma unroll
        for (int q = 0; q < 4; ++q)
          if (rel_c < qmaxc[q] &&
              quadrant_hit(ca, cb, (float)(txi * GSR_TILE_X + (q & 1) * 8), (float)(tyi * GSR_TILE_Y + (q >> 1) * 8)))
            keep4 |= 1u << q;
      }
    }
    if (staged) {
      s2[lane] = make_float4(cc.x, c2.x, cc.y, c2.y);
      s3[lane] = make_float4(cc.z, c2.z, 0.f, 0.f);
    }
    uint32_t g_next = gi_next & gmask;
    nqm = cull_decode(qm_next);
    asm volatile("" : "+v"(g_next), "+v"(nqm)::"memory");
#ifndef GSR_EXP_NOREACH
    if (staged && keep4 != 0u) atomicOr(reach32 + 2 * ng, vbit);
#endif
    if (row_pending) store_row();
    if (h - 64 > lo) {
      load(g_next);
      const int pn = max(h - 129 - lane, lo);
      gi_next = sorted_gauss[range.x + pn];
      if (masks) qm_next = cull_raw(pn);
    }
#pragma unroll
    for (int i = 0; i < NM; ++i) acc[i] = 0.f;
#pragma unroll
    for (int i = 0; i < NM; ++i) accb[i] = 0.f;
    __syncthreads();
#pragma unroll
    for (int j = 0; j < NQ; ++j) {
      const int q = qb + j;
      const unsigned long long kq = __ballot((keep4 >> q) & 1u);
      if (kq == 0ull) continue;
      planes[TWO ? 2 * lane : lane] = make_float4(de0[j].x, de1[j].x, de2[j].x, dpd[j]);
      if (TWO) planes[2 * lane + 1] = make_float4(de0[j].y, de1[j].y, de2[j].y, 0.f);
      const f2 pxy = {lxf + (float)((q & 1) * 8), lyf + (float)((q >> 1) * 8)};
      int fill = 0;
      unsigned long long pend = 0ull, rest = kq;
      int jc = (int)__builtin_ctzll(rest);
      float4 pa = s0[jc], pb = s1[jc], pc = s2[jc];
      float4 pd = s3[jc];
      float4 ya, yb, yc, yd;
      auto step = [&](const float4& ga, const float4& gb, const float4& gc, const float4& gd, float4& xa, float4& xb,
                      float4& xc, float4& xd) -> bool {
        rest &= rest - 1ull;
        const int jn = rest != 0ull ? (int)__builtin_ctzll(rest) : jc;
        xa = s0[jn], xb = s1[jn], xc = s2[jn];
        xd = s3[jn];
        const uint32_t rel = __float_as_uint(gb.w);
        const f2 dd = f2{ga.x, ga.y} - pxy;
        const f2 bc = f2{ga.z, ga.w} * f2{dd.y, dd.y};
        const float power2 = fmaf(dd.x, fmaf(gb.x, dd.x, bc.x), bc.y * dd.y);
        const float G = __builtin_amdgcn_exp2f(power2);
        const float alpha = fminf(GSR_ALPHA_MAX, gb.y * G);
        const unsigned long long hm = (__ballot(rel < last[j]) & __ballot(power2 <= 0.0f)) & __ballot(alpha >= GSR_ALPHA_MIN);
        const bool hit = (hm >> lane) & 1ull;
        const float a_eff = vsel(hm, alpha, 0.0f);
        const float g_eff = vsel(hm, G, 0.0f);
        const float oma = 1.f - a_eff;
        const float inv_1ma = fast_rcp(oma);
        T[j] = T[j] * inv_1ma;
        f2 cdp = __builtin_elementwise_fma(f2{gd.x, gd.y}, de2[j], dpa0[j]);
        cdp = __builtin_elementwise_fma(f2{gc.z, gc.w}, de1[j], cdp);
        cdp = __builtin_elementwise_fma(f2{gc.x, gc.y}, de0[j], cdp);
        const f2 dif = cdp - SS2[j];
        const f2 ibg = f2{inv_1ma, inv_1ma} * nbgs[j];
        float u, u1 = 0.f;
        if (TWO) {
          u1 = g_eff * fmaf(T[j], fmaf(gb.z - Sd[j], dpd[j], dif.x), ibg.x);
          u = fmaf(g_eff, fmaf(T[j], dif.y, ibg.y), u1);
        } else {
          u = g_eff * fmaf(T[j], fmaf(gb.z - Sd[j], dpd[j], dif.x), ibg.x);
        }
        const float w = a_eff * T[j];
        SS2[j] = __builtin_elementwise_fma(f2{a_eff, a_eff}, cdp, f2{oma, oma} * SS2[j]);
        Sd[j] = fmaf(a_eff, gb.z, oma * Sd[j]);
        const int n = __popcll(hm);
        if (fill + n > GSR_HCAP_TW) {
          asm volatile("s_waitcnt lgkmcnt(0)" ::: "memory");
          flush(j, pend);
          asm volatile("s_waitcnt lgkmcnt(0)" ::: "memory");
          fill = 0;
          pend = 0ull;
        }
        if (hit) hits[fill + (int)mask_rank(hm)] = make_float4(u, u1, w, __uint_as_float((uint32_t)lane));
        if (lane == 0) list[jc] = (uint32_t)fill | ((uint32_t)n << 16);
        fill += n;
        pend |= 1ull << jc;
        if (rest == 0ull) return false;
        jc = jn;
        return true;
      };
      while (step(pa, pb, pc, pd, ya, yb, yc, yd) && step(ya, yb, yc, yd, pa, pb, pc, pd)) {
      }
      asm volatile("s_waitcnt lgkmcnt(0)" ::: "memory");
      flush(j, pend);
      asm volatile("s_waitcnt lgkmcnt(0)" ::: "memory");
    }
    __syncthreads();
  }
  if (hi > lo && lo + ((hi - lo - 1) & 63) - lane >= lo) {
    make_row();
    store_row();
  }
  GSR_TL_END(1, hi)
}

void launch_render_backward(const RenderSet& rs, const GeomState& g, const uint32_t* sorted_gauss,
                            const ImageState& img, const float* dL_dcolor, const float* dL_ddepth,
                            const float* dL_dalpha, const BackwardState& bw, hipStream_t stream) {
  const int nt = rs.gx * rs.gy;
  if (nt <= 0 || rs.V <= 0) return;
  const bool split = rs.ckpt != nullptr && rs.dpix2 == nullptr && rs.col2 == nullptr;
  const int extra = split ? rs.split_extra : 0;
  const dim3 grid(block_grid(rs, 4) + extra);
  const uint32_t* items = split ? img.split_items : nullptr;
  if (rs.dpix2 != nullptr) {
    g_blend_kernel[1] = "k_render_bwd_tw<true>";
    hipLaunchKernelGGL(k_render_bwd_tw<true>, dim3(block_grid(rs, 4)), dim3(64), 0, stream, rs,
                       (const uint2*)img.ranges, (const uint32_t*)img.quad_maxc, sorted_gauss, (const GaussRec*)g.rec,
                       (const uint32_t*)g.goff, (const float*)img.final_T, (const uint32_t*)img.n_contrib, dL_dcolor,
                       dL_ddepth, dL_dalpha, bw.grow, bw.reach);
    return;
  }
  g_blend_kernel[1] = "k_render_bwd";
  hipLaunchKernelGGL(k_render_bwd, grid, dim3(256), 0, stream, rs, (const uint2*)img.ranges,
                     (const uint32_t*)img.quad_maxc, sorted_gauss, (const GaussRec*)g.rec, (const uint32_t*)g.goff,
                     (const float*)img.final_T, (const uint32_t*)img.n_contrib, dL_dcolor, dL_ddepth, dL_dalpha,
                     bw.grow, bw.reach, extra, items);
}

bool split_on(int V, int P, int width, int height, long long instances) {
  const size_t tiles = (size_t)div_up(width, GSR_TILE_X) * div_up(height, GSR_TILE_Y);
  if (!split_fits(V, tiles)) return false;
  const char* e = getenv("GSR_BWD_SPLIT");
  if (e != nullptr && strcmp(e, "0") == 0) return false;
  return !fwd_tile_kernel(instances, (long long)V * P, V);
}

}

#ifdef GSR_TIMELINE
extern "C" int gsr_diag_pairs(void* host, int reset) {
  if (hipDeviceSynchronize() != hipSuccess) return -1;
  if (hipMemcpyFromSymbol(host, HIP_SYMBOL(gsr::g_pairs), 7 * sizeof(unsigned long long), 0,
                          hipMemcpyDeviceToHost) != hipSuccess)
    return -1;
  if (reset) {
    const unsigned long long z[7] = {0, 0, 0, 0, 0, 0, 0};
    if (hipMemcpyToSymbol(HIP_SYMBOL(gsr::g_pairs), z, sizeof(z), 0, hipMemcpyHostToDevice) != hipSuccess) return -1;
  }
  return 0;
}
extern "C" int gsr_diag_timeline(int which, void* host, int n) {
  if (which < 0 || which > 1 || n > GSR_TL_MAX) return -1;
  if (hipDeviceSynchronize() != hipSuccess) return -1;
  if (hipMemcpyFromSymbol(host, HIP_SYMBOL(gsr::g_timeline), sizeof(uint4) * n,
                          sizeof(uint4) * GSR_TL_MAX * which, hipMemcpyDeviceToHost) != hipSuccess)
    return -1;
  return 0;
}
#endif
```

threestudio-3dgs_amd/csrc/gsr_timed.hip:

```cpp
#include "gsr_chain.h"
#include "gsr_kernels.h"
#include "gsr_math.h"

namespace gsr {

template <bool TWO>
__attribute__((amdgpu_waves_per_eu(3, 8)))
__global__ __launch_bounds__(256) void k_tv_grad(GaussBackwardArgs a, ViewGradArgs va, TimedGradArgs tv) {
  const int idx = a.g0 + blockIdx.x * 256 + threadIdx.x;
  const bool valid = idx < a.g1;
  const int ix = valid ? idx : a.g0;
  const bool acc = tv.accumulate != 0;
  const bool scales_shared = tv.scales_v == nullptr, rots_shared = tv.rotations_v == nullptr;
  const unsigned long long reach_word = valid ? va.reach[ix] : 0ull;
  float dop = 0.f, dcr = 0.f, dcg = 0.f, dcb = 0.f;
  float d2[3] = {0.f, 0.f, 0.f};
  float dss[3] = {0.f, 0.f, 0.f}, dqs[4] = {0.f, 0.f, 0.f, 0.f};
  if (valid && acc) {
    dop = a.dL_dopacity[idx];
    if (a.dL_dcolors) dcr = a.dL_dcolors[3 * idx], dcg = a.dL_dcolors[3 * idx + 1], dcb = a.dL_dcolors[3 * idx + 2];
    if (TWO && tv.dcolors2)
      for (int k = 0; k < 3; ++k) d2[k] = tv.dcolors2[3 * idx + k];
    if (scales_shared)
      for (int k = 0; k < 3; ++k) dss[k] = a.dL_dscales[3 * idx + k];
    if (rots_shared)
      for (int k = 0; k < 4; ++k) dqs[k] = a.dL_drotations[4 * idx + k];
  }
  float ss[3] = {1.f, 1.f, 1.f}, qs[4] = {1.f, 0.f, 0.f, 0.f};
  if (scales_shared)
    for (int k = 0; k < 3; ++k) ss[k] = a.scales[3 * ix + k];
  if (rots_shared)
    for (int k = 0; k < 4; ++k) qs[k] = a.rotations[4 * ix + k];
  GaussRec nrec;
  uint32_t ngo = 0u;
  auto fetch = [&](int vl) {
    const size_t o = (size_t)(va.v0 + vl) * a.P + ix;
    nrec = va.g.rec[o];
    ngo = va.g.goff[o];
  };
  const int vfirst = reach_word != 0ull ? (int)__builtin_ctzll(reach_word) : va.V;
  if (vfirst < va.V) fetch(vfirst);
#pragma unroll 1
  for (int vl = 0; vl < va.V; ++vl) {
    const int vg = va.v0 + vl;
    const size_t o = (size_t)vg * a.P + ix;
    auto zero_rows = [&]() {
      if (!valid) return;
      float* m2 = va.dmeans2D + 3 * o;
      m2[0] = 0.f, m2[1] = 0.f, m2[2] = 0.f;
      for (int k = 0; k < 3; ++k) tv.dmeans_v[3 * o + k] = 0.f;
      if (!scales_shared)
        for (int k = 0; k < 3; ++k) tv.dscales_v[3 * o + k] = 0.f;
      if (!rots_shared)
        for (int k = 0; k < 4; ++k) tv.drotations_v[4 * o + k] = 0.f;
      if (TWO && tv.dcolors2_v)
        for (int k = 0; k < 3; ++k) tv.dcolors2_v[3 * o + k] = 0.f;
    };
    if (!((reach_word >> vl) & 1ull)) {
      zero_rows();
      continue;
    }
    const GaussRec gr = nrec;
    const uint32_t go = ngo;
    const float3 mean = make_float3(tv.means_v[3 * o], tv.means_v[3 * o + 1], tv.means_v[3 * o + 2]);
    float3 scale = make_float3(ss[0], ss[1], ss[2]);
    float4 rot = make_float4(qs[0], qs[1], qs[2], qs[3]);
    if (!scales_shared) scale = make_float3(tv.scales_v[3 * o], tv.scales_v[3 * o + 1], tv.scales_v[3 * o + 2]);
    if (!rots_shared)
      rot = make_float4(tv.rotations_v[4 * o], tv.rotations_v[4 * o + 1], tv.rotations_v[4 * o + 2],
                        tv.rotations_v[4 * o + 3]);
    const unsigned long long later = reach_word & ~((2ull << vl) - 1ull);
    if (later != 0ull) fetch((int)__builtin_ctzll(later));
    const ViewCam& cam = va.cam[vl];
    typedef __attribute__((address_space(4))) const float* cfptr;
    float viewm[16], projm[16];
#pragma unroll
    for (int i = 0; i < 16; ++i) viewm[i] = ((cfptr)cam.view)[i], projm[i] = ((cfptr)cam.proj)[i];
    ViewGeom vgm;
    vgm.view = viewm;
    vgm.proj = projm;
    vgm.tanx = cam.tanx;
    vgm.tany = cam.tany;
    vgm.fy = va.H / (2.0f * cam.tany);
    vgm.fx = va.W / (2.0f * cam.tanx);
    const float4* grow = va.grow + (size_t)(TWO ? 4 : 3) * va.row_start[vl];
    const uint2* cut = va.img.cut + (size_t)vg * va.tiles;
    const RowSums r = gather_rows<TWO>((uint32_t)ix, gr, go, va.gx, cut, grow);
    bool reached = (r.dmx != 0.f) | (r.dmy != 0.f) | (r.dca != 0.f) | (r.dcb != 0.f) | (r.dcc != 0.f) |
                   (r.dop != 0.f) | (r.dcr != 0.f) | (r.dcg != 0.f) | (r.dcbl != 0.f) | (r.ddep != 0.f);
    if (TWO) reached = reached | (r.dr2 != 0.f) | (r.dg2 != 0.f) | (r.db2 != 0.f);
    if (!reached) {
      zero_rows();
      continue;
    }
    float cov3D[6];
    cov3d_from_scale_rot(scale, a.scale_modifier, rot, cov3D);
    float dcv[6];
    float3 dm;
    cov2d_backward(mean, cov3D, vgm, r.dca, r.dcb, r.dcc, dcv, dm);
    proj_backward(mean, projm, r.dmx, r.dmy, dm);
    dm.x += viewm[2] * r.ddep;
    dm.y += viewm[6] * r.ddep;
    dm.z += viewm[10] * r.ddep;
    float ds[3], dq[4];
    scale_rot_backward(scale, rot, a.scale_modifier, dcv, ds, dq);
    if (valid) {
      float* m2 = va.dmeans2D + 3 * o;
      m2[0] = TWO ? r.dmx1 : r.dmx;
      m2[1] = TWO ? r.dmy1 : r.dmy;
      m2[2] = 0.f;
      tv.dmeans_v[3 * o] = dm.x;
      tv.dmeans_v[3 * o + 1] = dm.y;
      tv.dmeans_v[3 * o + 2] = dm.z;
      if (!scales_shared)
        for (int k = 0; k < 3; ++k) tv.dscales_v[3 * o + k] = ds[k];
      if (!rots_shared)
        for (int k = 0; k < 4; ++k) tv.drotations_v[4 * o + k] = dq[k];
      if (TWO && tv.dcolors2_v) {
        tv.dcolors2_v[3 * o] = r.dr2;
        tv.dcolors2_v[3 * o + 1] = r.dg2;
        tv.dcolors2_v[3 * o + 2] = r.db2;
      }
    }
    dcr += r.dcr;
    dcg += r.dcg;
    dcb += r.dcbl;
    dop += r.dop;
    if (TWO) {
      d2[0] += r.dr2;
      d2[1] += r.dg2;
      d2[2] += r.db2;
    }
#pragma unroll
    for (int k = 0; k < 3; ++k) dss[k] += ds[k];
#pragma unroll
    for (int k = 0; k < 4; ++k) dqs[k] += dq[k];
  }
  if (!valid) return;
  a.dL_dopacity[idx] = dop;
  if (a.dL_dcolors) {
    a.dL_dcolors[3 * idx] = dcr;
    a.dL_dcolors[3 * idx + 1] = dcg;
    a.dL_dcolors[3 * idx + 2] = dcb;
  }
  if (TWO && tv.dcolors2)
    for (int k = 0; k < 3; ++k) tv.dcolors2[3 * idx + k] = d2[k];
  if (scales_shared)
    for (int k = 0; k < 3; ++k) a.dL_dscales[3 * idx + k] = dss[k];
  if (rots_shared)
    for (int k = 0; k < 4; ++k) a.dL_drotations[4 * idx + k] = dqs[k];
}

void launch_timed_gauss_backward(const GaussBackwardArgs& a, const ViewGradArgs& va, const TimedGradArgs& tv,
                                 bool two_colors, hipStream_t stream) {
  const int n = a.g1 - a.g0;
  if (n <= 0 || va.V <= 0) return;
  auto kern = two_colors ? k_tv_grad<true> : k_tv_grad<false>;
  hipLaunchKernelGGL(kern, dim3(div_up(n, 256)), dim3(256), 0, stream, a, va, tv);
}

}
```

Baseline: 3979.

## Fuse per-Gaussian gradient-row offsets into preprocess via wave-level group prefix sums

Removes the per-Gaussian goff array and its count/write kernels. Preprocess now computes a wave-inclusive prefix of row counts, stores each Gaussian's offset within its 64-wide group in the upper bits of rec.d.w next to the clamp flags, and writes one partial per group. The scan kernel turns those partials into group bases. Backward and render kernels rebuild the row offset as group base plus local offset. This saves two launches and a full V*P pass over memory, at the cost of extra bit packing, a new tile-grid size limit, and an export kernel that masks out the packed bits.

```diff
diff --git a/threestudio-3dgs_amd/csrc/gsr_api.hip b/threestudio-3dgs_amd/csrc/gsr_api.hip
--- a/threestudio-3dgs_amd/csrc/gsr_api.hip
+++ b/threestudio-3dgs_amd/csrc/gsr_api.hip
@@ -251,6 +251,9 @@
   const int V = sc.V, P = sc.P;
   if (check_set(V, P) != GSR_OK) return GSR_EINVAL;
   if (sc.width <= 0 || sc.height <= 0) return fail(GSR_EINVAL, "%s", "image size must be positive");
+  if ((long long)GSR_ROW_GROUP * div_up(sc.width, GSR_TILE_X) * div_up(sc.height, GSR_TILE_Y) >=
+      (1ll << GSR_ROW_LOCAL_BITS))
+    return fail(GSR_EINVAL, "%s", "tile grid too large: 64 x tiles must stay below 2^29 (gradient-row offsets)");
   if ((sc.shs == nullptr) == (sc.colors_precomp == nullptr))
     return fail(GSR_EINVAL, "%s", "Please provide exactly one of either SHs or precomputed colors!");
   if (((sc.scales == nullptr || sc.rotations == nullptr) && sc.cov3D_precomp == nullptr) ||
@@ -1105,7 +1108,7 @@
   GeomState g = GeomState::carve((void*)geom, V, P, nullptr);
   hipStream_t s = (hipStream_t)stream;
   const size_t n = (size_t)V * (size_t)P;
-  if (out_rec) GSR_HIP_CHECK(hipMemcpyAsync(out_rec, g.rec, n * sizeof(GaussRec), hipMemcpyDeviceToDevice, s));
+  if (out_rec) launch_export_records(g.rec, (GaussRec*)out_rec, n, s);
   if (out_tiles) GSR_HIP_CHECK(hipMemcpyAsync(out_tiles, g.tiles, n * sizeof(uint2), hipMemcpyDeviceToDevice, s));
   return last_launch();
 }
diff --git a/threestudio-3dgs_amd/csrc/gsr_backward.hip b/threestudio-3dgs_amd/csrc/gsr_backward.hip
--- a/threestudio-3dgs_amd/csrc/gsr_backward.hip
+++ b/threestudio-3dgs_amd/csrc/gsr_backward.hip
@@ -138,13 +138,14 @@
     cnt += __popcll(bal);
   }
   asm volatile("s_waitcnt lgkmcnt(0)" ::: "memory");
+  const uint32_t* __restrict__ rgrp = va.g.row_group((size_t)vg);
   GaussRec nrec;
   uint32_t ngo = 0u;
   int nidx = 0;
   if (lane < cnt) {
     nidx = slice + list[lane];
     const size_t o0 = (size_t)vg * a.P + nidx;
-    nrec = va.g.rec[o0], ngo = va.g.goff[o0];
+    nrec = va.g.rec[o0], ngo = rgrp[nidx / GSR_ROW_GROUP];
   }
 #pragma unroll 1
   for (int i = lane; i - lane < cnt; i += 64) {
@@ -152,15 +153,15 @@
     const int idx = nidx;
     const size_t o = (size_t)vg * a.P + idx;
     const GaussRec gr = nrec;
-    const uint32_t go = ngo;
+    const uint32_t go = GeomState::row_base(ngo, gr.d.w);
     if (i + 64 < cnt) {
       nidx = slice + list[i + 64];
       const size_t on = (size_t)vg * a.P + nidx;
-      nrec = va.g.rec[on], ngo = va.g.goff[on];
+      nrec = va.g.rec[on], ngo = rgrp[nidx / GSR_ROW_GROUP];
     }
     float* m2 = va.dmeans2D + 3 * o;
     float4* rec = recv + (size_t)idx * (RS / 4);
-    const uint32_t clamp_bits = gr.d.w;
+    const uint32_t clamp_bits = gr.d.w & GSR_CLAMP_MASK;
     const RowSums r = gather_rows<TWO>((uint32_t)idx, gr, go, va.gx, cut, grow);
     bool reached = (r.dmx != 0.f) | (r.dmy != 0.f) | (r.dca != 0.f) | (r.dcb != 0.f) | (r.dcc != 0.f) |
                    (r.dop != 0.f) | (r.dcr != 0.f) | (r.dcg != 0.f) | (r.dcbl != 0.f) | (r.ddep != 0.f);
@@ -434,7 +435,9 @@
   auto fetch = [&](int vl) {
     const size_t o = (size_t)(va.v0 + vl) * a.P + ix;
     nrec = va.g.rec[o];
-    ngo = va.g.goff[o];
+    uint32_t grp = (uint32_t)ix / GSR_ROW_GROUP;
+    asm volatile("" : "+v"(grp));
+    ngo = va.g.row_group((size_t)(va.v0 + vl))[grp];
   };
   const int vfirst = reach_word != 0ull ? (int)__builtin_ctzll(reach_word) : va.V;
   if (vfirst < va.V) fetch(vfirst);
@@ -447,7 +450,7 @@
       continue;
     }
     const GaussRec gr = nrec;
-    const uint32_t go = ngo;
+    const uint32_t go = GeomState::row_base(ngo, gr.d.w);
     const unsigned long long later = reach_word & ~((2ull << vl) - 1ull);
     if (later != 0ull) fetch((int)__builtin_ctzll(later));
     const ViewCam& cam = va.cam[vl];
diff --git a/threestudio-3dgs_amd/csrc/gsr_binning.hip b/threestudio-3dgs_amd/csrc/gsr_binning.hip
--- a/threestudio-3dgs_amd/csrc/gsr_binning.hip
+++ b/threestudio-3dgs_amd/csrc/gsr_binning.hip
@@ -87,36 +87,21 @@
   if (t == 0) g.counters[2 * gridDim.x + v] = carry;
 }
 
-__global__ __launch_bounds__(256) void k_goff_count(int P, int nbg, GeomState g) {
-  __shared__ uint32_t s_wave[8];
-  const int v = blockIdx.x / nbg, b = blockIdx.x - v * nbg, t = threadIdx.x;
-  const uint2* tl = g.tiles + (size_t)v * P;
-  uint32_t sum = 0u, vis = 0u;
-#pragma unroll
-  for (int k = 0; k < GSR_GOFF_TILE / 256; ++k) {
-    const int i = b * GSR_GOFF_TILE + k * 256 + t;
-    const uint32_t x = i < P ? tl[i].x : 0u;
-    sum += x;
-    vis += x > 0u ? 1u : 0u;
-  }
-  sum = block_sum_u32<256>(sum, s_wave);
-  vis = block_sum_u32<256>(vis, s_wave);
-  if (t == 0) g.goff_part[(size_t)v * nbg + b] = sum, g.vis_part[(size_t)v * nbg + b] = vis;
-}
-
 __global__ __launch_bounds__(1024) void k_goff_scan(int nbg, GeomState g) {
   __shared__ uint32_t s_w[16];
   const int v = blockIdx.x, t = threadIdx.x, w = t >> 6, lane = t & 63;
   uint32_t* row = g.goff_part + (size_t)v * nbg;
+  const uint2* part = g.grp_part + (size_t)v * nbg;
   uint32_t carry = 0u, vis = 0u;
-  for (int i = t; i < nbg; i += 1024) vis += g.vis_part[(size_t)v * nbg + i];
   for (int c0 = 0; c0 < nbg; c0 += 1024 * 4) {
     const int i0 = c0 + 4 * t;
     uint32_t x[4], run = 0u;
 #pragma unroll
     for (int k = 0; k < 4; ++k) {
       x[k] = run;
-      run += i0 + k < nbg ? row[i0 + k] : 0u;
+      const uint2 p = i0 + k < nbg ? part[i0 + k] : make_uint2(0u, 0u);
+      run += p.x;
+      vis += p.y;
     }
     uint32_t inc = run;
 #pragma unroll
@@ -150,40 +135,6 @@
     for (int i = 0; i < 16; ++i) vt += s_w[i];
     g.counters[v] = carry;
     g.counters[gridDim.x + v] = vt;
-  }
-}
-
-__global__ __launch_bounds__(256) void k_goff_write(int P, int nbg, GeomState g) {
-  __shared__ uint32_t s_x[GSR_GOFF_TILE + GSR_GOFF_TILE / 16];
-  __shared__ uint32_t s_wave[8];
-  const int v = blockIdx.x / nbg, b = blockIdx.x - v * nbg, t = threadIdx.x;
-  const uint2* tl = g.tiles + (size_t)v * P + (size_t)b * GSR_GOFF_TILE;
-  uint32_t* go = g.goff + (size_t)v * P + (size_t)b * GSR_GOFF_TILE;
-  const int n = min(GSR_GOFF_TILE, P - b * GSR_GOFF_TILE);
-  constexpr int PER = GSR_GOFF_TILE / 256;
-  auto pad = [](int i) { return i + (i >> 4); };
-#pragma unroll
-  for (int k = 0; k < PER; ++k) {
-    const int i = k * 256 + t;
-    s_x[pad(i)] = i < n ? tl[i].x : 0u;
-  }
-  __syncthreads();
-  uint32_t x[PER], run = 0u;
-#pragma unroll
-  for (int k = 0; k < PER; ++k) {
-    const uint32_t c = s_x[pad(t * PER + k)];
-    x[k] = run;
-    run += c;
-  }
-  uint32_t tot;
-  const uint32_t off = g.goff_part[(size_t)v * nbg + b] + block_exclusive_scan<256>(run, &tot, s_wave);
-#pragma unroll
-  for (int k = 0; k < PER; ++k) s_x[pad(t * PER + k)] = off + x[k];
-  __syncthreads();
-#pragma unroll
-  for (int k = 0; k < PER; ++k) {
-    const int i = k * 256 + t;
-    if (i < n) go[i] = s_x[pad(i)];
   }
 }
 
@@ -340,10 +291,7 @@
 void launch_binning_counts(int V, int P, const GeomState& g, hipStream_t stream) {
   if (V <= 0) return;
   const int nbe = GeomState::dup_blocks(P);
-  const int nbg = GeomState::goff_blocks(P);
-  if (P > 0) hipLaunchKernelGGL(k_goff_count, dim3(V * nbg), dim3(256), 0, stream, P, nbg, g);
-  hipLaunchKernelGGL(k_goff_scan, dim3(V), dim3(1024), 0, stream, P > 0 ? nbg : 0, g);
-  if (P > 0) hipLaunchKernelGGL(k_goff_write, dim3(V * nbg), dim3(256), 0, stream, P, nbg, g);
+  hipLaunchKernelGGL(k_goff_scan, dim3(V), dim3(1024), 0, stream, P > 0 ? g.nbg : 0, g);
   if (P > 0)
     hipLaunchKernelGGL(k_inst_count, dim3(V * ((nbe + 4 * GSR_INST_GROUPS - 1) / (4 * GSR_INST_GROUPS))), dim3(256),
                        0, stream, P, nbe, g);
diff --git a/threestudio-3dgs_amd/csrc/gsr_common.h b/threestudio-3dgs_amd/csrc/gsr_common.h
--- a/threestudio-3dgs_amd/csrc/gsr_common.h
+++ b/threestudio-3dgs_amd/csrc/gsr_common.h
@@ -26,7 +26,10 @@
 #define GSR_SORT_TILE (GSR_SORT_THREADS * GSR_SORT_ITEMS)
 #define GSR_RADIX_BITS 8
 #define GSR_RADIX (1 << GSR_RADIX_BITS)
-#define GSR_GOFF_TILE 4096
+#define GSR_ROW_GROUP 64
+#define GSR_ROW_SHIFT 3
+#define GSR_ROW_LOCAL_BITS 29
+#define GSR_CLAMP_MASK 7u
 #define GSR_DUP_TILE 64
 
 #define GSR_NEAR_CULL 0.2f
@@ -158,9 +161,11 @@
   uint32_t* sort_counts;
   uint32_t* sort_totals;
   uint32_t* kept_counts;
-  uint32_t* goff;
+  uint2* grp_part;
   uint32_t* goff_part;
-  uint32_t* vis_part;
+  int nbg;
+  __device__ const uint32_t* row_group(size_t v) const { return goff_part + v * (size_t)nbg; }
+  __device__ static uint32_t row_base(uint32_t group_base, uint32_t dw) { return group_base + (dw >> GSR_ROW_SHIFT); }
   int vbits;
   __host__ __device__ uint32_t vmask() const { return vbits >= 32 ? 0xFFFFFFFFu : (1u << vbits) - 1u; }
   __host__ __device__ uint32_t vsent() const { return vbits > 26 ? 0u : (1u << (32 - vbits)) - 1u; }
@@ -170,7 +175,7 @@
   uint32_t* counters;
   static int sort_blocks(int P) { return div_up(P > 0 ? P : 1, GSR_SORT_TILE); }
   static int dup_blocks(int P) { return div_up(P > 0 ? P : 1, GSR_DUP_TILE); }
-  static int goff_blocks(int P) { return div_up(P > 0 ? P : 1, GSR_GOFF_TILE); }
+  __host__ __device__ static int goff_blocks(int P) { return div_up(P > 0 ? P : 1, GSR_ROW_GROUP); }
   static GeomState carve(void* base, int V, int P, size_t* bytes) {
     Carver c(base);
     GeomState g;
@@ -186,9 +191,9 @@
     g.sort_totals = c.take<uint32_t>(nv * GSR_RADIX);
     g.kept_counts = c.take<uint32_t>(nv * dup_blocks(P));
     g.counters = c.take<uint32_t>(3 * nv + 64);
-    g.goff = c.take<uint32_t>(n);
+    g.nbg = goff_blocks(P);
     g.goff_part = c.take<uint32_t>(nv * goff_blocks(P));
-    g.vis_part = c.take<uint32_t>(nv * goff_blocks(P));
+    g.grp_part = c.take<uint2>(nv * goff_blocks(P));
     g.vbits = 1;
     while (g.vbits < 32 && (1ull << g.vbits) < (unsigned long long)(P > 1 ? P : 2)) ++g.vbits;
     g.drange = c.take<uint32_t>(132);
diff --git a/threestudio-3dgs_amd/csrc/gsr_kernels.h b/threestudio-3dgs_amd/csrc/gsr_kernels.h
--- a/threestudio-3dgs_amd/csrc/gsr_kernels.h
+++ b/threestudio-3dgs_amd/csrc/gsr_kernels.h
@@ -37,6 +37,7 @@
 };
 void launch_preprocess(const PreprocessArgs& a, const SetCams& cams, const GeomState& g, hipStream_t stream,
                        const PreprocessTimed* timed = nullptr);
+void launch_export_records(const GaussRec* src, GaussRec* dst, size_t n, hipStream_t stream);
 
 void launch_binning_counts(int V, int P, const GeomState& g, hipStream_t stream);
 void launch_emit(int V, int P, int W, const GeomState& g, const SegInfo& inst, const TilePack& tp, uint32_t* keys,
diff --git a/threestudio-3dgs_amd/csrc/gsr_preprocess.hip b/threestudio-3dgs_amd/csrc/gsr_preprocess.hip
--- a/threestudio-3dgs_amd/csrc/gsr_preprocess.hip
+++ b/threestudio-3dgs_amd/csrc/gsr_preprocess.hip
@@ -1,5 +1,6 @@
 #include "gsr_kernels.h"
 #include "gsr_math.h"
+#include "gsr_wave.h"
 
 namespace gsr {
 
@@ -72,6 +73,9 @@
   if (!TIMED && a.col2 != nullptr) c2 = make_float3(a.col2[3 * ix], a.col2[3 * ix + 1], a.col2[3 * ix + 2]);
   const int gx = (a.W + GSR_TILE_X - 1) / GSR_TILE_X;
   const int gy = (a.H + GSR_TILE_Y - 1) / GSR_TILE_Y;
+  const int grp = __builtin_amdgcn_readfirstlane(idx0 / GSR_ROW_GROUP + ((t / GSR_ROW_GROUP) & 1));
+  static_assert(GSR_PRE_GAUSS == 2 * GSR_ROW_GROUP && GSR_ROW_GROUP == 64, "one wave per row group");
+  static_assert(GSR_ROW_SHIFT + GSR_ROW_LOCAL_BITS == 32, "d.w = clamp flags | local row offset");
 
 #pragma unroll 1
   for (int v = v0; v < v1; ++v) {
@@ -100,6 +104,7 @@
     int radius = 0;
     uint2 tiles = make_uint2(0u, 0u);
     uint32_t dkey = 0xFFFFFFFFu;
+    uint2 rect = make_uint2(0u, 0u);
     const float3 p_view = xform_point4x3(p_orig, viewmatrix);
     if (p_view.z > GSR_NEAR_CULL) {
       const float4 p_hom = xform_point4x4(p_orig, projmatrix);
@@ -132,10 +137,10 @@
           rec.a = make_float4(pimg.x, pimg.y, conic.x, conic.y);
           rec.b = make_float4(conic.z, opacity, p_view.z, c2.x);
           rec.c = make_float4(rgb.x, rgb.y, rgb.z, c2.y);
-          rec.d = make_uint4((uint32_t)xmin | ((uint32_t)ymin << 16), (uint32_t)xmax | ((uint32_t)ymax << 16),
-                             __float_as_uint(c2.z), clamp_bits);
-          if (valid) g.rec[vi] = rec;
+          rect = make_uint2((uint32_t)xmin | ((uint32_t)ymin << 16), (uint32_t)xmax | ((uint32_t)ymax << 16));
+          if (valid) g.rec[vi].a = rec.a, g.rec[vi].b = rec.b, g.rec[vi].c = rec.c;
           radius = r;
+          tiles.x = (uint32_t)area | clamp_bits << GSR_ROW_LOCAL_BITS;
           uint32_t kept = 0;
           const SpanPrep sp = span_prep(rec.a.x, rec.a.y, rec.a.z, rec.a.w, rec.b.x, rec.b.y);
           for (int ty = ymin; ty < ymax; ++ty) {
@@ -143,10 +148,24 @@
             span_row(sp, ty, xmin, xmax, t0, t1);
             kept += (uint32_t)(t1 - t0);
           }
-          tiles = make_uint2((uint32_t)area, kept);
+          tiles.y = kept;
           dkey = __float_as_uint(p_view.z);
         }
       }
+    }
+    const uint32_t rdw = tiles.x >> GSR_ROW_LOCAL_BITS;
+    tiles.x &= (1u << GSR_ROW_LOCAL_BITS) - 1u;
+    const uint32_t rows = valid ? tiles.x : 0u;
+    const uint32_t rincl = wave_incl_sum_dpp(rows);
+    const unsigned long long vbal = __ballot(rows != 0u);
+    if (rows != 0u)
+      g.rec[vi].d = make_uint4(rect.x, rect.y, __float_as_uint(c2.z), rdw | (rincl - rows) << GSR_ROW_SHIFT);
+    if ((t & 63) == 63 && grp < g.nbg) {
+      const size_t pe = ((size_t)v * (size_t)g.nbg + (size_t)grp) * sizeof(uint2);
+      uint32_t zo;
+      asm volatile("v_mov_b32 %0, 0" : "=v"(zo));
+      *reinterpret_cast<uint2*>(reinterpret_cast<char*>(g.grp_part) + pe + zo) =
+          make_uint2(rincl, (uint32_t)__popcll(vbal));
     }
     if (valid) {
       a.radii[vi] = radius;
@@ -217,6 +236,22 @@
   hipLaunchKernelGGL(k_depth_range, dim3(1), dim3(64), 0, stream, g.drange);
 }
 
+__global__ __launch_bounds__(256) void k_export_records(const uint4* __restrict__ src, uint4* __restrict__ dst,
+                                                        size_t pieces) {
+  const size_t i = (size_t)blockIdx.x * 256 + threadIdx.x;
+  if (i >= pieces) return;
+  uint4 x = src[i];
+  if ((i & 3) == 3) x.w &= GSR_CLAMP_MASK;
+  dst[i] = x;
+}
+
+void launch_export_records(const GaussRec* src, GaussRec* dst, size_t n, hipStream_t stream) {
+  if (n == 0) return;
+  const size_t pieces = 4 * n;
+  hipLaunchKernelGGL(k_export_records, dim3((unsigned)((pieces + 255) / 256)), dim3(256), 0, stream,
+                     reinterpret_cast<const uint4*>(src), reinterpret_cast<uint4*>(dst), pieces);
+}
+
 void launch_preprocess_kernel(const PreprocessArgs& a, const SetCams& cams, const GeomState& g, hipStream_t stream,
                               const PreprocessTimed* timed) {
   const int nvc = (a.V + GSR_PRE_VIEWS - 1) / GSR_PRE_VIEWS;
diff --git a/threestudio-3dgs_amd/csrc/gsr_render.hip b/threestudio-3dgs_amd/csrc/gsr_render.hip
--- a/threestudio-3dgs_amd/csrc/gsr_render.hip
+++ b/threestudio-3dgs_amd/csrc/gsr_render.hip
@@ -763,7 +763,7 @@
 __device__ __forceinline__ void bwd_tile(BwdLDS& s, const RenderSet& rs, int v, int tile, int chunk, bool split,
                                          const uint2* __restrict__ ranges, const uint32_t* __restrict__ quad_maxc,
                                          const uint32_t* __restrict__ sorted_gauss, const GaussRec* __restrict__ rec,
-                                         const uint32_t* __restrict__ goff, const float* __restrict__ final_Ts,
+                                         const uint32_t* __restrict__ rgrp, const float* __restrict__ final_Ts,
                                          const uint32_t* __restrict__ n_contrib, const float* __restrict__ dL_dcolor,
                                          const float* __restrict__ dL_ddepth, const float* __restrict__ dL_dalpha,
                                          float4* __restrict__ grow, unsigned long long* __restrict__ reach) {
@@ -781,7 +781,7 @@
     quad_maxc += vg * 4 * tiles;
     sorted_gauss += rs.inst_start[v];
     rec += vg * rs.P;
-    goff += vg * rs.P;
+    rgrp += vg * (size_t)GeomState::goff_blocks(rs.P);
     final_Ts += vg * HWs;
     n_contrib += vg * HWs;
     dL_dcolor += (size_t)v * 3 * HWs;
@@ -901,7 +901,7 @@
       if (piece == 2 && rs.col2 != nullptr)
         npc = make_float4(rs.col2[3 * g0], rs.col2[3 * g0 + 1], rs.col2[3 * g0 + 2], 0.f);
       if (piece == 2) ngo = g0;
-      if (piece == 3) ngo = goff[g0];
+      if (piece == 3) ngo = rgrp[g0 / GSR_ROW_GROUP];
     }
     if (hi - 64 > lo) gi_next = fetch_raw(hi - 64);
   }
@@ -1062,7 +1062,8 @@
         } else {
           const uint32_t dx_ = __float_as_uint(npc.x), dy_ = __float_as_uint(npc.y);
           const int xmin = dx_ & 0xffff, ymin = dx_ >> 16, xmax = dy_ & 0xffff;
-          s.slot[cst] = ngo + (uint32_t)((tyi - ymin) * (xmax - xmin) + (txi - xmin));
+          s.slot[cst] = GeomState::row_base(ngo, __float_as_uint(npc.w)) +
+                        (uint32_t)((tyi - ymin) * (xmax - xmin) + (txi - xmin));
         }
       }
       if (rowp != nullptr) *rowp = rowv;
@@ -1076,7 +1077,7 @@
           if (piece == 2 && rs.col2 != nullptr)
             npc = make_float4(rs.col2[3 * gnx], rs.col2[3 * gnx + 1], rs.col2[3 * gnx + 2], 0.f);
           if (piece == 2) ngo = gnx;
-          if (piece == 3) ngo = goff[gnx];
+          if (piece == 3) ngo = rgrp[gnx / GSR_ROW_GROUP];
         }
         if (h - 128 > lo) gi_next = fetch_raw(h - 128);
       }
@@ -1242,7 +1243,7 @@
 
 __global__ __launch_bounds__(256) __attribute__((amdgpu_waves_per_eu(5, 8))) void k_render_bwd(
     RenderSet rs, const uint2* __restrict__ ranges, const uint32_t* __restrict__ quad_maxc,
-    const uint32_t* __restrict__ sorted_gauss, const GaussRec* __restrict__ rec, const uint32_t* __restrict__ goff,
+    const uint32_t* __restrict__ sorted_gauss, const GaussRec* __restrict__ rec, const uint32_t* __restrict__ rgrp,
     const float* __restrict__ final_Ts, const uint32_t* __restrict__ n_contrib, const float* __restrict__ dL_dcolor,
     const float* __restrict__ dL_ddepth, const float* __restrict__ dL_dalpha, float4* __restrict__ grow,
     unsigned long long* __restrict__ reach, int extra, const uint32_t* __restrict__ items) {
@@ -1264,7 +1265,7 @@
   v = __builtin_amdgcn_readfirstlane(v);
   tile = __builtin_amdgcn_readfirstlane(tile);
   chunk = __builtin_amdgcn_readfirstlane(chunk);
-  bwd_tile(s, rs, v, tile, chunk, split, ranges, quad_maxc, sorted_gauss, rec, goff, final_Ts,
+  bwd_tile(s, rs, v, tile, chunk, split, ranges, quad_maxc, sorted_gauss, rec, rgrp, final_Ts,
                 n_contrib, dL_dcolor, dL_ddepth, dL_dalpha, grow, reach);
 }
 
@@ -1272,7 +1273,7 @@
 template <bool TWO>
 __global__ __launch_bounds__(64) void k_render_bwd_tw(
     RenderSet rs, const uint2* __restrict__ ranges, const uint32_t* __restrict__ quad_maxc,
-    const uint32_t* __restrict__ sorted_gauss, const GaussRec* __restrict__ rec, const uint32_t* __restrict__ goff,
+    const uint32_t* __restrict__ sorted_gauss, const GaussRec* __restrict__ rec, const uint32_t* __restrict__ rgrp,
     const float* __restrict__ final_Ts, const uint32_t* __restrict__ n_contrib, const float* __restrict__ dL_dcolor,
     const float* __restrict__ dL_ddepth, const float* __restrict__ dL_dalpha, float4* __restrict__ grow,
     unsigned long long* __restrict__ reach) {
@@ -1298,7 +1299,7 @@
     quad_maxc += vgs * 4 * tiles;
     sorted_gauss += rs.inst_start[v];
     rec += vgs * rs.P;
-    goff += vgs * rs.P;
+    rgrp += vgs * (size_t)GeomState::goff_blocks(rs.P);
     final_Ts += vgs * HW;
     n_contrib += vgs * HW;
     dL_dcolor += (size_t)v * 3 * HW;
@@ -1393,7 +1394,7 @@
       na = r[0];
       nb = r[1];
       nd = r[3];
-      ngo = goff[g];
+      ngo = rgrp[g / GSR_ROW_GROUP];
       ng = g;
     }
     {
@@ -1532,7 +1533,8 @@
                       : emb ? make_float4(vcopy(nb.w), vcopy(nc.w), vcopy(nd.z), 0.f)
                             : make_float4(vcopy(n2.x), vcopy(n2.y), vcopy(n2.z), 0.f);
     const uint32_t cdx = __float_as_uint(vcopy(nd.x)), cdy = __float_as_uint(vcopy(nd.y));
-    const uint32_t cgo = __float_as_uint(vcopy(__uint_as_float(ngo)));
+    const uint32_t cgo = GeomState::row_base(__float_as_uint(vcopy(__uint_as_float(ngo))),
+                                             __float_as_uint(vcopy(nd.w)));
     const int rel_c = h - 1 - lane;
     const bool staged = rel_c >= lo;
     uint32_t keep4 = 0u;
@@ -1666,13 +1668,13 @@
     g_blend_kernel[1] = "k_render_bwd_tw<true>";
     hipLaunchKernelGGL(k_render_bwd_tw<true>, dim3(block_grid(rs, 4)), dim3(64), 0, stream, rs,
                        (const uint2*)img.ranges, (const uint32_t*)img.quad_maxc, sorted_gauss, (const GaussRec*)g.rec,
-                       (const uint32_t*)g.goff, (const float*)img.final_T, (const uint32_t*)img.n_contrib, dL_dcolor,
+                       (const uint32_t*)g.goff_part, (const float*)img.final_T, (const uint32_t*)img.n_contrib, dL_dcolor,
                        dL_ddepth, dL_dalpha, bw.grow, bw.reach);
     return;
   }
   g_blend_kernel[1] = "k_render_bwd";
   hipLaunchKernelGGL(k_render_bwd, grid, dim3(256), 0, stream, rs, (const uint2*)img.ranges,
-                     (const uint32_t*)img.quad_maxc, sorted_gauss, (const GaussRec*)g.rec, (const uint32_t*)g.goff,
+                     (const uint32_t*)img.quad_maxc, sorted_gauss, (const GaussRec*)g.rec, (const uint32_t*)g.goff_part,
                      (const float*)img.final_T, (const uint32_t*)img.n_contrib, dL_dcolor, dL_ddepth, dL_dalpha,
                      bw.grow, bw.reach, extra, items);
 }
diff --git a/threestudio-3dgs_amd/csrc/gsr_timed.hip b/threestudio-3dgs_amd/csrc/gsr_timed.hip
--- a/threestudio-3dgs_amd/csrc/gsr_timed.hip
+++ b/threestudio-3dgs_amd/csrc/gsr_timed.hip
@@ -17,14 +17,14 @@
   float d2[3] = {0.f, 0.f, 0.f};
   float dss[3] = {0.f, 0.f, 0.f}, dqs[4] = {0.f, 0.f, 0.f, 0.f};
   if (valid && acc) {
-    dop = a.dL_dopacity[idx];
-    if (a.dL_dcolors) dcr = a.dL_dcolors[3 * idx], dcg = a.dL_dcolors[3 * idx + 1], dcb = a.dL_dcolors[3 * idx + 2];
+    dop = a.dL_dopacity[ix];
+    if (a.dL_dcolors) dcr = a.dL_dcolors[3 * ix], dcg = a.dL_dcolors[3 * ix + 1], dcb = a.dL_dcolors[3 * ix + 2];
     if (TWO && tv.dcolors2)
-      for (int k = 0; k < 3; ++k) d2[k] = tv.dcolors2[3 * idx + k];
+      for (int k = 0; k < 3; ++k) d2[k] = tv.dcolors2[3 * ix + k];
     if (scales_shared)
-      for (int k = 0; k < 3; ++k) dss[k] = a.dL_dscales[3 * idx + k];
+      for (int k = 0; k < 3; ++k) dss[k] = a.dL_dscales[3 * ix + k];
     if (rots_shared)
-      for (int k = 0; k < 4; ++k) dqs[k] = a.dL_drotations[4 * idx + k];
+      for (int k = 0; k < 4; ++k) dqs[k] = a.dL_drotations[4 * ix + k];
   }
   float ss[3] = {1.f, 1.f, 1.f}, qs[4] = {1.f, 0.f, 0.f, 0.f};
   if (scales_shared)
@@ -32,11 +32,9 @@
   if (rots_shared)
     for (int k = 0; k < 4; ++k) qs[k] = a.rotations[4 * ix + k];
   GaussRec nrec;
-  uint32_t ngo = 0u;
   auto fetch = [&](int vl) {
     const size_t o = (size_t)(va.v0 + vl) * a.P + ix;
     nrec = va.g.rec[o];
-    ngo = va.g.goff[o];
   };
   const int vfirst = reach_word != 0ull ? (int)__builtin_ctzll(reach_word) : va.V;
   if (vfirst < va.V) fetch(vfirst);
@@ -51,8 +49,11 @@
       for (int k = 0; k < 3; ++k) tv.dmeans_v[3 * o + k] = 0.f;
       if (!scales_shared)
         for (int k = 0; k < 3; ++k) tv.dscales_v[3 * o + k] = 0.f;
-      if (!rots_shared)
-        for (int k = 0; k < 4; ++k) tv.drotations_v[4 * o + k] = 0.f;
+      if (!rots_shared) {
+        float z;
+        asm volatile("v_mov_b32 %0, 0" : "=v"(z));
+        for (int k = 0; k < 4; ++k) tv.drotations_v[4 * o + k] = z;
+      }
       if (TWO && tv.dcolors2_v)
         for (int k = 0; k < 3; ++k) tv.dcolors2_v[3 * o + k] = 0.f;
     };
@@ -61,7 +62,6 @@
       continue;
     }
     const GaussRec gr = nrec;
-    const uint32_t go = ngo;
     const float3 mean = make_float3(tv.means_v[3 * o], tv.means_v[3 * o + 1], tv.means_v[3 * o + 2]);
     float3 scale = make_float3(ss[0], ss[1], ss[2]);
     float4 rot = make_float4(qs[0], qs[1], qs[2], qs[3]);
@@ -85,6 +85,9 @@
     vgm.fx = va.W / (2.0f * cam.tanx);
     const float4* grow = va.grow + (size_t)(TWO ? 4 : 3) * va.row_start[vl];
     const uint2* cut = va.img.cut + (size_t)vg * va.tiles;
+    uint32_t grp = (uint32_t)ix / GSR_ROW_GROUP;
+    asm volatile("" : "+v"(grp));
+    const uint32_t go = GeomState::row_base(va.g.row_group((size_t)vg)[grp], gr.d.w);
     const RowSums r = gather_rows<TWO>((uint32_t)ix, gr, go, va.gx, cut, grow);
     bool reached = (r.dmx != 0.f) | (r.dmy != 0.f) | (r.dca != 0.f) | (r.dcb != 0.f) | (r.dcc != 0.f) |
                    (r.dop != 0.f) | (r.dcr != 0.f) | (r.dcg != 0.f) | (r.dcbl != 0.f) | (r.ddep != 0.f);
@@ -137,18 +140,18 @@
     for (int k = 0; k < 4; ++k) dqs[k] += dq[k];
   }
   if (!valid) return;
-  a.dL_dopacity[idx] = dop;
+  a.dL_dopacity[ix] = dop;
   if (a.dL_dcolors) {
-    a.dL_dcolors[3 * idx] = dcr;
-    a.dL_dcolors[3 * idx + 1] = dcg;
-    a.dL_dcolors[3 * idx + 2] = dcb;
+    a.dL_dcolors[3 * ix] = dcr;
+    a.dL_dcolors[3 * ix + 1] = dcg;
+    a.dL_dcolors[3 * ix + 2] = dcb;
   }
   if (TWO && tv.dcolors2)
-    for (int k = 0; k < 3; ++k) tv.dcolors2[3 * idx + k] = d2[k];
+    for (int k = 0; k < 3; ++k) tv.dcolors2[3 * ix + k] = d2[k];
   if (scales_shared)
-    for (int k = 0; k < 3; ++k) a.dL_dscales[3 * idx + k] = dss[k];
+    for (int k = 0; k < 3; ++k) a.dL_dscales[3 * ix + k] = dss[k];
   if (rots_shared)
-    for (int k = 0; k < 4; ++k) a.dL_drotations[4 * idx + k] = dqs[k];
+    for (int k = 0; k < 4; ++k) a.dL_drotations[4 * ix + k] = dqs[k];
 }
 
 void launch_timed_gauss_backward(const GaussBackwardArgs& a, const ViewGradArgs& va, const TimedGradArgs& tv,
```

Result: no change. 4002 (median of 6 runs) (+0.6%).
